# pvjosue/CWFA

Measured on AMD Instinct MI355X. Metric: volumes/sec inverse-pass @512×512×96 fp32; NLL match vs ref (1/2/4/8 GPU), higher is better.
Workload: dtype f32 (storage, accumulation, wavelets, couplings); convolution products on the bf16 matrix cores from an exact three-way bf16 split of both fp32 operands, six products per fp32 product: fp32-equivalent; plain-fp32-MFMA figure: fp32_mfma; 1 GPU; 512x512x96 volume, 4-scale CWFA (CAT blocks, 64 ch) + LRNN inverse, z=0, batch 1/GPU, random-init weights (BASELINE.json configs[2]); precision=split, parallelism=replicated x1 (independent volumes per GPU, no collective)

## Files before the change

### cwfa_amd/_lib.py

```python
import ctypes as C
import os

_HERE = os.path.dirname(os.path.abspath(__file__))
LIB_PATH = os.path.join(_HERE, "libcwfa_hip.so")

CLAMP = {"NONE": 0, "ATAN": 1, "TANH": 2, "SIGMOID": 3}
ACT = {None: 0, "none": 0, "elu": 1, "prelu": 2, "gelu": 3, "relu": 4}
CHAIN_MAX = 8

c_f32p = C.c_void_p
c_i64p = C.c_void_p
c_f64p = C.c_void_p


class AffineStage(C.Structure):
    _fields_ = [("s_raw", c_f32p), ("t", c_f32p), ("s_bs", C.c_int64), ("t_bs", C.c_int64), ("clamp_kind", C.c_int),
                ("clamp", C.c_float), ("pre_scale", C.c_float), ("t_neg_div_sqrt2", C.c_int), ("perm", c_i64p),
                ("perm_axis", C.c_int), ("gin", C.c_int)]


class Chain(C.Structure):
    _fields_ = [("n_stages", C.c_int), ("stage", AffineStage * CHAIN_MAX), ("src_c", C.c_void_p), ("src_h", C.c_void_p)]


class ChainGrads(C.Structure):
    _fields_ = [("ds", c_f32p * CHAIN_MAX), ("dt", c_f32p * CHAIN_MAX), ("ds_bs", C.c_int64 * CHAIN_MAX),
                ("dt_bs", C.c_int64 * CHAIN_MAX)]


class ConvOpts(C.Structure):
    _fields_ = [("bias", c_f32p), ("act", C.c_int), ("prelu_alpha", c_f32p), ("residual", c_f32p), ("res_bs", C.c_int64),
                ("act2", C.c_int), ("in_scale", c_f32p), ("in_shift", c_f32p), ("in_affine_bs", C.c_int), ("in_add", c_f32p),
                ("in_add_bs", C.c_int64), ("upshuffle2", C.c_int), ("in_blocked8", C.c_int), ("out_blocked8", C.c_int),
                ("in_cat", c_f32p), ("in_cat_bs", C.c_int64), ("in_cat_from", C.c_int), ("in_cat_c1", C.c_int), ("out_stats", c_f64p), ("prelu_per_channel", C.c_int),
                ("out_sample_stats", c_f64p)]


class Couple(C.Structure):
    _fields_ = [("x", c_f32p), ("y", c_f32p), ("x_bs", C.c_int64), ("y_bs", C.c_int64), ("n", C.c_int), ("clamp_kind", C.c_int),
                ("clamp", C.c_float), ("pre_scale", C.c_float), ("rev", C.c_int), ("logdet", c_f64p), ("in_blocked8", C.c_int)]


class EvalAffine(C.Structure):
    _fields_ = [("enabled", C.c_int), ("scale", C.c_float), ("std", C.c_float), ("mean", C.c_float)]


class EvalPost(C.Structure):
    _fields_ = [("normalize", C.c_int), ("threshold", C.c_int), ("norm_sub", C.c_float), ("norm_div", C.c_float),
                ("vol_min", C.c_float), ("lower", C.c_float), ("upper", C.c_float), ("clamp_value", C.c_float)]


LION_MAX_TENSORS = 96
LION_BLOCK_ELEMS = 4096


class LionTensor(C.Structure):
    _fields_ = [("p", c_f32p), ("g", c_f32p), ("m", c_f32p), ("numel", C.c_int64)]


class LionTable(C.Structure):
    _fields_ = [("n", C.c_int), ("t", LionTensor * LION_MAX_TENSORS)]


NLL_MAX_LEVELS = 8


class NllLevels(C.Structure):
    _fields_ = [("n", C.c_int), ("level", c_f32p * NLL_MAX_LEVELS), ("bs", C.c_int64 * NLL_MAX_LEVELS)]


EXTREMA_STRIDE = 12
SELECT_WORKSPACE_BYTES = 8448
PREP_MAX_BINS = 10239
PREP_MOMENTS_WORKSPACE = 4096
PREP_VOL = {"none": 0, "two": 1, "le": 2, "maxnorm": 3, "max_only": 4}
PREP_APPLY = {"clamp_zero": 0, "sub_div": 1, "div_mul": 2}
DECONV_PRE = {None: 0, "none": 0, "relu": 1}
DECONV_POST = {None: 0, "none": 0, "abs": 1}

i, i64, f, d, p = C.c_int, C.c_int64, C.c_float, C.c_double, C.c_void_p
SIGNATURES = {
    "cwfa_version": (i, []),
    "cwfa_last_error": (C.c_char_p, []),
    "cwfa_set_option": (i, [C.c_char_p, i]),
    "cwfa_haar1d_fwd_f32": (i, [p, p, p, i, i, i64, i64, i64, i64, p]),
    "cwfa_haar1d_inv_f32": (i, [p, p, p, i, i, i64, i64, i64, i64, p]),
    "cwfa_haar2d_fwd_f32": (i, [p, p, i, i, i, i, i, f, p]),
    "cwfa_haar2d_inv_f32": (i, [p, p, i, i, i, i, i, f, p]),
    "cwfa_haar3d_fwd_f32": (i, [p, p, i, i, i, i, i, f, i64, p]),
    "cwfa_haar3d_inv_f32": (i, [p, p, i, i, i, i, i, f, i64, p]),
    "cwfa_gather_f32": (i, [p, p, p, i, i, i, i, i, i64, i64, p]),
    "cwfa_affine_f32": (i, [p, p, C.POINTER(AffineStage), i, i, i, i, i, i64, i64, p, p, p]),
    "cwfa_channel_affine_f32": (i, [p, p, p, p, i, p, p, i, i, i64, i64, i64, p]),
    "cwfa_chain_inv_f32": (i, [p, p, p, C.POINTER(Chain), i, i, i, i, i64, i64, i64, p, p]),
    "cwfa_chain_inv_var_f32": (i, [p, p, C.POINTER(Chain), f, f, i, i, i, i, i64, i64, p]),
    "cwfa_chain_inv_roi_cov_f32": (i, [p, C.POINTER(Chain), f, i, i, i, i, i, p, i, p, i, p, i64, p]),
    "cwfa_rand_uniform_f32": (i, [p, i, i64, i64, C.c_uint64, C.c_uint32, C.c_uint32, p]),
    "cwfa_rand_trunc_normal_f32": (i, [p, i, i64, i64, f, C.c_uint64, C.c_uint32, C.c_uint32, p]),
    "cwfa_chain_inv_samples_f32": (i, [p, p, p, C.POINTER(Chain), i, i, i, i, i, i64, i64, i64, i64, i64, i64, f, C.c_uint64, C.c_uint32,
                                       C.c_uint32, p]),
    "cwfa_chain_nll_map_f32": (i, [p, p, p, p, C.POINTER(Chain), i, i, i, i, i64, i64, i64, i64, p, p]),
    "cwfa_nll_compose_f32": (i, [C.POINTER(NllLevels), p, i, i, i64, i64, p]),
    "cwfa_chain_fwd_f32": (i, [p, p, p, C.POINTER(Chain), p, i, i, i, i, i64, i64, i64, p, p, p]),
    "cwfa_conv2d_packed_floats": (i64, [i, i, i]),
    "cwfa_conv2d_pack_f32": (i, [p, p, i, i, i, i, p]),
    "cwfa_conv2d_f32": (i, [p, p, p, i, i, i, i, i, i, i64, i64, C.POINTER(ConvOpts), p]),
    "cwfa_subnet_pack1x1_f32": (i, [p, p, p]),
    "cwfa_subnet_layer_tape_f32": (i, [p, p, p, p, p, p, p, i, i, i, i64, i64, i64, p]),
    "cwfa_subnet_layer_f32": (i, [p, p, p, p, p, p, i, i, i, i64, i64, p]),
    "cwfa_conv3d_1k1_f32": (i, [p, p, p, p, p, p, p, i, i, i, i, i, p]),
    "cwfa_conv3d_1k1_split_f32": (i, [p, p, p, p, p, p, p, i, i, i, i, i, p]),
    "cwfa_channel_stats_f32": (i, [p, p, i, i, i64, i64, p]),
    "cwfa_bn_fold_f32": (i, [p, d, p, p, p, p, f, p, i, p, p, i, p]),
    "cwfa_maxpool_f32": (i, [p, p, p, p, p, i, i, i, i, i, i, p]),
    "cwfa_sample_stats_f32": (i, [p, p, i, i64, p]),
    "cwfa_layernorm_apply_f32": (i, [p, p, p, p, f, p, i, i64, p]),
    "cwfa_convnext_tail_f32": (i, [p, p, p, p, f, p, p, p, p, p, p, p, i, p, i, i, i64, i64, i64, i64, i64, p]),
    "cwfa_attention_combine_f32": (i, [p, p, p, p, p, p, p, p, i, i, i64, p]),
    "cwfa_scale_channels_f32": (i, [p, p, p, i, i, i64, p]),
    "cwfa_axpby_f32": (i, [p, p, f, f, p, i64, p]),
    "cwfa_bn_running_update_f32": (i, [p, C.c_double, f, p, p, p, i, p]),
    "cwfa_bn_finish_f32": (i, [p, d, p, p, p, f, i, p, p, f, p, p, f, f, i, p, p, i, i, p]),
    "cwfa_chain_bwd_f32": (i, [p, p, C.POINTER(Chain), C.POINTER(ChainGrads), p, p, i, i, i, i, i64, i64, i64, f, f, i, p, p]),
    "cwfa_affine_bwd_f32": (i, [p, p, C.POINTER(AffineStage), i, i, i, i, i, i64, i64, p, p, p, p, p]),
    "cwfa_chain_inv_bwd_f32": (i, [p, p, C.POINTER(Chain), C.POINTER(ChainGrads), i, i, i, i, i64, i64, f, i, i, p, p, p, p]),
    "cwfa_conv2d_wgrad_workspace_bytes": (i64, [i, i, i, i, i, i]),
    "cwfa_conv2d_wgrad_f32": (i, [p, p, p, p, p, i, i, i, i, i, i, i64, i64, f, p]),
    "cwfa_elu_bwd_f32": (i, [p, p, p, p, i, i64, i64, i64, i64, i64, p]),
    "cwfa_conv3d_hidden_fwd_f32": (i, [p, p, p, p, i, i, i, i, i, p]),
    "cwfa_conv3d_hidden_bwd_f32": (i, [p, p, p, p, p, p, i, i, i, i, i, p]),
    "cwfa_conv3d_input_bwd_f32": (i, [p, p, p, i, i, i, i, i, p]),
    "cwfa_conv3d_wgrad_workspace_bytes": (i64, [i, i, i, i]),
    "cwfa_conv3d_wgrad_f32": (i, [p, p, p, p, p, i, i, i, i, i, i, i, f, p]),
    "cwfa_prelu_bwd_f32": (i, [p, p, p, p, p, i, i64, i64, i64, i64, p]),
    "cwfa_plane_affine_f32": (i, [p, p, p, i, p, p, i, i, i64, i64, i64, i64, p]),
    "cwfa_bn_bwd_stats_f32": (i, [p, p, p, p, i, i, i64, i64, i64, p]),
    "cwfa_bn_act_bwd_f32": (i, [p, p, p, i, p, p, p, p, p, i, i, i64, i64, i64, i64, p]),
    "cwfa_maxpool2_bwd_f32": (i, [p, p, p, p, i, i, i, i, p]),
    "cwfa_gelu_f32": (i, [p, p, p, i64, i, p]),
    "cwfa_layernorm_bwd_f32": (i, [p, p, p, p, p, p, p, p, p, i, i64, p]),
    "cwfa_attention_bwd_f32": (i, [p, p, p, p, p, p, p, p, p, i, i, i64, p]),
    "cwfa_split_workspace_bytes": (i64, [i, i, i64]),
    "cwfa_split_input_f32": (i, [p, p, i, i, i64, i64, p, p, i64, p, i64, p]),
    "cwfa_conv_split_packed_bytes": (i64, [i, i, i]),
    "cwfa_conv_split_pack_f32": (i, [p, p, i, i, i, i, p]),
    "cwfa_conv_split_f32": (i, [p, p, p, i, i, i, i, i, i, i64, C.POINTER(ConvOpts), p]),
    "cwfa_conv3x3_split_packed_bytes": (i64, [i, i]),
    "cwfa_conv3x3_split_pack_f32": (i, [p, p, i, i, p]),
    "cwfa_conv3x3_split_f32": (i, [p, p, p, i, i, i, i, i, i64, i64, C.POINTER(ConvOpts), p]),
    "cwfa_conv7x7_split_packed_bytes": (i64, [i, i]),
    "cwfa_conv7x7_split_pack_f32": (i, [p, p, i, i, p]),
    "cwfa_conv7x7_split_f32": (i, [p, p, p, i, i, i, i, i, i64, i64, C.POINTER(ConvOpts), p]),
    "cwfa_couple_rows": (i, [i, p]),
    "cwfa_conv3x3_split_couple_f32": (i, [p, p, p, i, i, i, i, i64, C.POINTER(Couple), p]),
    "cwfa_subnet_layer_split_packed_bytes": (i64, []),
    "cwfa_subnet_layer_split_pack_f32": (i, [p, p, p, p]),
    "cwfa_subnet_layer_split_f32": (i, [p, p, p, p, p, i, i, i, i64, i64, i, p]),
    "cwfa_subnet_layer_split_tape_f32": (i, [p, p, p, p, p, p, i, i, i, i64, i64, i64, p]),
    "cwfa_conv3x3_out_split_packed_bytes": (i64, [i]),
    "cwfa_conv3x3_out_split_pack_f32": (i, [p, p, i, p]),
    "cwfa_conv3x3_out_split_f32": (i, [p, p, p, p, i, i, i, i, i64, i64, i, p]),
    "cwfa_subnet_layer_first_packed_bytes": (i64, []),
    "cwfa_subnet_layer_first_pack_f32": (i, [p, p, p, i, p, p]),
    "cwfa_subnet_layer_first_f32": (i, [p, p, p, p, p, p, i, i, i, i, i64, i64, i64, i, p]),
    "cwfa_extract_views_f32": (i, [p, p, p, i, i, i, i, i, i, f, f, i64, p]),
    "cwfa_eval_splits": (i64, [i, i64]),
    "cwfa_volume_extrema_f32": (i, [p, p, p, p, i, i64, i64, i64, C.POINTER(EvalAffine), p]),
    "cwfa_volume_metrics_f32": (i, [p, p, p, p, i, i64, i64, i64, C.POINTER(EvalAffine), f, f, f, p]),
    "cwfa_mip3_f32": (i, [p, p, p, p, p, p, i, i, i, i, i64, i64, i, C.POINTER(EvalAffine), C.POINTER(EvalPost), p]),
    "cwfa_projection_compose_f32": (i, [p, p, p, p, p, i, i, i, i, i, i, i, p]),
    "cwfa_roi_means_f32": (i, [p, p, p, i, i, i, i, i, i64, p]),
    "cwfa_select_positive_f32": (i, [p, i, i64, i64, i64, p, p, p, p]),
    "cwfa_prep_volumes_f16": (i, [p, p, p, i, i, i, i, i, i, i, i, i, f, f, i, p]),
    "cwfa_prep_frames_f32": (i, [p, p, i, i, i, i, i, i, i, p]),
    "cwfa_histogram_f32": (i, [p, i64, f, f, p, i, p, i, p]),
    "cwfa_prep_apply_f32": (i, [p, i64, i, f, f, i, p]),
    "cwfa_moments_f64": (i, [p, i64, d, p, p, i, p]),
    "cwfa_stack_mean_std_f32": (i, [p, p, p, i, i64, i64, p]),
    "cwfa_lion_step_f32": (i, [C.POINTER(LionTable), f, f, f, f, p, p, p]),
    "cwfa_wmse_workspace_bytes": (i64, [i64]),
    "cwfa_wmse_loss_f32": (i, [p, p, p, f, f, p, p, p, i64, p]),
    "cwfa_select_nonzero_f32": (i, [p, i, i64, i64, i64, p, p, p, p]),
    "cwfa_deconv_spectrum_mul_c64": (i, [p, p, p, i, i64, i, i, p]),
    "cwfa_deconv_project_f32": (i, [p, p, i, i, i, i, i, i, i, i, i, i, i, p]),
    "cwfa_deconv_ratio_f32": (i, [p, p, p, p, i64, p]),
    "cwfa_deconv_clamp_f32": (i, [p, i64, p, p, f, p]),
    "cwfa_deconv_update_f32": (i, [p, p, i, i, i, i, p]),
}
del i, i64, f, d, p

_lib = None


class CwfaHipError(RuntimeError):
    pass


def lib():
    global _lib
    if _lib is None:
        if not os.path.exists(LIB_PATH):
            raise CwfaHipError(
                f"{LIB_PATH} not found: build the HIP extension first (python -m cwfa_amd.build, or "
                f"__graft_entry__.build()).  cwfa_amd has no CPU / PyTorch fallback.")
        import torch
        h = C.CDLL(LIB_PATH)
        for name, (res, args) in SIGNATURES.items():
            fn = getattr(h, name)
            fn.restype = res
            fn.argtypes = args
        if h.cwfa_version() < 100:
            raise CwfaHipError("libcwfa_hip.so is older than this Python layer")
        _lib = h
    return _lib


def check(rc, what=""):
    if rc != 0:
        msg = lib().cwfa_last_error()
        raise CwfaHipError(f"{what or 'libcwfa_hip'} failed (code {rc}): {msg.decode() if msg else ''}")
```

### cwfa_amd/csrc/conv2d.hip

```cpp
#include "conv_internal.h"

#include <string.h>
#include <type_traits>

namespace {

template <int KS_, int CK_, int MT_, int NT_, int WM_, int WN_, int XV_ = 1>
struct Cfg {
    static constexpr int KS = KS_, CK = CK_, MT = MT_, NT = NT_, WM = WM_, WN = WN_;
    static constexpr int XV = XV_;
    static_assert(XV_ == 1 || (XV_ == 4 && KS_ == 1), "vector staging needs halo-free tiles");
    static constexpr int PAD = KS / 2;
    static constexpr int NTHREADS = 64 * WM * WN;
    static constexpr int CT = 32 * MT * WM;
    static constexpr int TR = NT * WN;
    static constexpr int TC = 32;
    static constexpr int XR = TR + KS - 1;
    static constexpr int XC = TC + KS - 1;
    static constexpr int XS = CK * XR * XC;
    static constexpr int XS_PAD = (XS + 3) & ~3;
    static constexpr int WS = KS * KS * CK * CT;
    static constexpr int XPT = (XS / XV + NTHREADS - 1) / NTHREADS;
    static constexpr int WPT = (WS / 4 + NTHREADS - 1) / NTHREADS;
    static constexpr int BUF = XS_PAD + WS;
// ... 481 lines not shown
    if (ks == 7) return cls == 0 ? Sel{6, C7_32::CT, C7_32::CK} : Sel{7, C7_64::CT, C7_64::CK};
    return Sel{-1, 0, 0};
}

int classify_epilogue(const cwfa_conv_opts& o) {
    const bool res = o.residual != nullptr;
    if (o.out_blocked8) return EPI_NONE_BLK8;
    if (o.upshuffle2) return (!res && o.act == CWFA_ACT_NONE && o.act2 == CWFA_ACT_NONE) ? EPI_UP : EPI_GENERIC;
    if (!res && o.act2 == CWFA_ACT_NONE) {
        if (o.act == CWFA_ACT_NONE) return EPI_NONE;
        if (o.act == CWFA_ACT_ELU) return EPI_ELU;
        if (o.act == CWFA_ACT_PRELU) return EPI_PRELU;
    }
    if (res && o.act == CWFA_ACT_NONE && o.act2 == CWFA_ACT_ELU) return EPI_RES_ELU;
    if (res && o.act == CWFA_ACT_NONE && o.act2 == CWFA_ACT_PRELU) return EPI_RES_PRELU;
    if (res && o.act == CWFA_ACT_GELU && o.act2 == CWFA_ACT_NONE) return EPI_GELU_RES;
    return EPI_GENERIC;
}

template <class C>
int prepare(ConvParams& p, dim3& grid) {
    p.tiles_x = (p.W + C::TC - 1) / C::TC;
    p.tiles_y = (p.H + C::TR - 1) / C::TR;
    p.nchunks = (p.Cin + C::CK - 1) / C::CK;
    const int ctiles = (p.Cout + C::CT - 1) / C::CT;
    CWFA_REQUIRE((int64_t)p.tiles_x * p.tiles_y < (1ll << 31) && ctiles <= 65535 && p.B <= 65535, CWFA_E_SHAPE,
                 "cwfa_conv2d_f32: grid too large");
    CWFA_REQUIRE((int64_t)(p.Cin + C::CK) * p.H * p.W * 4 < (1ll << 31), CWFA_E_SHAPE,
                 "cwfa_conv2d_f32: one sample's input must stay below 2 GiB (32-bit buffer offsets)");
    grid = dim3((unsigned)(p.tiles_x * p.tiles_y), ctiles, p.B);
    return CWFA_OK;
}

template <class C, int EPI, bool PRO>
int launch_epi(ConvParams p, hipStream_t stream) {
    dim3 grid;
    int rc = prepare<C>(p, grid);
    if (rc) return rc;
    constexpr int LDS = EPI == EPI_GENERIC && C::LDS_BYTES < C::NTHREADS * 64 ? C::NTHREADS * 64 : C::LDS_BYTES;
    rc = cwfa_max_lds<&conv2d_mfma_kernel<C, EPI, PRO>>(LDS, "cwfa_conv2d_f32");
    if (rc) return rc;
    hipLaunchKernelGGL((conv2d_mfma_kernel<C, EPI, PRO>), grid, dim3(C::NTHREADS), LDS, stream, p);
    CWFA_LAUNCH_CHECK("cwfa_conv2d_f32");
    return CWFA_OK;
}

template <class C, unsigned ALLOWED, bool PRO>
int launch_sel(const ConvParams& p, int epi, hipStream_t st) {
    if (!(ALLOWED & (1u << epi)) && epi != EPI_NONE_BLK8) epi = EPI_GENERIC;
    switch (epi) {
        case EPI_NONE: if constexpr (ALLOWED & (1u << EPI_NONE)) return launch_epi<C, EPI_NONE, PRO>(p, st); break;
        case EPI_ELU: if constexpr (ALLOWED & (1u << EPI_ELU)) return launch_epi<C, EPI_ELU, PRO>(p, st); break;
        case EPI_RES_ELU: if constexpr (ALLOWED & (1u << EPI_RES_ELU)) return launch_epi<C, EPI_RES_ELU, PRO>(p, st); break;
        case EPI_PRELU: if constexpr (ALLOWED & (1u << EPI_PRELU)) return launch_epi<C, EPI_PRELU, PRO>(p, st); break;
        case EPI_RES_PRELU: if constexpr (ALLOWED & (1u << EPI_RES_PRELU)) return launch_epi<C, EPI_RES_PRELU, PRO>(p, st); break;
        case EPI_GELU_RES: if constexpr (ALLOWED & (1u << EPI_GELU_RES)) return launch_epi<C, EPI_GELU_RES, PRO>(p, st); break;
        case EPI_UP: if constexpr (ALLOWED & (1u << EPI_UP)) return launch_epi<C, EPI_UP, PRO>(p, st); break;
        case EPI_NONE_BLK8:
            if constexpr (ALLOWED & (1u << EPI_NONE_BLK8)) return launch_epi<C, EPI_NONE_BLK8, PRO>(p, st);
            cwfa_set_error("cwfa_conv2d_f32: out_blocked8 is built for the 1x1 kernels with more than 32 output channels");
            return CWFA_E_SHAPE;
        default: break;
    }
    return launch_epi<C, EPI_GENERIC, PRO>(p, st);
}

template <class C, unsigned ALLOWED, unsigned ALLOWED_PRO>
int launch(const ConvParams& p, int epi, hipStream_t st) {
    if (p.o.in_scale || p.o.in_add) return launch_sel<C, ALLOWED_PRO, true>(p, epi, st);
    return launch_sel<C, ALLOWED, false>(p, epi, st);
}

}
int g_cwfa_split_xcd_map = 1;
int g_cwfa_split_rows16 = 1;
extern int g_cwfa_mip3_ablate;
namespace {

int fill_params(ConvParams& p, const char* name, const float* x, const float* w_packed, float* y, int B, int Cin, int H,
                int W, int Cout, int64_t x_bs, int64_t y_bs, const cwfa_conv_opts* opts) {
    CWFA_REQUIRE(B >= 0 && Cin > 0 && Cout > 0 && H >= 0 && W >= 0, CWFA_E_INVAL, "%s: bad size", name);
    if (B == 0 || H == 0 || W == 0) return 1;
    CWFA_REQUIRE(x && w_packed && y, CWFA_E_INVAL, "%s: null pointer", name);
    CWFA_REQUIRE(!opts || !opts->out_sample_stats, CWFA_E_INVAL, "%s: out_sample_stats is a feature of the few-channel cwfa_conv7x7_split_f32", name);
    CWFA_REQUIRE((int64_t)Cin * H * W < (1ll << 30) && (int64_t)Cout * H * W * (p.o.upshuffle2 ? 1 : 1) < (1ll << 30), CWFA_E_SHAPE, "%s: C*H*W exceeds the 32-bit byte offsets of a tile (2^30 elements per image)", name);
    CWFA_REQUIRE(cwfa_aligned16(w_packed), CWFA_E_ALIGN, "%s: packed weights must be 16-byte aligned", name);
    p.x = x; p.wp = w_packed; p.y = y;
    p.B = B; p.Cin = Cin; p.H = H; p.W = W; p.Cout = Cout;
    p.x_bs = x_bs; p.y_bs = y_bs;
    p.products = g_cwfa_operand == CwfaOperand::split3 ? 6 : 1;
    if (opts) p.o = *opts;
    CWFA_REQUIRE(!(p.o.in_scale && !p.o.in_shift), CWFA_E_INVAL, "%s: in_scale without in_shift", name);
    CWFA_REQUIRE(p.o.act >= 0 && p.o.act <= CWFA_ACT_RELU && p.o.act2 >= 0 && p.o.act2 <= CWFA_ACT_RELU, CWFA_E_INVAL,
                 "%s: bad activation", name);
    CWFA_REQUIRE(!((p.o.act == CWFA_ACT_PRELU || p.o.act2 == CWFA_ACT_PRELU) && !p.o.prelu_alpha), CWFA_E_INVAL,
                 "%s: PReLU without prelu_alpha", name);
    return CWFA_OK;
}

typedef Cfg<1, 16, 2, 4, 4, 2> CS;
constexpr int CS_XB = 3 * 2 * 8 * 32 * 16, CS_WB = 3 * 2 * 256 * 16, CS_BUFB = CS_XB + CS_WB;

__device__ __forceinline__ void split3(float v, unsigned short (&o)[3]) {
    const __bf16 a1 = (__bf16)v;
    const float r1 = v - (float)a1;
    const __bf16 a2 = (__bf16)r1;
    const float r2 = r1 - (float)a2;
    const __bf16 a3 = (__bf16)r2;
    o[0] = __builtin_bit_cast(unsigned short, a1);
    o[1] = __builtin_bit_cast(unsigned short, a2);
    o[2] = __builtin_bit_cast(unsigned short, a3);
}

__device__ __forceinline__ unsigned short f16_bits(float v) { return __builtin_bit_cast(unsigned short, (_Float16)v); }

template <bool F16 = false>
__global__ __launch_bounds__(256) void split_input_kernel(const float* __restrict__ x, uint4* __restrict__ ws, int Cin, int CG2,
                                                          int64_t HW, int64_t x_bs, const float* __restrict__ sc,
                                                          const float* __restrict__ sh, int64_t aff_bs,
                                                          const float* __restrict__ add, int64_t add_bs) {
    const int64_t px = (int64_t)blockIdx.x * 256 + threadIdx.x;
    if (px >= HW) return;
    const int cg = blockIdx.y, b = blockIdx.z;
    unsigned short pc[3][8];
#pragma unroll
    for (int j = 0; j < 8; ++j) {
        const int c = cg * 8 + j;
        float v = 0.f;
        if (c < Cin) {
            v = x[(int64_t)b * x_bs + (int64_t)c * HW + px];
            if (sc) v = v * sc[(int64_t)b * aff_bs + c] + sh[(int64_t)b * aff_bs + c];
            if (add) v += add[(int64_t)b * add_bs + (int64_t)c * HW + px];
        }
        if constexpr (F16) {
            pc[0][j] = f16_bits(v);
            continue;
        }
        unsigned short o[3];
        split3(v, o);
        pc[0][j] = o[0]; pc[1][j] = o[1]; pc[2][j] = o[2];
    }
#pragma unroll
    for (int q = 0; q < (F16 ? 1 : 3); ++q) {
        uint4 u;
        u.x = pc[q][0] | ((unsigned)pc[q][1] << 16);
        u.y = pc[q][2] | ((unsigned)pc[q][3] << 16);
        u.z = pc[q][4] | ((unsigned)pc[q][5] << 16);
        u.w = pc[q][6] | ((unsigned)pc[q][7] << 16);
        ws[(((int64_t)b * 3 + q) * CG2 + cg) * HW + px] = u;
    }
}

template <bool F16 = false>
__global__ __launch_bounds__(256) void split_pack_kernel(const float* __restrict__ w, uint4* __restrict__ out, int Cout, int Cin,
                                                         int nchunks, int taps, int transposed, int64_t total) {
    const int64_t i = (int64_t)blockIdx.x * blockDim.x + threadIdx.x;
    if (i >= total) return;
    const int col = (int)(i % 256), h = (int)((i / 256) % 2), tap = (int)((i / 512) % taps);
    const int chunk = (int)((i / (512 * (int64_t)taps)) % nchunks);
    const int ctile = (int)(i / ((int64_t)512 * taps * nchunks));
    const int co = ctile * 256 + col;
    unsigned short pc[3][8];
#pragma unroll
    for (int j = 0; j < 8; ++j) {
        const int ci = chunk * 16 + h * 8 + j;
        float v = 0.f;
        if (co < Cout && ci < Cin)
            v = transposed ? w[((int64_t)ci * (Cout / 4) + (co >> 2)) * 4 + (co & 3)] : w[((int64_t)co * Cin + ci) * taps + tap];
        if constexpr (F16) {
            pc[0][j] = f16_bits(v);
            pc[1][j] = pc[2][j] = 0;
            continue;
        }
        unsigned short o[3];
        split3(v, o);
        pc[0][j] = o[0]; pc[1][j] = o[1]; pc[2][j] = o[2];
    }
#pragma unroll
    for (int q = 0; q < 3; ++q) {
        uint4 u;
        u.x = pc[q][0] | ((unsigned)pc[q][1] << 16);
        u.y = pc[q][2] | ((unsigned)pc[q][3] << 16);
        u.z = pc[q][4] | ((unsigned)pc[q][5] << 16);
        u.w = pc[q][6] | ((unsigned)pc[q][7] << 16);
        out[((((int64_t)ctile * nchunks + chunk) * taps + tap) * 3 + q) * 512 + h * 256 + col] = u;
    }
}

struct SplitParams {
    ConvParams c;
    const void* ws;
    int CG2;
    int64_t ws_bs;
};

template <int EPI, bool F16 = false>
__global__ __launch_bounds__(512, 1) void conv1x1_split_kernel(SplitParams sp) {
    typedef CS C;
    const ConvParams& p = sp.c;
    extern __shared__ __attribute__((aligned(16))) float smem[];
    char* lds = reinterpret_cast<char*>(smem);
    const Tile t = make_tile<C>(p);
    const bool six = p.products != 1;
    const int tid = threadIdx.x, wave = tid >> 6;
    const int64_t HW = (int64_t)p.H * p.W;
    constexpr unsigned OOB = 0x80000000u;

    unsigned xoff[3];
#pragma unroll
    for (int i = 0; i < 3; ++i) {
        const int e = tid + i * 512;
        const int px = e & 31, row = (e >> 5) & 7, h = (e >> 8) & 1, piece = e >> 9;
        const int gr = t.row0 + row, gc = t.col0 + px;
        xoff[i] = (gr < p.H && gc < p.W) ? (unsigned)((((int64_t)piece * sp.CG2 + h) * HW + (int64_t)gr * p.W + gc) * 16) : OOB;
    }
    const auto rx = CWFA_RSRC(reinterpret_cast<const char*>(sp.ws) + (int64_t)t.b * sp.ws_bs, (int)sp.ws_bs);
    const auto rw = CWFA_RSRC(reinterpret_cast<const char*>(p.wp) + (int64_t)t.ct * p.nchunks * CS_WB, p.nchunks * CS_WB);
    const int xchunk = (int)(2 * HW * 16);
    constexpr int NPC = F16 ? 1 : 3;
    auto dma = [&](int chunk, int buf) {
        char* base = lds + buf * CS_BUFB + wave * 1024;
#pragma unroll
        for (int i = 0; i < NPC; ++i)
            __builtin_amdgcn_raw_ptr_buffer_load_lds(rx, (lds_ptr)(base + i * 8192), 16, xoff[i], chunk * xchunk, 0, 0);
#pragma unroll
        for (int i = 0; i < NPC; ++i)
            __builtin_amdgcn_raw_ptr_buffer_load_lds(rw, (lds_ptr)(base + CS_XB + i * 8192), 16, (unsigned)(tid + i * 512) * 16u,
                                                     chunk * CS_WB, 0, 0);
    };

    f32x16 acc[2][4];
#pragma unroll
    for (int m = 0; m < 2; ++m)
#pragma unroll
        for (int n = 0; n < 4; ++n)
#pragma unroll
            for (int r = 0; r < 16; ++r) acc[m][n][r] = 0.f;

    const char* alane = lds + CS_XB + ((t.kh * 256) + t.wm * 64 + t.l31) * 16;
    const char* blane = lds + ((t.kh * 8 + t.wn * 4) * 32 + t.l31) * 16;

    dma(0, 0);
    dma(1, 1);
    if constexpr (F16) asm volatile("s_waitcnt vmcnt(2)" ::: "memory");
    else asm volatile("s_waitcnt vmcnt(6)" ::: "memory");
    __builtin_amdgcn_s_barrier();
    int buf = 0;
    for (int chunk = 0; chunk < p.nchunks; ++chunk) {
        int nb = buf + 2;
        nb = nb >= 3 ? nb - 3 : nb;
        dma(chunk + 2, nb);
        const char* ab = alane + buf * CS_BUFB;
        const char* bb = blane + buf * CS_BUFB;
        bf16x8 A[2][3], Bq[2][3];
#pragma unroll
        for (int m = 0; m < 2; ++m)
#pragma unroll
            for (int q = 0; q < 3; ++q) A[m][q] = *reinterpret_cast<const bf16x8*>(ab + (q * 512 + m * 32) * 16);
#pragma unroll
        for (int q = 0; q < 3; ++q) Bq[0][q] = *reinterpret_cast<const bf16x8*>(bb + (q * 512) * 16);
#pragma unroll
        for (int n = 0; n < 4; ++n) {
            if (n < 3) {
#pragma unroll
                for (int q = 0; q < 3; ++q) Bq[(n + 1) & 1][q] = *reinterpret_cast<const bf16x8*>(bb + (q * 512 + (n + 1) * 32) * 16);
            }
#pragma unroll
            for (int m = 0; m < 2; ++m) {
                f32x16 c = acc[m][n];
                if constexpr (F16) {
                    acc[m][n] = __builtin_amdgcn_mfma_f32_32x32x16_f16(__builtin_bit_cast(f16x8, A[m][0]), __builtin_bit_cast(f16x8, Bq[n & 1][0]),
                                                                       c, 0, 0, 0);
                    continue;
                }
                if (six) {
                    c = __builtin_amdgcn_mfma_f32_32x32x16_bf16(A[m][2], Bq[n & 1][0], c, 0, 0, 0);
                    c = __builtin_amdgcn_mfma_f32_32x32x16_bf16(A[m][1], Bq[n & 1][1], c, 0, 0, 0);
                    c = __builtin_amdgcn_mfma_f32_32x32x16_bf16(A[m][0], Bq[n & 1][2], c, 0, 0, 0);
                    c = __builtin_amdgcn_mfma_f32_32x32x16_bf16(A[m][1], Bq[n & 1][0], c, 0, 0, 0);
                    c = __builtin_amdgcn_mfma_f32_32x32x16_bf16(A[m][0], Bq[n & 1][1], c, 0, 0, 0);
                }
                c = __builtin_amdgcn_mfma_f32_32x32x16_bf16(A[m][0], Bq[n & 1][0], c, 0, 0, 0);
                acc[m][n] = c;
            }
        }
        if constexpr (F16) asm volatile("s_waitcnt vmcnt(2)\n\ts_waitcnt lgkmcnt(0)" ::: "memory");
        else asm volatile("s_waitcnt vmcnt(6)\n\ts_waitcnt lgkmcnt(0)" ::: "memory");
        __builtin_amdgcn_s_barrier();
        buf = buf + 1 == 3 ? 0 : buf + 1;
    }
    asm volatile("s_waitcnt vmcnt(0)" ::: "memory");
    __syncthreads();
    epilogue<C, EPI>(p, t, acc);
}

template <int EPI>
int launch_split(SplitParams sp, hipStream_t stream) {
    ConvParams& p = sp.c;
    p.tiles_x = (p.W + CS::TC - 1) / CS::TC;
    p.tiles_y = (p.H + CS::TR - 1) / CS::TR;
    const int ctiles = (p.Cout + CS::CT - 1) / CS::CT;
    CWFA_REQUIRE((int64_t)p.tiles_x * p.tiles_y < (1ll << 31) && ctiles <= 65535 && p.B <= 65535, CWFA_E_SHAPE,
                 "cwfa_conv_split_f32: grid too large");
    constexpr int LDS = 3 * CS_BUFB;
    return cwfa_with_operand([&](auto, auto f16) -> int {
        constexpr auto kern = &conv1x1_split_kernel<EPI, f16>;
        const int rc = cwfa_max_lds<kern>(LDS, "cwfa_conv_split_f32");
        if (rc) return rc;
        hipLaunchKernelGGL(kern, dim3((unsigned)(p.tiles_x * p.tiles_y), ctiles, p.B), dim3(512), LDS, stream, sp);
        CWFA_LAUNCH_CHECK("cwfa_conv_split_f32");
        return CWFA_OK;
    });
}

}

extern "C" int64_t cwfa_split_workspace_bytes(int B, int Cin, int64_t HW) {
    if (B < 0 || Cin <= 0 || HW < 0) return -1;
    const int64_t CG2 = 2 * ((Cin + 15) / 16);
    return (int64_t)B * 3 * CG2 * HW * 16;
}

extern "C" int cwfa_split_input_f32(const float* x, void* ws, int B, int Cin, int64_t HW, int64_t x_bs, const float* in_scale,
                                    const float* in_shift, int64_t in_affine_bs, const float* in_add, int64_t in_add_bs,
                                    void* stream) {
    CWFA_REQUIRE(x && ws, CWFA_E_INVAL, "cwfa_split_input_f32: null pointer");
    CWFA_REQUIRE(B >= 0 && Cin > 0 && HW >= 0 && B <= 65535, CWFA_E_SHAPE, "cwfa_split_input_f32: bad shape");
    CWFA_REQUIRE(!in_scale == !in_shift, CWFA_E_INVAL, "cwfa_split_input_f32: in_scale and in_shift go together");
    CWFA_REQUIRE(cwfa_aligned16(ws), CWFA_E_ALIGN, "cwfa_split_input_f32: workspace must be 16-byte aligned");
    if (B == 0 || HW == 0) return CWFA_OK;
    const int CG2 = 2 * ((Cin + 15) / 16);
    CWFA_REQUIRE((int64_t)3 * CG2 * HW * 16 < (1ll << 31), CWFA_E_SHAPE, "cwfa_split_input_f32: one sample's planes must stay below 2 GiB");
    return cwfa_with_operand([&](auto, auto f16) -> int {
        hipLaunchKernelGGL(split_input_kernel<f16>, dim3((unsigned)((HW + 255) / 256), CG2, B), dim3(256), 0, (hipStream_t)stream, x,
                           reinterpret_cast<uint4*>(ws), Cin, CG2, HW, x_bs, in_scale, in_shift, in_affine_bs, in_add, in_add_bs);
        CWFA_LAUNCH_CHECK("cwfa_split_input_f32");
        return CWFA_OK;
    });
}

extern "C" int64_t cwfa_conv_split_packed_bytes(int Cout, int Cin, int ks) {
    if (Cout <= 0 || Cin <= 0 || ks != 1) return -1;
    return (int64_t)((Cout + 255) / 256) * ((Cin + 15) / 16) * CS_WB;
}

extern "C" int cwfa_conv_split_pack_f32(const float* w, void* packed, int Cout, int Cin, int ks, int transposed, void* stream) {
    CWFA_REQUIRE(w && packed, CWFA_E_INVAL, "cwfa_conv_split_pack_f32: null pointer");
    CWFA_REQUIRE(Cout > 0 && Cin > 0 && ks == 1 && (!transposed || Cout % 4 == 0), CWFA_E_SHAPE,
                 "cwfa_conv_split_pack_f32: bad shape (1x1 / transposed 2x2 only; 3x3: cwfa_conv3x3_split_pack_f32)");
    CWFA_REQUIRE(cwfa_aligned16(packed), CWFA_E_ALIGN, "cwfa_conv_split_pack_f32: packed image must be 16-byte aligned");
    const int nchunks = (Cin + 15) / 16, taps = ks * ks;
    const int64_t total = (int64_t)((Cout + 255) / 256) * nchunks * taps * 512;
    return cwfa_with_operand([&](auto, auto f16) -> int {
        hipLaunchKernelGGL(split_pack_kernel<f16>, dim3((unsigned)((total + 255) / 256)), dim3(256), 0, (hipStream_t)stream, w,
                           reinterpret_cast<uint4*>(packed), Cout, Cin, nchunks, taps, transposed, total);
        CWFA_LAUNCH_CHECK("cwfa_conv_split_pack_f32");
        return CWFA_OK;
    });
}

extern "C" int cwfa_conv_split_f32(const void* ws, const void* w_packed, float* y, int B, int Cin, int H, int W, int Cout, int ks,
                                   int64_t y_bs, const cwfa_conv_opts* opts, void* stream) {
    CWFA_REQUIRE(!(opts && (opts->in_blocked8 || opts->out_blocked8 || opts->in_cat)), CWFA_E_INVAL,
                 "cwfa_conv_split_f32: blocked layouts / two-source inputs are not built here");
    CWFA_REQUIRE(ws && w_packed && y, CWFA_E_INVAL, "cwfa_conv_split_f32: null pointer");
    CWFA_REQUIRE(ks == 1, CWFA_E_SHAPE, "cwfa_conv_split_f32: kernel size %d (1x1 only; 3x3: cwfa_conv3x3_split_f32)", ks);
    SplitParams sp{};
    int rc = fill_params(sp.c, "cwfa_conv_split_f32", reinterpret_cast<const float*>(ws), reinterpret_cast<const float*>(w_packed), y,
                         B, Cin, H, W, Cout, 0, y_bs, opts);
    if (rc) return rc < 0 ? rc : CWFA_OK;
    ConvParams& p = sp.c;
    CWFA_REQUIRE(!p.o.in_scale && !p.o.in_add, CWFA_E_INVAL, "cwfa_conv_split_f32: the load-side prologue belongs in cwfa_split_input_f32");
    CWFA_REQUIRE(!p.o.upshuffle2 || (ks == 1 && Cout % 4 == 0), CWFA_E_SHAPE, "cwfa_conv_split_f32: upshuffle2 needs ks=1, Cout=4*Co");
    CWFA_REQUIRE(!p.o.out_stats && !p.o.prelu_per_channel, CWFA_E_INVAL, "cwfa_conv_split_f32: out_stats / prelu_per_channel are features of cwfa_conv3x3_split_f32");
    p.nchunks = (Cin + 15) / 16;
    sp.ws = ws;
    sp.CG2 = 2 * p.nchunks;
    sp.ws_bs = (int64_t)3 * sp.CG2 * H * W * 16;
    CWFA_REQUIRE(sp.ws_bs + (int64_t)4 * H * W * 16 < (1ll << 31) && (int64_t)(p.nchunks * ks * ks + 2) * CS_WB < (1ll << 31), CWFA_E_SHAPE,
                 "cwfa_conv_split_f32: one sample's planes / one cout tile's weights must stay below 2 GiB");
    const int epi = classify_epilogue(p.o);
    hipStream_t st = (hipStream_t)stream;
    switch (epi) {
        case EPI_NONE: return launch_split<EPI_NONE>(sp, st);
        case EPI_UP: return launch_split<EPI_UP>(sp, st);
        default: return launch_split<EPI_GENERIC>(sp, st);
    }
}

int g_cwfa_wino_min_cout = 1;
int g_cwfa_wino_2d = 512;
CwfaOperand g_cwfa_operand = CwfaOperand::split3;

extern "C" int cwfa_set_option(const char* name, int value) {
    CWFA_REQUIRE(name, CWFA_E_INVAL, "cwfa_set_option: null name");
    if (strcmp(name, "winograd_min_cout") == 0) {
        g_cwfa_wino_min_cout = value;
        return CWFA_OK;
    }
    if (strcmp(name, "winograd_2d") == 0) {
        g_cwfa_wino_2d = value;
        return CWFA_OK;
    }
    if (strcmp(name, "wgrad_split") == 0) {
        g_cwfa_wgrad_split = value != 0;
        return CWFA_OK;
    }
    if (strcmp(name, "wgrad_rows") == 0) {
        g_cwfa_wgrad_rows = value;
        return CWFA_OK;
    }
    if (strcmp(name, "split3x3_xcd_map") == 0) {
        g_cwfa_split_xcd_map = value;
        return CWFA_OK;
    }
    if (strcmp(name, "mip3_ablate") == 0) {
        CWFA_REQUIRE(value >= 0 && value <= 7, CWFA_E_INVAL, "cwfa_set_option: mip3_ablate is a mask of bits 0..2");
        g_cwfa_mip3_ablate = value;
        return CWFA_OK;
    }
    if (strcmp(name, "split3x3_rows16") == 0) {
        g_cwfa_split_rows16 = value;
        return CWFA_OK;
    }
    if (strcmp(name, "split_products") == 0) {
        CWFA_REQUIRE(value == 1 || value == 6, CWFA_E_INVAL, "cwfa_set_option: split_products must be 1 or 6");
        CWFA_REQUIRE(value == 1 || g_cwfa_operand != CwfaOperand::fp16, CWFA_E_INVAL,
                     "cwfa_set_option: split_products = 6 needs split_operand = 0 (the three-piece split is a bf16 format)");
        if (value == 6) g_cwfa_operand = CwfaOperand::split3;
        else if (g_cwfa_operand == CwfaOperand::split3) g_cwfa_operand = CwfaOperand::bf16;
        return CWFA_OK;
    }
    if (strcmp(name, "split_operand") == 0) {
        CWFA_REQUIRE(value == 0 || value == 1, CWFA_E_INVAL, "cwfa_set_option: split_operand must be 0 (bf16) or 1 (fp16)");
        CWFA_REQUIRE(value == 0 || g_cwfa_operand != CwfaOperand::split3, CWFA_E_INVAL,
                     "cwfa_set_option: split_operand = 1 (fp16) needs split_products = 1 (fp16 operands take one product)");
        if (value == 1) g_cwfa_operand = CwfaOperand::fp16;
        else if (g_cwfa_operand == CwfaOperand::fp16) g_cwfa_operand = CwfaOperand::bf16;
        return CWFA_OK;
    }
    cwfa_set_error("cwfa_set_option: unknown option '%s'", name);
    return CWFA_E_INVAL;
}

extern "C" int64_t cwfa_conv2d_packed_floats(int Cout, int Cin, int ks) {
    const Sel s = select_cfg(ks, Cout);
    if (s.id < 0 || Cout <= 0 || Cin <= 0) return -1;
    if (cwfa_wino_selected(ks, Cout)) return cwfa_wino_packed_floats(Cout, Cin);
    const int64_t ctiles = (Cout + s.CT - 1) / s.CT, nchunks = (Cin + s.CK - 1) / s.CK;
    return ctiles * nchunks * ks * ks * s.CK * s.CT;
}

extern "C" int cwfa_conv2d_pack_f32(const float* w, float* packed, int Cout, int Cin, int ks, int transposed, void* stream) {
    CWFA_REQUIRE(w && packed, CWFA_E_INVAL, "cwfa_conv2d_pack_f32: null pointer");
    CWFA_REQUIRE(!transposed || (ks == 1 && Cout % 4 == 0), CWFA_E_SHAPE,
                 "cwfa_conv2d_pack_f32: transposed source needs ks=1 (2x2 stride-2 deconv as 1x1) and Cout = 4*Co");
    const int64_t total = cwfa_conv2d_packed_floats(Cout, Cin, ks);
    CWFA_REQUIRE(total > 0, CWFA_E_SHAPE, "cwfa_conv2d_pack_f32: unsupported filter %dx%d, Cout=%d, Cin=%d", ks, ks, Cout, Cin);
    if (cwfa_wino_selected(ks, Cout)) return cwfa_wino_pack(w, packed, Cout, Cin, (hipStream_t)stream);
    const Sel s = select_cfg(ks, Cout);
    const int nchunks = (Cin + s.CK - 1) / s.CK;
    hipLaunchKernelGGL(pack_kernel, dim3((unsigned)((total + 255) / 256)), dim3(256), 0, (hipStream_t)stream, w, packed, Cout,
                       Cin, ks, s.CT, s.CK, nchunks, total, transposed);
    CWFA_LAUNCH_CHECK("cwfa_conv2d_pack_f32");
    return CWFA_OK;
}

extern "C" int cwfa_conv2d_f32(const float* x, const float* w_packed, float* y, int B, int Cin, int H, int W, int Cout, int ks,
                               int64_t x_bs, int64_t y_bs, const cwfa_conv_opts* opts, void* stream) {
    CWFA_REQUIRE(!(opts && opts->in_blocked8), CWFA_E_INVAL, "cwfa_conv2d_f32: in_blocked8 is a cwfa_conv3x3_split_f32 feature");
    CWFA_REQUIRE(!(opts && opts->in_cat) || (ks == 1 && Cout <= 64 && !opts->in_scale && !opts->in_add && opts->in_cat_from % 16 == 0 &&
                                             opts->in_cat_from > 0 && opts->in_cat_from < Cin && opts->in_cat_c1 > 0 &&
                                             opts->in_cat_c1 <= opts->in_cat_from),
                 CWFA_E_INVAL, "cwfa_conv2d_f32: in_cat needs a 1x1 bank with <= 64 outputs packed with in_cat_from (a multiple of 16) "
                               "columns for the first source, and no load-side affine / add");
    CWFA_REQUIRE(!(opts && opts->out_blocked8) || (ks == 1 && Cout % 8 == 0 && !opts->residual && opts->act == CWFA_ACT_NONE &&
                                                   opts->act2 == CWFA_ACT_NONE && !opts->upshuffle2 && !opts->in_scale && !opts->in_add &&
                                                   cwfa_aligned16(y) && (y_bs & 3) == 0 && (!opts->bias || cwfa_aligned16(opts->bias))),
                 CWFA_E_INVAL, "cwfa_conv2d_f32: out_blocked8 needs a plain 1x1 bank (bias only), Cout %% 8 == 0 and 16-byte aligned y / bias");
    const Sel s = select_cfg(ks, Cout);
    CWFA_REQUIRE(s.id >= 0, CWFA_E_SHAPE, "cwfa_conv2d_f32: kernel size %d not in {1,3,7}", ks);
    ConvParams p{};
    int rc = fill_params(p, "cwfa_conv2d_f32", x, w_packed, y, B, Cin, H, W, Cout, x_bs, y_bs, opts);
    if (rc) return rc < 0 ? rc : CWFA_OK;
    CWFA_REQUIRE(!p.o.upshuffle2 || (ks == 1 && Cout % 4 == 0), CWFA_E_SHAPE, "cwfa_conv2d_f32: upshuffle2 needs ks=1, Cout=4*Co");
    CWFA_REQUIRE(!p.o.out_stats && !p.o.prelu_per_channel, CWFA_E_INVAL, "cwfa_conv2d_f32: out_stats / prelu_per_channel are features of cwfa_conv3x3_split_f32");
    const int epi = classify_epilogue(p.o);
    hipStream_t st = (hipStream_t)stream;
    if (cwfa_wino_selected(ks, Cout)) return cwfa_wino_conv(x, w_packed, y, B, Cin, H, W, Cout, x_bs, y_bs, p.o, st);
// ... 69 lines not shown
```

### cwfa_amd/csrc/conv_split3x3.hip

```cpp
#include "conv_internal.h"

extern int g_cwfa_split_xcd_map;
extern int g_cwfa_split_rows16;

namespace {

constexpr int TR = 8, TC = 32;

template <int KS, int RPW = 4>
struct XG {
    static constexpr int TRW = 2 * RPW, NT = 2 * RPW;
    static constexpr int PAD = KS / 2, XR = TRW + 2 * PAD, XC = TC + 2 * PAD, NTAP = KS * KS;
    static constexpr int EPK = XR * XC;
    static constexpr int KHB = KS == 7 ? 8512 : RPW == 8 ? 9792 : 5440;
    static constexpr int XPB = 2 * KHB;
    static constexpr int XB = 3 * XPB;
    static constexpr bool SPECIAL = KS == 3 && RPW == 4;
    static constexpr int NEK = SPECIAL ? 2 : 3;
    static_assert(EPK * 16 <= KHB && KHB % 256 == 64 && 2 * EPK <= 512 * NEK, "staging entry map");
    static_assert(!SPECIAL || (EPK > 256 && EPK <= 384), "3x3 staging entry map");
    static_assert(KS == 3 || RPW == 4, "7x7: 8-row tiles");
};

template <int MPW, int KS = 3, int RPW = 4, int WM = 4>
// ... 229 lines not shown
            for (int mt = 0; mt < MPW; ++mt) {
                mfma6(acc[mt][nt], A[mt], Bq[nt % NB]);
                CWFA_FENCE();
                if (MA < MPW && nt == 0 && mt == 0) {
                    read_a(abase, MA, MPW);
#pragma unroll
                    for (int n2 = 1; n2 < NB && n2 < NT; ++n2) read_b(n2, bbase, n2);
                    CWFA_FENCE();
                }
            }
            if (nt == 0) {
                if (P == LA || P == LB) load_entry(cwfa_ic<0>{}, xs[0], sk[0], P == LA ? ce + 2 : co + 2);
                if (P == LA + 1 || P == LB + 1) load_entry(cwfa_ic<1>{}, xs[1], sk[1], P == LA + 1 ? ce + 2 : co + 2);
                if constexpr (NEK > 2) {
                    if (P == LA + 2 || P == LB + 2) load_entry(cwfa_ic<NEK - 1>{}, xs[NEK - 1], sk[NEK - 1], P == LA + 2 ? ce + 2 : co + 2);
                }
                CWFA_FENCE();
            }
            if (nt == 1) {
                dma_w(step + 1, sl ^ 1);
                CWFA_FENCE();
            }
        }
        {
            const int nP = P == NTAP - 1 ? 0 : P + 1;
            const int nA = 2 * nP, nB = 2 * nP + 1;
            const int nbufA = nA >= NTAP, ntA = nA - NTAP * nbufA, nbufB = nB >= NTAP, ntB = nB - NTAP * nbufB;
            const int noffA = nbufA * XB + ((ntA / KS) * XC + ntA % KS) * 16, noffB = nbufB * XB + ((ntB / KS) * XC + ntB % KS) * 16;
            read_b(0, blane + (sel ? noffB : noffA), 0);
            CWFA_FENCE();
        }
        asm volatile("s_waitcnt vmcnt(0)" ::: "memory");
        if constexpr (SIX) asm volatile("s_waitcnt lgkmcnt(3)" ::: "memory");
        else asm volatile("s_waitcnt lgkmcnt(1)" ::: "memory");
        __builtin_amdgcn_s_barrier();
        sl ^= 1;
        if (++P == NTAP) {
            P = 0;
            ce += 2;
        }
    }
    asm volatile("s_waitcnt vmcnt(0)" ::: "memory");

    const auto ry = CWFA_RSRC(p.y + (int64_t)b * p.y_bs, p.Cout * plane);
    const auto rr = CWFA_RSRC(p.o.residual ? p.o.residual + (int64_t)b * p.o.res_bs : p.y, p.o.residual ? p.Cout * plane : 0);
    const auto rb = CWFA_RSRC(p.o.bias ? p.o.bias : p.y, p.o.bias ? p.Cout * 4 : 0);
    const bool alpha_pc = p.o.prelu_per_channel != 0;
    const float alpha = (p.o.prelu_alpha && !alpha_pc) ? *p.o.prelu_alpha : 0.f;
    const auto rpa = CWFA_RSRC(alpha_pc ? p.o.prelu_alpha : p.y, alpha_pc ? p.Cout * 4 : 0);
    const int cwave = ct * CT + wm * MPW * 16;
    const unsigned glane = (unsigned)(4 * g) * (unsigned)plane;
    if constexpr (ACT1 == EPI_COUPLE) {
        static_assert(MPW <= 2 && !ADD, "coupling epilogue: narrow tilings only");
        constexpr int NP = MPW == 1 ? 2 : 4;
        const cwfa_couple& cp = p.cp;
        const auto cx = CWFA_RSRC(cp.x + (int64_t)b * cp.x_bs, cp.n * plane);
        const auto cy = CWFA_RSRC(cp.y + (int64_t)b * cp.y_bs, cp.n * plane);
        const unsigned jlane = (unsigned)((MPW == 1 ? 2 : 4) * g) * (unsigned)plane;
        const int jwave = wm * (MPW == 1 ? 8 : 16);
        float bs[NP], bt[NP];
#pragma unroll
        for (int k = 0; k < NP; ++k) {
            const int rs = k, rt = MPW == 1 ? k + 2 : 16 + k;
            bs[k] = __builtin_bit_cast(float, __builtin_amdgcn_raw_buffer_load_b32(rb, (unsigned)(16 * g), (cwave + rs) * 4, 0));
            bt[k] = __builtin_bit_cast(float, __builtin_amdgcn_raw_buffer_load_b32(rb, (unsigned)(16 * g), (cwave + rt) * 4, 0));
        }
        float ssum = 0.f;
#pragma unroll
        for (int nt = 0; nt < NT; ++nt) {
            const int row = row0 + wn * RW + (nt >> 1), col = col0 + 16 * (nt & 1) + c16;
            const bool ok = row < p.H && col < p.W;
            const unsigned po = ok ? (unsigned)((row * p.W + col) * 4) + jlane : OOB;
            float xv[NP];
#pragma unroll
            for (int k = 0; k < NP; ++k) xv[k] = __builtin_bit_cast(float, __builtin_amdgcn_raw_buffer_load_b32(cx, po, (jwave + k) * plane, 0));
#pragma unroll
            for (int k = 0; k < NP; ++k) {
                const float sr = acc[0][nt][k] + bs[k];
                float tr;
                if constexpr (MPW == 1) tr = acc[0][nt][k + 2] + bt[k];
                else tr = acc[MPW - 1][nt][k] + bt[k];
                const float sv = cwfa_soft_clamp(sr * cp.pre_scale, cp.clamp_kind, cp.clamp);
                const float tv = tr * cp.pre_scale;
                const float yv = cp.rev ? (xv[k] - tv) * __expf(-sv) : __expf(sv) * xv[k] + tv;
                __builtin_amdgcn_raw_buffer_store_b32(__builtin_bit_cast(unsigned, yv), cy, po, (jwave + k) * plane, 0);
                ssum += ok ? sv : 0.f;
            }
            CWFA_FENCE();
        }
        if (cp.logdet) {
            const double ws = cwfa_wave_sum((double)ssum);
            double* red = reinterpret_cast<double*>(lds);
            __builtin_amdgcn_s_barrier();
            if (lane == 0) red[wave] = ws;
            __syncthreads();
            if (tid == 0) {
                double tot = 0.0;
#pragma unroll
                for (int w = 0; w < 8; ++w) tot += red[w];
                atomicAdd(&cp.logdet[b], cp.rev ? -tot : tot);
            }
        }
        return;
    }
    const bool outb = p.o.out_blocked8 != 0;
    const bool want_stats = ACT1 != EPI_RUNTIME && p.o.out_stats != nullptr;
    float* red = reinterpret_cast<float*>(lds);
#pragma unroll
    for (int mt = 0; mt < MPW; ++mt) {
        float bias[4];
        float st1[4] = {0.f, 0.f, 0.f, 0.f}, st2[4] = {0.f, 0.f, 0.f, 0.f};
#pragma unroll
        for (int r = 0; r < 4; ++r)
            bias[r] = __builtin_bit_cast(float, __builtin_amdgcn_raw_buffer_load_b32(rb, (unsigned)(16 * g), (cwave + mt * 16 + r) * 4, 0));
        float al[4] = {alpha, alpha, alpha, alpha};
        if (alpha_pc) {
#pragma unroll
            for (int r = 0; r < 4; ++r)
                al[r] = __builtin_bit_cast(float, __builtin_amdgcn_raw_buffer_load_b32(rpa, (unsigned)(16 * g), (cwave + mt * 16 + r) * 4, 0));
        }
        constexpr int RLA = NT < 4 ? NT : 4;
        float rv[ACT1 == EPI_RUNTIME ? NT : 1][4];
        auto load_res = [&](int nt) {
            const int row = row0 + wn * RW + (nt >> 1), col = col0 + 16 * (nt & 1) + c16;
            const unsigned po = (row < p.H && col < p.W) ? (unsigned)((row * p.W + col) * 4) + glane : OOB;
#pragma unroll
            for (int r = 0; r < 4; ++r)
                rv[ACT1 == EPI_RUNTIME ? nt : 0][r] = __builtin_bit_cast(float, __builtin_amdgcn_raw_buffer_load_b32(rr, po, (cwave + mt * 16 + r) * plane, 0));
        };
        if constexpr (ACT1 == EPI_RUNTIME) {
#pragma unroll
            for (int nt = 0; nt < NT; ++nt)
#pragma unroll
                for (int r = 0; r < 4; ++r) rv[nt][r] = 0.f;
            if (p.o.residual) {
#pragma unroll
                for (int nt = 0; nt < RLA; ++nt) load_res(nt);
            }
            CWFA_FENCE();
        }
#pragma unroll
        for (int nt = 0; nt < NT; ++nt) {
            const int row = row0 + wn * RW + (nt >> 1), col = col0 + 16 * (nt & 1) + c16;
            if constexpr (ACT1 == EPI_RUNTIME) {
                if (nt + RLA < NT && p.o.residual) load_res(nt + RLA);
                CWFA_FENCE();
            }
            if constexpr (ACT1 != EPI_RUNTIME) {
                if (outb) {
                    f32x4 o4;
#pragma unroll
                    for (int r = 0; r < 4; ++r) o4[r] = cwfa_act_ct<ACT1>(acc[mt][nt][r] + bias[r], al[r]);
                    const unsigned pb = (row < p.H && col < p.W) ? (unsigned)(((g >> 1) * HW + row * p.W + col) * 32 + (g & 1) * 16) : OOB;
                    cwfa_buffer_store_b128(__builtin_bit_cast(u32x4, o4), ry, pb, (cwave + mt * 16) * plane);
                    continue;
                }
            }
            const unsigned po = (row < p.H && col < p.W) ? (unsigned)((row * p.W + col) * 4) + glane : OOB;
#pragma unroll
            for (int r = 0; r < 4; ++r) {
                const int soff = (cwave + mt * 16 + r) * plane;
                float v = acc[mt][nt][r] + bias[r];
                if constexpr (ACT1 == EPI_RUNTIME) {
                    v = cwfa_act(v, p.o.act, al[r]);
                    v += rv[nt][r];
                    v = cwfa_act(v, p.o.act2, al[r]);
                } else {
                    v = cwfa_act_ct<ACT1>(v, al[r]);
                    if (want_stats) {
                        const float vm = po != OOB ? v : 0.f;
                        st1[r] += vm;
                        st2[r] += vm * vm;
                    }
                }
                __builtin_amdgcn_raw_buffer_store_b32(__builtin_bit_cast(unsigned, v), ry, po, soff, 0);
            }
            CWFA_FENCE();
        }
        if constexpr (ACT1 != EPI_RUNTIME) {
            if (want_stats) {
#pragma unroll
                for (int r = 0; r < 4; ++r) {
                    const float a1 = cwfa_row16_sum(st1[r]), a2 = cwfa_row16_sum(st2[r]);
                    if (c16 == 0) {
                        const int ch = (wm * MPW + mt) * 16 + 4 * g + r;
                        red[(wn * CT + ch) * 2] = a1;
                        red[(wn * CT + ch) * 2 + 1] = a2;
                    }
                }
            }
        }
    }
    if constexpr (ACT1 != EPI_RUNTIME) {
        if (want_stats) {
            asm volatile("s_waitcnt lgkmcnt(0)\n\ts_barrier" ::: "memory");
            const int ch = ct * CT + tid;
            if (tid < CT && ch < p.Cout) {
                double s1 = 0.0, s2 = 0.0;
#pragma unroll
                for (int k = 0; k < WN; ++k) {
                    s1 += (double)red[(k * CT + tid) * 2];
                    s2 += (double)red[(k * CT + tid) * 2 + 1];
                }
                atomicAdd(&p.o.out_stats[2 * ch], s1);
                atomicAdd(&p.o.out_stats[2 * ch + 1], s2);
            }
        }
    }
}

namespace few {
constexpr int XR = TR + 6, XC = TC + 6, EPK = XR * XC;
constexpr int XPB = EPK * 16;
constexpr int NSTEP = 13, CT = 64, MPW = 2, WM = 2, WN = 4, RW = 2, NT = 4;
constexpr int WSL = 3 * 4 * CT * 16;
constexpr int OFF_W = 3 * XPB, LDS = OFF_W + 2 * WSL;
static_assert(2 * 512 >= EPK && 2 * LDS <= 160 * 1024, "few-channel 7x7: staging map / two blocks per CU");
}

template <bool SIX, bool F16>
__global__ __launch_bounds__(512, 2) void conv7x7_few_split_kernel(SParams p) {
    using namespace few;
    extern __shared__ __attribute__((aligned(16))) char lds[];
    const int tid = threadIdx.x, lane = tid & 63, c16 = lane & 15, g = lane >> 4;
    const int wave = __builtin_amdgcn_readfirstlane(tid >> 6);
    const int wm = wave % WM, wn = wave / WM;
    const int plane = p.H * p.W * 4;
    constexpr unsigned OOB = 0x80000000u;
    constexpr int NQ = SIX ? 3 : 1;
    const int b = blockIdx.z;
    int sp;
    if (p.xcd_map && (p.ntiles & 7) == 0) sp = (blockIdx.x & 7) * (p.ntiles >> 3) + (blockIdx.x >> 3);
    else sp = blockIdx.x;
    const int row0 = (sp / p.tiles_x) * TR, col0 = (sp % p.tiles_x) * TC;

    constexpr int NPC = (SIX ? WSL : WSL / 3) / 1024;
    const auto rw = CWFA_RSRC(p.wp, NSTEP * WSL);
    auto dma_w = [&](int slice, int slot) {
        cwfa_static_for<(NPC + 7) / 8>([&](auto ic_) {
            constexpr int i = decltype(ic_)::value;
            const int piece = i * 8 + wave;
            if (piece < NPC) {
                char* dst = lds + OFF_W + slot * WSL + piece * 1024;
                __builtin_amdgcn_raw_ptr_buffer_load_lds(rw, (lds_ptr)dst, 16, (unsigned)(lane * 16), slice * WSL + piece * 1024, 0, 0);
            }
        });
    };

    {
        const auto rx = CWFA_RSRC(p.x + (int64_t)b * p.x_bs, p.Cin * plane);
        float xv[2][8];
#pragma unroll
        for (int k = 0; k < 2; ++k) {
            const int e = tid + 512 * k, r = e / XC, c = e % XC;
            const int gr = row0 + r - 3, gc = col0 + c - 3;
            const bool ok = e < EPK && gr >= 0 && gr < p.H && gc >= 0 && gc < p.W;
            const unsigned fo = ok ? (unsigned)((gr * p.W + gc) * 4) : OOB;
#pragma unroll
            for (int j = 0; j < 8; ++j) xv[k][j] = __builtin_bit_cast(float, __builtin_amdgcn_raw_buffer_load_b32(rx, fo, j * plane, 0));
        }
        dma_w(0, 0);
#pragma unroll
        for (int k = 0; k < 2; ++k) {
            const int e = tid + 512 * k;
            bf16x8 pc[3];
#pragma unroll
            for (int j = 0; j < 8; ++j) {
                __bf16 a1, a2 = (__bf16)0.f, a3 = (__bf16)0.f;
                cwfa_split3<SIX, F16>(xv[k][j], a1, a2, a3);
                pc[0][j] = a1; pc[1][j] = a2; pc[2][j] = a3;
            }
            if (e < EPK) {
#pragma unroll
                for (int q = 0; q < NQ; ++q) *reinterpret_cast<bf16x8*>(lds + q * XPB + e * 16) = pc[q];
            }
        }
    }
    asm volatile("s_waitcnt vmcnt(0)\n\ts_waitcnt lgkmcnt(0)" ::: "memory");
    __builtin_amdgcn_s_barrier();

    const int alane = OFF_W + (g * CT + wm * MPW * 16 + c16) * 16;
    const int blane = (wn * RW * XC + c16) * 16;
    auto bbase_of = [&](int s) {
        const int t = 4 * s + g < 48 ? 4 * s + g : 48;
        return blane + ((t / 7) * XC + t % 7) * 16;
    };

    f32x4 acc[MPW][NT];
#pragma unroll
    for (int mt = 0; mt < MPW; ++mt)
#pragma unroll
        for (int nt = 0; nt < NT; ++nt) acc[mt][nt] = f32x4{0.f, 0.f, 0.f, 0.f};
    bf16x8 A[MPW][3], Bq[2][3];
    auto read_b = [&](int set, int bbase, int nt) {
#pragma unroll
        for (int q = 0; q < NQ; ++q)
            Bq[set][q] = *reinterpret_cast<const bf16x8*>(lds + bbase + q * XPB + ((nt >> 1) * XC + 16 * (nt & 1)) * 16);
    };
    auto mfma6 = [&](f32x4& c, const bf16x8 (&a)[3], const bf16x8 (&bb)[3]) {
        if constexpr (SIX) {
            CWFA_MFMA(a[2], bb[0], c);
            CWFA_MFMA(a[1], bb[1], c);
            CWFA_MFMA(a[0], bb[2], c);
            CWFA_MFMA(a[1], bb[0], c);
            CWFA_MFMA(a[0], bb[1], c);
        }
// ... 163 lines not shown
inline int nsteps_of(int Cin, int ntap = 9) { return ntap * (((Cin + 15) / 16 + 1) / 2); }

template <int MPW, bool ADD, int ACT1, int KS = 3, int RPW = 4, int WM = 4>
int launch(const SParams& p, hipStream_t stream) {
    typedef Geo<MPW, KS, RPW, WM> G;
    constexpr int TRW = XG<KS, RPW>::TRW;
    const int tiles_y = (p.H + TRW - 1) / TRW, ctiles = (p.Cout + G::CT - 1) / G::CT;
    SParams q = p;
    q.ntiles = p.tiles_x * tiles_y;
    q.ctiles = ctiles;
    q.xcd_map = g_cwfa_split_xcd_map;
    if ((int64_t)q.ntiles * ctiles >= (1ll << 31)) {
        cwfa_set_error("cwfa_conv3x3_split_f32: grid too large");
        return CWFA_E_SHAPE;
    }
    if ((ACT1 == EPI_RUNTIME || ACT1 == EPI_COUPLE) && (p.o.out_stats || p.o.out_blocked8)) {
        cwfa_set_error("cwfa_conv3x3_split_f32: out_stats / out_blocked8 reached a run-time epilogue");
        return CWFA_E_INVAL;
    }
    return cwfa_with_operand([&](auto six, auto f16) -> int {
        constexpr auto kern = &conv3x3_split_kernel<MPW, six, ADD, ACT1, KS, RPW, WM, f16>;
        const int rc = cwfa_max_lds<kern>(G::LDS, "cwfa_conv3x3_split_f32");
        if (rc) return rc;
        hipLaunchKernelGGL(kern, dim3((unsigned)(q.ntiles * ctiles), 1, p.B), dim3(512), G::LDS, stream, q);
        CWFA_LAUNCH_CHECK("cwfa_conv3x3_split_f32");
        return CWFA_OK;
    });
}

template <int MPW>
int launch_epi(const SParams& p, hipStream_t st) {
    const bool plain = !p.o.residual && p.o.act2 == CWFA_ACT_NONE;
    if (p.o.in_add) {
        if (plain && p.o.act == CWFA_ACT_PRELU) return launch<MPW, true, CWFA_ACT_PRELU>(p, st);
        return launch<MPW, true, EPI_RUNTIME>(p, st);
    }
    if (plain && p.o.act == CWFA_ACT_PRELU) return launch<MPW, false, CWFA_ACT_PRELU>(p, st);
    if (plain && p.o.act == CWFA_ACT_NONE) return launch<MPW, false, CWFA_ACT_NONE>(p, st);
    return launch<MPW, false, EPI_RUNTIME>(p, st);
}

void pack_bank(const float* w, void* packed, int Cout, int Cin, int ct, int ntap, hipStream_t st) {
    const int nchunks = (Cin + 15) / 16, nsteps = nsteps_of(Cin, ntap);
    const int64_t total = (int64_t)((Cout + ct - 1) / ct) * nsteps * 4 * ct;
    cwfa_with_operand([&](auto, auto f16) -> int {
        auto go = [&](auto CT) {
            hipLaunchKernelGGL((split3x3_pack_kernel<decltype(CT)::value, f16>), dim3((unsigned)((total + 255) / 256)), dim3(256), 0, st, w,
                               reinterpret_cast<uint4*>(packed), Cout, Cin, nchunks, nsteps, total, ntap);
        };
        if (ct == 16) go(cwfa_ic<16>{});
        else if (ct == 32) go(cwfa_ic<32>{});
        else if (ct == 48) go(cwfa_ic<48>{});
        else if (ct == 96) go(cwfa_ic<96>{});
        else if (ct == 128) go(cwfa_ic<128>{});
        else if (ct == 256) go(cwfa_ic<256>{});
        else go(cwfa_ic<64>{});
        return CWFA_OK;
    });
}

}

static int couple_row_source(int n, int r) {
    int j, which;
    if (n <= 32) {
        const int wm = r >> 4, g = (r >> 2) & 3, q = r & 3;
        j = 8 * wm + 2 * g + (q & 1);
        which = q >> 1;
    } else {
        const int wm = r >> 5;
        which = (r >> 4) & 1;
        j = 16 * wm + (r & 15);
    }
    return j < n ? which * n + j : -1;
}

extern "C" int cwfa_couple_rows(int n, int* rows) {
    if (n <= 0 || n > 64) return -1;
    const int total = n <= 32 ? 64 : 128;
    if (rows)
        for (int r = 0; r < total; ++r) rows[r] = couple_row_source(n, r);
    return total;
}

extern "C" int cwfa_conv3x3_split_couple_f32(const float* x, const void* w_packed, const float* bias_rows, int B, int Cin, int H, int W,
                                             int64_t x_bs, const cwfa_couple* cp, void* stream) {
    CWFA_REQUIRE(B >= 0 && Cin > 0 && H >= 0 && W >= 0, CWFA_E_INVAL, "cwfa_conv3x3_split_couple_f32: bad size");
    CWFA_REQUIRE(cp, CWFA_E_INVAL, "cwfa_conv3x3_split_couple_f32: null coupling descriptor");
    CWFA_REQUIRE(cp->n > 0 && cp->n <= 64, CWFA_E_SHAPE, "cwfa_conv3x3_split_couple_f32: 1 <= n <= 64 (got %d)", cp->n);
    if (B == 0 || H == 0 || W == 0) return CWFA_OK;
    CWFA_REQUIRE(x && w_packed && cp->x && cp->y, CWFA_E_INVAL, "cwfa_conv3x3_split_couple_f32: null pointer");
    CWFA_REQUIRE(cwfa_aligned16(w_packed), CWFA_E_ALIGN, "cwfa_conv3x3_split_couple_f32: packed weights must be 16-byte aligned");
    CWFA_REQUIRE(cp->clamp_kind >= CWFA_CLAMP_NONE && cp->clamp_kind <= CWFA_CLAMP_SIGMOID, CWFA_E_INVAL,
                 "cwfa_conv3x3_split_couple_f32: bad clamp kind %d", cp->clamp_kind);
    SParams p{};
    p.x = x; p.wp = w_packed; p.y = cp->y;
    p.B = B; p.Cin = Cin; p.H = H; p.W = W; p.x_bs = x_bs; p.y_bs = cp->y_bs;
    p.Cout = cwfa_couple_rows(cp->n, nullptr);
    p.o.bias = bias_rows;
    p.o.in_blocked8 = cp->in_blocked8;
    CWFA_REQUIRE(!cp->in_blocked8 || (Cin % 8 == 0 && cwfa_aligned16(x) && (x_bs & 3) == 0), CWFA_E_ALIGN,
                 "cwfa_conv3x3_split_couple_f32: blocked input needs Cin %% 8 == 0 and 16-byte alignment");
    p.cp = *cp;
    p.nchunks = (Cin + 15) / 16;
    p.nsteps = nsteps_of(Cin);
    p.nrun = p.nsteps - ((p.nchunks & 1) ? 4 : 0);
    p.tiles_x = (W + TC - 1) / TC;
    CWFA_REQUIRE((int64_t)(Cin + 64) * H * W * 4 < (1ll << 31) && (int64_t)(cp->n + 64) * H * W * 4 < (1ll << 31), CWFA_E_SHAPE,
                 "cwfa_conv3x3_split_couple_f32: one sample's input / active half must stay below 2 GiB");
    CWFA_REQUIRE((int64_t)p.tiles_x * ((H + TR - 1) / TR) < (1ll << 31) && B <= 65535, CWFA_E_SHAPE,
                 "cwfa_conv3x3_split_couple_f32: grid too large");
    hipStream_t st = (hipStream_t)stream;
    if (p.Cout == 64) {
        if (g_cwfa_split_rows16 && H > 8)
            return launch<1, false, EPI_COUPLE, 3, 8>(p, st);
        return launch<1, false, EPI_COUPLE>(p, st);
    }
    return launch<2, false, EPI_COUPLE>(p, st);
}

extern "C" int64_t cwfa_conv3x3_split_packed_bytes(int Cout, int Cin) {
    if (Cout <= 0 || Cin <= 0) return -1;
    const int ct = ct_of(Cout);
    return (int64_t)((Cout + ct - 1) / ct) * nsteps_of(Cin) * 3 * 4 * ct * 16;
}

extern "C" int cwfa_conv3x3_split_pack_f32(const float* w, void* packed, int Cout, int Cin, void* stream) {
    CWFA_REQUIRE(w && packed, CWFA_E_INVAL, "cwfa_conv3x3_split_pack_f32: null pointer");
    CWFA_REQUIRE(Cout > 0 && Cin > 0, CWFA_E_SHAPE, "cwfa_conv3x3_split_pack_f32: bad shape");
    CWFA_REQUIRE(cwfa_aligned16(packed), CWFA_E_ALIGN, "cwfa_conv3x3_split_pack_f32: packed image must be 16-byte aligned");
    pack_bank(w, packed, Cout, Cin, ct_of(Cout), 9, (hipStream_t)stream);
    CWFA_LAUNCH_CHECK("cwfa_conv3x3_split_pack_f32");
    return CWFA_OK;
}

extern "C" int cwfa_conv3x3_split_f32(const float* x, const void* w_packed, float* y, int B, int Cin, int H, int W, int Cout,
                                      int64_t x_bs, int64_t y_bs, const cwfa_conv_opts* opts, void* stream) {
    CWFA_REQUIRE(B >= 0 && Cin > 0 && Cout > 0 && H >= 0 && W >= 0, CWFA_E_INVAL, "cwfa_conv3x3_split_f32: bad size");
    if (B == 0 || H == 0 || W == 0) return CWFA_OK;
    CWFA_REQUIRE(x && w_packed && y, CWFA_E_INVAL, "cwfa_conv3x3_split_f32: null pointer");
    CWFA_REQUIRE(cwfa_aligned16(w_packed), CWFA_E_ALIGN, "cwfa_conv3x3_split_f32: packed weights must be 16-byte aligned");
    SParams p{};
    p.x = x; p.wp = w_packed; p.y = y;
    p.B = B; p.Cin = Cin; p.H = H; p.W = W; p.Cout = Cout; p.x_bs = x_bs; p.y_bs = y_bs;
    if (opts) p.o = *opts;
    CWFA_REQUIRE(!p.o.upshuffle2 && !p.o.in_cat, CWFA_E_SHAPE, "cwfa_conv3x3_split_f32: upshuffle2 / in_cat are 1x1 features");
    CWFA_REQUIRE(!p.o.out_sample_stats, CWFA_E_INVAL, "cwfa_conv3x3_split_f32: out_sample_stats is a feature of the few-channel cwfa_conv7x7_split_f32");
    CWFA_REQUIRE(!p.o.in_blocked8 || (Cin % 8 == 0 && cwfa_aligned16(x) && (x_bs & 3) == 0 && !p.o.in_add), CWFA_E_ALIGN,
                 "cwfa_conv3x3_split_f32: blocked input needs Cin %% 8 == 0, 16-byte alignment and no added tensor");
    CWFA_REQUIRE(!p.o.out_blocked8 || (Cout % 8 == 0 && cwfa_aligned16(y) && (y_bs & 3) == 0 && !p.o.residual && p.o.act2 == CWFA_ACT_NONE &&
                                       (p.o.act == CWFA_ACT_NONE || p.o.act == CWFA_ACT_PRELU)),
                 CWFA_E_ALIGN, "cwfa_conv3x3_split_f32: blocked output needs Cout %% 8 == 0, 16-byte alignment and a bias / PReLU epilogue");
    CWFA_REQUIRE(!(p.o.in_scale && !p.o.in_shift), CWFA_E_INVAL, "cwfa_conv3x3_split_f32: in_scale without in_shift");
    CWFA_REQUIRE(!p.o.out_stats || (!p.o.out_blocked8 && !p.o.residual && p.o.act2 == CWFA_ACT_NONE &&
                                    (p.o.act == CWFA_ACT_NONE || p.o.act == CWFA_ACT_PRELU)),
                 CWFA_E_INVAL, "cwfa_conv3x3_split_f32: out_stats needs an NCHW output and a bias / PReLU epilogue");
    CWFA_REQUIRE(!((p.o.out_stats || p.o.out_blocked8) && p.o.in_add && p.o.act == CWFA_ACT_NONE), CWFA_E_INVAL,
                 "cwfa_conv3x3_split_f32: out_stats / out_blocked8 with in_add need a PReLU epilogue");
    CWFA_REQUIRE(p.o.act >= 0 && p.o.act <= CWFA_ACT_RELU && p.o.act2 >= 0 && p.o.act2 <= CWFA_ACT_RELU, CWFA_E_INVAL,
                 "cwfa_conv3x3_split_f32: bad activation");
    CWFA_REQUIRE(!((p.o.act == CWFA_ACT_PRELU || p.o.act2 == CWFA_ACT_PRELU) && !p.o.prelu_alpha), CWFA_E_INVAL,
                 "cwfa_conv3x3_split_f32: PReLU without prelu_alpha");
    p.nchunks = (Cin + 15) / 16;
    p.nsteps = nsteps_of(Cin);
    p.nrun = p.nsteps - ((p.nchunks & 1) ? 4 : 0);
    p.tiles_x = (W + TC - 1) / TC;
    const int mpw = mpw_of(Cout);
    CWFA_REQUIRE((int64_t)(Cin + 64) * H * W * 4 < (1ll << 31) && (int64_t)(Cout + 64 * mpw) * H * W * 4 < (1ll << 31) &&
                     (int64_t)(p.nsteps + 2) * 3 * 4 * 64 * mpw * 16 < (1ll << 31), CWFA_E_SHAPE,
                 "cwfa_conv3x3_split_f32: one sample's input / output / one cout tile's weights must stay below 2 GiB");
    CWFA_REQUIRE((int64_t)p.tiles_x * ((H + TR - 1) / TR) < (1ll << 31) && B <= 65535, CWFA_E_SHAPE, "cwfa_conv3x3_split_f32: grid too large");
    hipStream_t st = (hipStream_t)stream;
    const int wm = wm_of(Cout);
    if (wm != 4) {
        CWFA_REQUIRE(!p.o.in_scale && !p.o.in_add && !p.o.out_blocked8, CWFA_E_INVAL,
                     "cwfa_conv3x3_split_f32: banks with <= 48 or 65 .. 96 outputs take no load-side prologue and write NCHW");
        const bool plain = !p.o.residual && p.o.act2 == CWFA_ACT_NONE;
        const int epi = plain && p.o.act == CWFA_ACT_NONE ? 0 : plain && p.o.act == CWFA_ACT_PRELU ? 1 : 2;
#define CWFA_NARROW(M, W_)                                                                                                                   \
    do {                                                                                                                                     \
        if (epi == 0) return launch<M, false, CWFA_ACT_NONE, 3, 8, W_>(p, st);                                                               \
        if (epi == 1) return launch<M, false, CWFA_ACT_PRELU, 3, 8, W_>(p, st);                                                              \
        return launch<M, false, EPI_RUNTIME, 3, 8, W_>(p, st);                                                                               \
    } while (0)
        if (mpw == 3 && wm == 2) CWFA_NARROW(3, 2);
        if (mpw == 3) CWFA_NARROW(3, 1);
        if (mpw == 2) CWFA_NARROW(2, 1);
        CWFA_NARROW(1, 1);
#undef CWFA_NARROW
    }
    if (mpw == 4) return launch_epi<4>(p, st);
    if (mpw == 2) return launch_epi<2>(p, st);
    if (g_cwfa_split_rows16 && H > 8 && !p.o.in_scale && !p.o.in_add && !p.o.residual && p.o.act == CWFA_ACT_NONE && p.o.act2 == CWFA_ACT_NONE)
        return launch<2, false, CWFA_ACT_NONE, 3, 8, 2>(p, st);
    if (g_cwfa_split_rows16 && H > 8 && !p.o.in_scale && !p.o.in_add && !p.o.out_stats && !p.o.out_blocked8)
        return launch<2, false, EPI_RUNTIME, 3, 8, 2>(p, st);
    return launch_epi<1>(p, st);
}

extern "C" int64_t cwfa_conv7x7_split_packed_bytes(int Cout, int Cin) {
    if (Cout <= 0 || Cout > 64 || Cin <= 0) return -1;
    if (Cin <= 8) return (int64_t)few::NSTEP * few::WSL;
    return (int64_t)nsteps_of(Cin, 49) * 3 * 4 * 64 * 16;
}

extern "C" int cwfa_conv7x7_split_pack_f32(const float* w, void* packed, int Cout, int Cin, void* stream) {
    CWFA_REQUIRE(w && packed, CWFA_E_INVAL, "cwfa_conv7x7_split_pack_f32: null pointer");
    CWFA_REQUIRE(Cout > 0 && Cout <= 64 && Cin > 0, CWFA_E_SHAPE, "cwfa_conv7x7_split_pack_f32: 1 <= Cout <= 64");
    CWFA_REQUIRE(cwfa_aligned16(packed), CWFA_E_ALIGN, "cwfa_conv7x7_split_pack_f32: packed image must be 16-byte aligned");
    if (Cin <= 8) {
        cwfa_with_operand([&](auto, auto f16) -> int {
            hipLaunchKernelGGL((split7x7_few_pack_kernel<f16>), dim3((few::NSTEP * 4 * 64 + 255) / 256), dim3(256), 0, (hipStream_t)stream, w,
                               reinterpret_cast<uint4*>(packed), Cout, Cin);
            return CWFA_OK;
        });
    } else {
        pack_bank(w, packed, Cout, Cin, 64, 49, (hipStream_t)stream);
    }
    CWFA_LAUNCH_CHECK("cwfa_conv7x7_split_pack_f32");
    return CWFA_OK;
}

extern "C" int cwfa_conv7x7_split_f32(const float* x, const void* w_packed, float* y, int B, int Cin, int H, int W, int Cout,
                                      int64_t x_bs, int64_t y_bs, const cwfa_conv_opts* opts, void* stream) {
    CWFA_REQUIRE(B >= 0 && Cin > 0 && Cout > 0 && Cout <= 64 && H >= 0 && W >= 0, CWFA_E_INVAL, "cwfa_conv7x7_split_f32: bad size (Cout <= 64)");
    if (B == 0 || H == 0 || W == 0) return CWFA_OK;
    CWFA_REQUIRE(x && w_packed && y, CWFA_E_INVAL, "cwfa_conv7x7_split_f32: null pointer");
    CWFA_REQUIRE(cwfa_aligned16(w_packed), CWFA_E_ALIGN, "cwfa_conv7x7_split_f32: packed weights must be 16-byte aligned");
    SParams p{};
    p.x = x; p.wp = w_packed; p.y = y;
    p.B = B; p.Cin = Cin; p.H = H; p.W = W; p.Cout = Cout; p.x_bs = x_bs; p.y_bs = y_bs;
    if (opts) p.o = *opts;
    CWFA_REQUIRE(!p.o.upshuffle2 && !p.o.in_cat && !p.o.in_scale && !p.o.in_add && !p.o.in_blocked8 && !p.o.out_blocked8 && !p.o.residual && !p.o.out_stats &&
                     p.o.act == CWFA_ACT_NONE && p.o.act2 == CWFA_ACT_NONE,
                 CWFA_E_INVAL, "cwfa_conv7x7_split_f32: bias-only epilogue, no load-side prologue, NCHW maps");
    CWFA_REQUIRE(!p.o.out_sample_stats || Cin <= 8, CWFA_E_INVAL, "cwfa_conv7x7_split_f32: out_sample_stats is written by the few-channel form (Cin <= 8) only");
    p.nchunks = (Cin + 15) / 16;
    p.nsteps = nsteps_of(Cin, 49);
    p.nrun = p.nchunks == 1 ? 25 : p.nsteps;
    p.tiles_x = (W + TC - 1) / TC;
    CWFA_REQUIRE((int64_t)(Cin + 64) * H * W * 4 < (1ll << 31) && (int64_t)(Cout + 64) * H * W * 4 < (1ll << 31), CWFA_E_SHAPE,
                 "cwfa_conv7x7_split_f32: one sample's input / output must stay below 2 GiB");
    CWFA_REQUIRE((int64_t)p.tiles_x * ((H + TR - 1) / TR) < (1ll << 31) && B <= 65535, CWFA_E_SHAPE, "cwfa_conv7x7_split_f32: grid too large");
    hipStream_t st = (hipStream_t)stream;
    if (Cin <= 8) {
        p.ntiles = p.tiles_x * ((H + TR - 1) / TR);
        p.ctiles = 1;
        p.xcd_map = g_cwfa_split_xcd_map;
        return cwfa_with_operand([&](auto six, auto f16) -> int {
            constexpr auto kern = &conv7x7_few_split_kernel<six, f16>;
            const int rc = cwfa_max_lds<kern>(few::LDS, "cwfa_conv7x7_split_f32");
            if (rc) return rc;
            hipLaunchKernelGGL(kern, dim3((unsigned)p.ntiles, 1, B), dim3(512), few::LDS, st, p);
            CWFA_LAUNCH_CHECK("cwfa_conv7x7_split_f32");
            return CWFA_OK;
        });
    }
    return launch<2, false, CWFA_ACT_NONE, 7, 4, 2>(p, st);
}
```

### cwfa_amd/csrc/lrnn_ops.hip

```cpp
#include "common.h"

__global__ __launch_bounds__(256) void channel_stats_kernel(const float* __restrict__ x, double* __restrict__ stats, int64_t HW,
                                                            int64_t x_bs, int vec_ok) {
    __shared__ double red[16];
    const int c = blockIdx.y;
    const float* p = x + (int64_t)blockIdx.z * x_bs + (int64_t)c * HW;
    const int64_t per = (((HW + gridDim.x - 1) / gridDim.x) + 3) & ~(int64_t)3;
    const int64_t lo = (int64_t)blockIdx.x * per < HW ? (int64_t)blockIdx.x * per : HW, hi = lo + per < HW ? lo + per : HW;
    double s = 0.0, q = 0.0;
    if (vec_ok && (lo & 3) == 0) {
        const int64_t n4 = (hi - lo) >> 2;
        const f32x4* p4 = reinterpret_cast<const f32x4*>(p + lo);
        int64_t i = threadIdx.x;
        for (; i + 3 * (int64_t)blockDim.x < n4; i += 4 * (int64_t)blockDim.x) {
            f32x4 v[4];
#pragma unroll
            for (int u = 0; u < 4; ++u) v[u] = p4[i + u * (int64_t)blockDim.x];
#pragma unroll
            for (int u = 0; u < 4; ++u) {
                s += ((double)v[u][0] + (double)v[u][1]) + ((double)v[u][2] + (double)v[u][3]);
                q += ((double)v[u][0] * v[u][0] + (double)v[u][1] * v[u][1]) + ((double)v[u][2] * v[u][2] + (double)v[u][3] * v[u][3]);
            }
        }
        for (; i < n4; i += blockDim.x) {
// ... 75 lines not shown
                                 const float* __restrict__ mask_u, float drop_p, float keep_scale, int B, float* __restrict__ scale,
                                 float* __restrict__ shift, int C, int zero_stats) {
    const int c = blockIdx.x * blockDim.x + threadIdx.x;
    if (c == 0 && nbt && update_running) *nbt += 1;
    if (c >= C) return;
    double sc = 1.0, sh = 0.0;
    if (stats || rm) {
        double mean, var;
        if (stats) {
            const double s1 = stats[2 * c], s2 = stats[2 * c + 1];
            mean = s1 / count;
            var = s2 / count - mean * mean;
            if (var < 0.0) var = 0.0;
            if (update_running) {
                const double var_u = (s2 - s1 * mean) / (count > 1.0 ? count - 1.0 : 1.0);
                rm[c] = rm[c] * (1.f - momentum) + momentum * (float)mean;
                rv[c] = rv[c] * (1.f - momentum) + momentum * (float)var_u;
            }
            if (zero_stats) stats[2 * c] = stats[2 * c + 1] = 0.0;
        } else {
            mean = rm[c];
            var = rv[c];
        }
        sc = (w ? (double)w[c] : 1.0) / sqrt(var + (double)eps);
        sh = (bsh ? (double)bsh[c] : 0.0) - mean * sc;
    }
    if (mask || mask_u) {
        for (int b = 0; b < B; ++b) {
            const float m = mask ? mask[b * C + c] : (mask_u[b * C + c] >= drop_p ? 1.f : 0.f) / keep_scale;
            scale[b * C + c] = (float)sc * m;
            shift[b * C + c] = (float)sh * m;
        }
    } else {
        scale[c] = (float)sc;
        shift[c] = (float)sh;
    }
}

extern "C" int cwfa_bn_finish_f32(double* stats, double count, float* running_mean, float* running_var, long long* num_batches_tracked,
                                  float momentum, int update_running, const float* weight, const float* bias, float eps,
                                  const float* mask_bc, const float* mask_u, float drop_p, float keep_scale, int B, float* scale,
                                  float* shift, int C, int zero_stats, void* stream) {
    CWFA_REQUIRE(scale && shift, CWFA_E_INVAL, "cwfa_bn_finish_f32: null output");
    CWFA_REQUIRE(stats || (running_mean && running_var) || mask_bc || mask_u, CWFA_E_INVAL,
                 "cwfa_bn_finish_f32: neither batch nor running statistics nor a mask");
    CWFA_REQUIRE(!running_mean == !running_var, CWFA_E_INVAL, "cwfa_bn_finish_f32: running_mean and running_var go together");
    CWFA_REQUIRE(!(mask_bc && mask_u), CWFA_E_INVAL, "cwfa_bn_finish_f32: a mask OR a uniform draw");
    CWFA_REQUIRE(!(mask_bc || mask_u) || B > 0, CWFA_E_INVAL, "cwfa_bn_finish_f32: mask needs B > 0");
    CWFA_REQUIRE(!mask_u || (drop_p >= 0.f && drop_p < 1.f), CWFA_E_INVAL, "cwfa_bn_finish_f32: 0 <= drop_p < 1");
    CWFA_REQUIRE(!stats || count > 0, CWFA_E_INVAL, "cwfa_bn_finish_f32: count must be positive");
    CWFA_REQUIRE(!update_running || (stats && running_mean), CWFA_E_INVAL, "cwfa_bn_finish_f32: the running update needs statistics and buffers");
    CWFA_REQUIRE(C >= 0, CWFA_E_INVAL, "cwfa_bn_finish_f32: negative size");
    if (C == 0) return CWFA_OK;
    CWFA_REQUIRE(!mask_u || keep_scale > 0.f, CWFA_E_INVAL, "cwfa_bn_finish_f32: keep_scale = fp32(1 - p) must be positive");
    hipLaunchKernelGGL(bn_finish_kernel, dim3((C + 255) / 256), dim3(256), 0, (hipStream_t)stream, stats, count, running_mean, running_var,
                       num_batches_tracked, momentum, update_running, weight, bias, eps, mask_bc, mask_u, drop_p, keep_scale, B, scale,
                       shift, C, zero_stats);
    CWFA_LAUNCH_CHECK("cwfa_bn_finish_f32");
    return CWFA_OK;
}

__global__ void bn_running_update_kernel(const double* __restrict__ stats, double count, float momentum, float* __restrict__ rm,
                                         float* __restrict__ rv, long long* __restrict__ nbt, int C) {
    const int c = blockIdx.x * blockDim.x + threadIdx.x;
    if (c == 0 && nbt) *nbt += 1;
    if (c >= C) return;
    const double mean = stats[2 * c] / count;
    const double var_u = (stats[2 * c + 1] - stats[2 * c] * mean) / (count > 1.0 ? count - 1.0 : 1.0);
    rm[c] = rm[c] * (1.f - momentum) + momentum * (float)mean;
    rv[c] = rv[c] * (1.f - momentum) + momentum * (float)var_u;
}

extern "C" int cwfa_bn_running_update_f32(const double* stats, double count, float momentum, float* running_mean,
                                          float* running_var, long long* num_batches_tracked, int C, void* stream) {
    CWFA_REQUIRE(stats && running_mean && running_var, CWFA_E_INVAL, "cwfa_bn_running_update_f32: null pointer");
    CWFA_REQUIRE(C >= 0 && count > 0.0, CWFA_E_INVAL, "cwfa_bn_running_update_f32: bad size");
    if (C == 0) return CWFA_OK;
    hipLaunchKernelGGL(bn_running_update_kernel, dim3((C + 127) / 128), dim3(128), 0, (hipStream_t)stream, stats, count, momentum,
                       running_mean, running_var, num_batches_tracked, C);
    CWFA_LAUNCH_CHECK("cwfa_bn_running_update_f32");
    return CWFA_OK;
}

extern "C" int cwfa_bn_fold_f32(const double* stats, double count, const float* running_mean, const float* running_var,
                                const float* weight, const float* bias, float eps, const float* mask_bc, int B, float* scale,
                                float* shift, int C, void* stream) {
    CWFA_REQUIRE(scale && shift, CWFA_E_INVAL, "cwfa_bn_fold_f32: null output");
    CWFA_REQUIRE(stats || (running_mean && running_var) || mask_bc, CWFA_E_INVAL,
                 "cwfa_bn_fold_f32: neither batch nor running statistics nor a mask");
    CWFA_REQUIRE(!running_mean == !running_var, CWFA_E_INVAL, "cwfa_bn_fold_f32: running_mean and running_var go together");
    CWFA_REQUIRE(!mask_bc || B > 0, CWFA_E_INVAL, "cwfa_bn_fold_f32: mask needs B > 0");
    CWFA_REQUIRE(!stats || count > 0, CWFA_E_INVAL, "cwfa_bn_fold_f32: count must be positive");
    CWFA_REQUIRE(C >= 0, CWFA_E_INVAL, "cwfa_bn_fold_f32: negative size");
    if (C == 0) return CWFA_OK;
    hipLaunchKernelGGL(bn_fold_kernel, dim3((C + 255) / 256), dim3(256), 0, (hipStream_t)stream, stats, count, running_mean,
                       running_var, weight, bias, eps, mask_bc, B, scale, shift, C);
    CWFA_LAUNCH_CHECK("cwfa_bn_fold_f32");
    return CWFA_OK;
}

__global__ __launch_bounds__(256) void maxpool_kernel(const float* __restrict__ x, float* __restrict__ y,
                                                      float* __restrict__ full, const float* __restrict__ scale,
                                                      const float* __restrict__ shift, int C, int H, int W, int Ho, int Wo) {
    const int64_t n = (int64_t)Ho * Wo;
    const int64_t i = (int64_t)blockIdx.x * blockDim.x + threadIdx.x;
    if (i >= n) return;
    const int bc = blockIdx.y, c = bc % C;
    const int oy = (int)(i / Wo), ox = (int)(i % Wo);
    const int y0 = (int)(((int64_t)oy * H) / Ho), y1 = (int)((((int64_t)oy + 1) * H + Ho - 1) / Ho);
    const int x0 = (int)(((int64_t)ox * W) / Wo), x1 = (int)((((int64_t)ox + 1) * W + Wo - 1) / Wo);
    const float sc = scale ? scale[c] : 1.f, sh = shift ? shift[c] : 0.f;
    const float* px = x + (int64_t)bc * H * W;
    float* pf = full ? full + (int64_t)bc * H * W : nullptr;
    float m = -INFINITY;
    for (int yy = y0; yy < y1; ++yy)
        for (int xx = x0; xx < x1; ++xx) {
            float v = px[(int64_t)yy * W + xx];
            if (scale) v = v * sc + sh;
            if (pf) pf[(int64_t)yy * W + xx] = v;
            m = (v > m || v != v) ? v : m;
        }
    y[(int64_t)bc * n + i] = m;
}

__global__ __launch_bounds__(256) void maxpool2x2_kernel(const float* __restrict__ x, float* __restrict__ y, float* __restrict__ full,
                                                         const float* __restrict__ scale, const float* __restrict__ shift, int C,
                                                         int H, int W) {
    const int Wo = W >> 1, Ho = H >> 1, wq = W >> 2;
    const int64_t i = (int64_t)blockIdx.x * blockDim.x + threadIdx.x;
    if (i >= (int64_t)Ho * wq) return;
    const int bc = blockIdx.y, c = bc % C;
    const int oy = (int)(i / wq), q = (int)(i % wq);
    const float sc = scale ? scale[c] : 1.f, sh = shift ? shift[c] : 0.f;
    const int64_t o = (int64_t)bc * H * W + (int64_t)(2 * oy) * W + 4 * q;
    f32x4 r0 = *reinterpret_cast<const f32x4*>(x + o), r1 = *reinterpret_cast<const f32x4*>(x + o + W);
    if (scale) {
        r0 = r0 * sc + sh;
        r1 = r1 * sc + sh;
    }
    if (full) {
        *reinterpret_cast<f32x4*>(full + o) = r0;
        *reinterpret_cast<f32x4*>(full + o + W) = r1;
    }
    float m[2];
#pragma unroll
    for (int k = 0; k < 2; ++k) {
        float a = -INFINITY;
        const float v4[4] = {r0[2 * k], r0[2 * k + 1], r1[2 * k], r1[2 * k + 1]};
#pragma unroll
        for (int j = 0; j < 4; ++j) a = (v4[j] > a || v4[j] != v4[j]) ? v4[j] : a;
        m[k] = a;
    }
    *reinterpret_cast<float2*>(y + (int64_t)bc * Ho * Wo + (int64_t)oy * Wo + 2 * q) = make_float2(m[0], m[1]);
}

extern "C" int cwfa_maxpool_f32(const float* x, float* y, float* full, const float* scale, const float* shift, int B, int C,
                                int H, int W, int Ho, int Wo, void* stream) {
    CWFA_REQUIRE(x && y, CWFA_E_INVAL, "cwfa_maxpool_f32: null pointer");
    CWFA_REQUIRE(!(scale && !shift), CWFA_E_INVAL, "cwfa_maxpool_f32: scale without shift");
    CWFA_REQUIRE(B >= 0 && C >= 0 && H > 0 && W > 0 && Ho > 0 && Wo > 0 && Ho <= H && Wo <= W, CWFA_E_SHAPE,
                 "cwfa_maxpool_f32: bad shape");
    CWFA_REQUIRE((int64_t)B * C <= 65535, CWFA_E_SHAPE, "cwfa_maxpool_f32: B*C too large");
    if (B == 0 || C == 0) return CWFA_OK;
    const int64_t n = (int64_t)Ho * Wo;
    if (H == 2 * Ho && W == 2 * Wo && (W & 3) == 0 && cwfa_aligned16(x) && (!full || cwfa_aligned16(full)) &&
        (reinterpret_cast<uintptr_t>(y) & 7) == 0) {
        hipLaunchKernelGGL(maxpool2x2_kernel, dim3((unsigned)((n / 2 + 255) / 256), B * C), dim3(256), 0, (hipStream_t)stream, x, y, full,
                           scale, shift, C, H, W);
        CWFA_LAUNCH_CHECK("cwfa_maxpool_f32");
        return CWFA_OK;
    }
    hipLaunchKernelGGL(maxpool_kernel, dim3((unsigned)((n + 255) / 256), B * C), dim3(256), 0, (hipStream_t)stream, x, y, full,
                       scale, shift, C, H, W, Ho, Wo);
    CWFA_LAUNCH_CHECK("cwfa_maxpool_f32");
    return CWFA_OK;
}

__global__ __launch_bounds__(256) void sample_stats_kernel(const float* __restrict__ x, double* __restrict__ stats,
                                                           int64_t CHW) {
    __shared__ double red[16];
    const int b = blockIdx.y;
    const float* px = x + (int64_t)b * CHW;
    double s = 0.0, q = 0.0;
    for (int64_t i = (int64_t)blockIdx.x * blockDim.x + threadIdx.x; i < CHW; i += (int64_t)gridDim.x * blockDim.x) {
        const float v = px[i];
        s += v;
        q += (double)v * v;
    }
    s = cwfa_block_sum(s, red);
    q = cwfa_block_sum(q, red);
    if (threadIdx.x == 0) {
        atomicAdd(&stats[2 * b], s);
        atomicAdd(&stats[2 * b + 1], q);
    }
}

extern "C" int cwfa_sample_stats_f32(const float* x, double* stats, int B, int64_t CHW, void* stream) {
    CWFA_REQUIRE(x && stats, CWFA_E_INVAL, "cwfa_sample_stats_f32: null pointer");
    CWFA_REQUIRE(B >= 0 && CHW >= 0 && B <= 65535, CWFA_E_SHAPE, "cwfa_sample_stats_f32: bad shape");
    if (B == 0 || CHW == 0) return CWFA_OK;
    int blocks = (int)((CHW + 256 * 16 - 1) / (256 * 16));
    if (blocks < 1) blocks = 1;
    if (blocks > 1024) blocks = 1024;
    hipLaunchKernelGGL(sample_stats_kernel, dim3(blocks, B), dim3(256), 0, (hipStream_t)stream, x, stats, CHW);
    CWFA_LAUNCH_CHECK("cwfa_sample_stats_f32");
    return CWFA_OK;
}

__device__ __forceinline__ void cwfa_ln_coefs(const double* __restrict__ stats, int b, int64_t CHW, float eps, float& mean_f, float& rstd) {
    const double mean = stats[2 * b] / (double)CHW;
    double var = stats[2 * b + 1] / (double)CHW - mean * mean;
    if (var < 0.0) var = 0.0;
    rstd = (float)(1.0 / sqrt(var + (double)eps));
    mean_f = (float)mean;
}
__device__ __forceinline__ float cwfa_ln_apply(float x, float mean, float rstd, float w, float b) {
    const float v = (x - mean) * rstd;
    return v * w + b;
}

__global__ __launch_bounds__(256) void layernorm_apply_kernel(const float* __restrict__ x, const double* __restrict__ stats,
                                                              const float* __restrict__ w, const float* __restrict__ bsh,
                                                              float eps, float* __restrict__ y, int64_t CHW) {
    const int64_t i = (int64_t)blockIdx.x * blockDim.x + threadIdx.x;
    if (i >= CHW) return;
    const int b = blockIdx.y;
    float mean, rstd;
    cwfa_ln_coefs(stats, b, CHW, eps, mean, rstd);
    y[(int64_t)b * CHW + i] = cwfa_ln_apply(x[(int64_t)b * CHW + i], mean, rstd, w ? w[i] : 1.f, bsh ? bsh[i] : 0.f);
}

extern "C" int cwfa_layernorm_apply_f32(const float* x, const double* stats, const float* w, const float* b, float eps,
                                        float* y, int B, int64_t CHW, void* stream) {
    CWFA_REQUIRE(x && stats && y, CWFA_E_INVAL, "cwfa_layernorm_apply_f32: null pointer");
    CWFA_REQUIRE(B >= 0 && CHW >= 0 && B <= 65535, CWFA_E_SHAPE, "cwfa_layernorm_apply_f32: bad shape");
    if (B == 0 || CHW == 0) return CWFA_OK;
    hipLaunchKernelGGL(layernorm_apply_kernel, dim3((unsigned)((CHW + 255) / 256), B), dim3(256), 0, (hipStream_t)stream, x,
                       stats, w, b, eps, y, CHW);
    CWFA_LAUNCH_CHECK("cwfa_layernorm_apply_f32");
    return CWFA_OK;
}

struct TailParams {
    const float *v, *lw, *lb, *w1, *b1, *u, *gate, *x, *w0, *b0;
    const double* stats;
    float* y;
    float eps;
    int C, c_in, KP;
    int64_t HW, v_bs, u_bs, x_bs, y_bs, ntiles;
};

template <int MT, bool XRES>
__global__ __launch_bounds__(256, 4) void convnext_tail_kernel(TailParams p) {
    constexpr int KC = 8;
    constexpr unsigned OOB = 0x80000000u;
    __shared__ float Ws[MT * 32 * 65];
    __shared__ float Es[MT * 32 * 10];
    const int tid = threadIdx.x, lane = tid & 63, l31 = lane & 31, kh = lane >> 5;
    const int wave = __builtin_amdgcn_readfirstlane(tid >> 6);
    const int b = blockIdx.y, C = p.C, LS = p.KP + 1;
    const int plane = (int)(p.HW * 4);
    const int cbytes = C * plane;
    const auto rv = CWFA_RSRC(p.v + (int64_t)b * p.v_bs, cbytes);
    const auto rlw = CWFA_RSRC(p.lw, cbytes);
    const auto rlb = CWFA_RSRC(p.lb, cbytes);
    const auto ru = CWFA_RSRC(XRES ? p.v : p.u + (int64_t)b * p.u_bs, XRES ? 0 : cbytes);
    const auto rx = CWFA_RSRC(XRES ? p.x + (int64_t)b * p.x_bs : p.v, XRES ? p.c_in * plane : 0);
    const auto ry = CWFA_RSRC(p.y + (int64_t)b * p.y_bs, cbytes);
    auto ldf = [](decltype(rv) r, unsigned vo, int so) { return __builtin_bit_cast(float, __builtin_amdgcn_raw_buffer_load_b32(r, vo, so, 0)); };
    const int HW = (int)p.HW, ntiles = (int)p.ntiles, tstep = (int)gridDim.x * 4;
    float xa[KC], wa[KC], ba[KC], xb[KC], wb[KC], bb[KC];
    auto vo_of = [&](int tile) { const int px = tile * 32 + l31; return px < HW ? (unsigned)(px + kh * HW) * 4u : OOB; };
    auto load = [&](float (&xv)[KC], float (&wv)[KC], float (&bv)[KC], unsigned vo, int c) {
#pragma unroll
        for (int j = 0; j < KC; ++j) {
            const int so = (c * KC + j) * 2 * plane;
            xv[j] = ldf(rv, vo, so);
            wv[j] = ldf(rlw, vo, so);
            bv[j] = ldf(rlb, vo, so);
        }
    };
    int tile = (int)blockIdx.x * 4 + wave;
    unsigned vo = vo_of(tile);
    if (tile < ntiles) load(xa, wa, ba, vo, 0);
    CWFA_FENCE();

    for (int co = tid >> 6, ci = tid & 63; co < MT * 32; co += 4)
        if (ci < p.KP) Ws[co * LS + ci] = (co < C && ci < C) ? p.w1[co * C + ci] : 0.f;
    for (int e = tid; e < MT * 32 * 10; e += 256) {
        const int co = e / 10, j = e % 10;
        float val = 0.f;
        if (co < C) {
            if (j < 8) val = (XRES && j < p.c_in) ? p.w0[co * p.c_in + j] : 0.f;
            else if (j == 8) val = (XRES && p.b0) ? p.b0[co] : 0.f;
            else val = p.b1 ? p.b1[co] : 0.f;
        }
        Es[e] = val;
    }
    __syncthreads();

    float mean, rstd;
    cwfa_ln_coefs(p.stats, b, (int64_t)C * p.HW, p.eps, mean, rstd);
    const float gate = p.gate ? p.gate[b] : 1.f;
    const bool gated = p.gate != nullptr;
    const float* wl = Ws + l31 * LS + kh;
    const float* el = Es + 4 * kh * 10;
// ... 149 lines not shown
```

### cwfa_amd/ops.py

```python
import ctypes as C

import torch

from . import _lib
from ._lib import AffineStage, Chain, ConvOpts, check

__all__ = ["haar1d", "haar2d", "gather", "affine", "channel_affine", "chain_inv", "chain_inv_var", "chain_inv_roi_cov", "chain_inv_samples", "rand_uniform", "rand_trunc_normal", "chain_nll_map", "nll_compose", "chain_fwd", "pack_conv_weight",
           "conv2d", "conv2d_wgrad", "elu_bwd", "set_precision", "gelu_add", "gelu_bwd", "layernorm_bwd", "attention_bwd", "plane_affine", "bn_bwd_stats", "bn_act_bwd", "maxpool2_bwd", "chain_bwd", "chain_inv_bwd", "prelu_bwd", "conv3d_1k1_backward", "pack_1x1_panel", "pack_split_layer_weight", "subnet_layer", "conv3d_1k1", "channel_stats", "bn_fold", "bn_running_update", "maxpool", "sample_stats", "layernorm_apply",
           "convnext_tail", "conv_writes_sample_stats", "attention_combine", "scale_channels", "axpby", "stage", "lion_step", "global_extrema", "wmse_loss"]


def _stream():
    return C.c_void_p(torch.cuda.current_stream().cuda_stream)


def _p(t):
    return None if t is None else C.c_void_p(t.data_ptr())


def _dev(t, name="tensor"):
    if not torch.is_tensor(t):
        raise TypeError(f"{name}: expected a torch.Tensor, got {type(t)}")
    if not t.is_cuda:
        raise RuntimeError(f"{name}: cwfa_amd runs on MI355X only -- got a {t.device} tensor (no CPU fallback exists)")
# ... 409 lines not shown

def chain_fwd(x, stages, final_perm=None, logdet=None, sumsq=None, tables=None):
    L = _lib.lib()
    x, xbs = planes(x, "x")
    B, D, H, W = x.shape
    Cc = D // 2
    ch, keep = _chain(stages, tables)
    low = torch.empty((B, Cc, H, W), dtype=torch.float32, device=x.device)
    z = torch.empty((B, Cc, H, W), dtype=torch.float32, device=x.device)
    rec = chain_event_sink
    if rec is not None:
        e0, e1 = torch.cuda.Event(enable_timing=True), torch.cuda.Event(enable_timing=True)
        e0.record()
    check(L.cwfa_chain_fwd_f32(_p(x), _p(low), _p(z), C.byref(ch), _p(_idx(final_perm)), B, Cc, H, W, xbs, Cc * H * W,
                               Cc * H * W, _p(logdet), _p(sumsq), _stream()), "chain_fwd")
    if rec is not None:
        e1.record()
        rec.append(("fwd", B, Cc, H, W, len(stages), True, e0, e1))
    return z, low


chain_event_sink = None


def _chain_grads(grads, shape):
    B, Cc, H, W = shape
    gr = _lib.ChainGrads()
    for k, (ds, dt) in enumerate(grads):
        for name, t in (("ds", ds), ("dt", dt)):
            if t is None:
                continue
            t2, bs = planes(t, name)
            if t2.data_ptr() != t.data_ptr() or tuple(t.shape) != (B, Cc, H, W):
                raise ValueError(f"chain backward: {name}[{k}] must be a [B,C,H,W] view with contiguous planes")
            getattr(gr, name)[k] = t.data_ptr()
            getattr(gr, name + "_bs")[k] = bs
    return gr


def chain_inv_bwd(xhat, gt, stages, grads, gscale, loss_kind=2, accumulate=False, want_latent_grad=False, want_low_grad=False):
    L = _lib.lib()
    xhat, xbs = planes(xhat, "xhat")
    gt, gbs = planes(gt, "gt")
    if tuple(xhat.shape) != tuple(gt.shape):
        raise ValueError("chain_inv_bwd: xhat and gt differ in shape")
    B, D, H, W = xhat.shape
    Cc = D // 2
    ch, keep = _chain(stages)
    gr = _chain_grads(grads, (B, Cc, H, W))
    loss = torch.zeros(1, dtype=torch.float64, device=xhat.device)
    if want_low_grad and loss_kind != 0:
        raise ValueError("chain_inv_bwd: dL/dlow is formed from an upstream gradient (loss_kind 0)")
    gz = torch.empty((B, Cc, H, W), dtype=torch.float32, device=xhat.device) if want_latent_grad else None
    glow = torch.empty((B, Cc, H, W), dtype=torch.float32, device=xhat.device) if want_low_grad else None
    check(L.cwfa_chain_inv_bwd_f32(_p(xhat), _p(gt), C.byref(ch), C.byref(gr), B, Cc, H, W, xbs, gbs, float(gscale), int(loss_kind),
                                   int(bool(accumulate)), _p(loss), _p(gz), _p(glow), _stream()), "chain_inv_bwd")
    if want_latent_grad or want_low_grad:
        return loss, gz, glow
    return loss


def chain_bwd(z, stages, grads, final_perm=None, gscale=0.0, ldscale=0.0, gz=None, want_input_grad=False, accumulate=False, gld=None):
    L = _lib.lib()
    z, zbs = planes(z, "z")
    B, Cc, H, W = z.shape
    ch, keep = _chain(stages)
    gr = _chain_grads(grads, (B, Cc, H, W))
    gzbs = 0
    if gz is not None:
        gz, gzbs = planes(gz, "gz")
    gv0 = torch.empty((B, Cc, H, W), dtype=torch.float32, device=z.device) if want_input_grad else None
    if gld is not None:
        gld = _dev(gld, "gld").contiguous()
        if gld.numel() != B:
            raise ValueError("chain_bwd: gld must hold one value per sample")
    check(L.cwfa_chain_bwd_f32(_p(z), _p(gz), C.byref(ch), C.byref(gr), _p(_idx(final_perm)), _p(gv0), B, Cc, H, W, zbs, gzbs,
                               Cc * H * W, float(gscale), float(ldscale), int(bool(accumulate)), _p(gld), _stream()), "chain_bwd")
    return gv0


class PackedConv:
    __slots__ = ("packed", "cout", "cin", "ks", "transposed", "version", "src_ptr", "split", "epoch", "version1", "src_ptr1", "cat_c1",
                 "cat_from", "short", "walk")

    def __init__(self, packed, cout, cin, ks, transposed, version, src_ptr, split=False):
        self.packed, self.cout, self.cin, self.ks = packed, cout, cin, ks
        self.transposed, self.version, self.src_ptr = transposed, version, src_ptr
        self.split = split
        self.epoch = _pack_epoch
        self.walk = None


def pack_conv_weight(w, transposed=False, direct=False):
    pc = _pack_conv_weight(w, transposed, direct)
    if not direct and out_walk_bank(pc.cout, pc.cin, pc.ks, transposed):
        L = _lib.lib()
        wc = _dev(w, "weight").detach().contiguous()
        pc.walk = torch.empty(L.cwfa_conv3x3_out_split_packed_bytes(pc.cout), dtype=torch.uint8, device=wc.device)
        check(L.cwfa_conv3x3_out_split_pack_f32(_p(wc), _p(pc.walk), pc.cout, _stream()), "conv3x3_out_split_pack")
    return pc


def _pack_conv_weight(w, transposed, direct):
    L = _lib.lib()
    w = _dev(w, "weight").detach().contiguous()
    if transposed:
        cin, co, kh, kw = w.shape
        if (kh, kw) != (2, 2):
            raise ValueError("only 2x2 stride-2 transposed convolutions are supported")
        cout, ks = 4 * co, 1
    else:
        cout, cin, ks, kw = w.shape
        if ks != kw:
            raise ValueError("square kernels only")
    if direct:
        pass
    elif _split_bf16 and ks == 1 and cout >= 128:
        packed = torch.empty(L.cwfa_conv_split_packed_bytes(cout, cin, ks), dtype=torch.uint8, device=w.device)
        check(L.cwfa_conv_split_pack_f32(_p(w), _p(packed), cout, cin, ks, int(transposed), _stream()), "conv_split_pack")
        return PackedConv(packed, cout, cin, ks, transposed, w._version, w.data_ptr(), split=True)
    narrow_max = 32 if single_product() else SPLIT_3X3_NARROW_MAX
    if not direct and _split_bf16 >= 2 and ks == 3 and cout >= SPLIT_3X3_MIN_COUT and (cout > 32 or (cout <= narrow_max and cin >= 29)):
        packed = torch.empty(L.cwfa_conv3x3_split_packed_bytes(cout, cin), dtype=torch.uint8, device=w.device)
        check(L.cwfa_conv3x3_split_pack_f32(_p(w), _p(packed), cout, cin, _stream()), "conv3x3_split_pack")
        return PackedConv(packed, cout, cin, ks, transposed, w._version, w.data_ptr(), split=True)
    if not direct and SPLIT_7X7 and _split_bf16 >= 2 and ks == 7 and cout <= 64 and cin >= 32:
        packed = torch.empty(L.cwfa_conv7x7_split_packed_bytes(cout, cin), dtype=torch.uint8, device=w.device)
        check(L.cwfa_conv7x7_split_pack_f32(_p(w), _p(packed), cout, cin, _stream()), "conv7x7_split_pack")
        return PackedConv(packed, cout, cin, ks, transposed, w._version, w.data_ptr(), split=True)
    n = L.cwfa_conv2d_packed_floats(cout, cin, ks)
    if n <= 0:
        raise ValueError(f"unsupported filter bank {tuple(w.shape)}")
    packed = torch.empty(n, dtype=torch.float32, device=w.device)
    check(L.cwfa_conv2d_pack_f32(_p(w), _p(packed), cout, cin, ks, int(transposed), _stream()), "conv2d_pack")
    return PackedConv(packed, cout, cin, ks, transposed, w._version, w.data_ptr())


def pack_conv_weight_cat(w, c1):
    w = _dev(w, "weight").detach()
    cout, cin, ks, kw = w.shape
    if ks != 1 or kw != 1 or cout > 64 or not (0 < c1 < cin):
        raise ValueError(f"pack_conv_weight_cat: a 1x1 bank with <= 64 outputs and 0 < c1 < Cin is needed, got {tuple(w.shape)}, c1 = {c1}")
    start = (c1 + 15) // 16 * 16
    wz = torch.zeros((cout, start + cin - c1, 1, 1), dtype=torch.float32, device=w.device)
    wz[:, :c1] = w[:, :c1]
    wz[:, start:] = w[:, c1:]
    pc = pack_conv_weight(wz)
    pc.version, pc.src_ptr = w._version, w.data_ptr()
    pc.cat_c1, pc.cat_from = c1, start
    return pc


def conv_writes_stats(pc, act=None, residual=None, act2=None, out_blocked=False, in_add=False):
    return bool(pc.split and pc.ks == 3 and act in (None, "prelu") and residual is None and act2 is None and not out_blocked
                and not (in_add and act is None))


def conv_writes_sample_stats(pc):
    return bool(pc.split and pc.ks == 7 and pc.cin <= 8)


def conv2d(x, pc, bias=None, act=None, prelu_alpha=None, residual=None, act2=None, in_scale=None, in_shift=None,
           in_add=None, out=None, in_blocked=False, out_blocked=False, cat=None, out_stats=None, out_sample_stats=None):
    L = _lib.lib()
    x, xbs = planes(x, "x")
    B, Cin, H, W = x.shape
    o = ConvOpts()
    keep = [x]
    walk = out_walk_selected(pc, H, W, act=act, prelu_alpha=prelu_alpha, residual=residual, act2=act2, in_scale=in_scale, in_add=in_add,
                             out_blocked=out_blocked, cat=cat, out_stats=out_stats, out_sample_stats=out_sample_stats)
    if cat is not None:
        cat, cbs = planes(cat, "cat")
        c1 = getattr(pc, "cat_c1", None)
        if c1 is None or Cin != c1 or tuple(cat.shape) != (B, pc.cin - pc.cat_from, H, W) or in_scale is not None or in_add is not None:
            raise ValueError("conv2d: `cat` needs a bank from pack_conv_weight_cat for exactly these two inputs, and no load-side prologue")
        o.in_cat, o.in_cat_bs, o.in_cat_from, o.in_cat_c1 = cat.data_ptr(), cbs, pc.cat_from, c1
        keep.append(cat)
        Cin = pc.cin
    if Cin != pc.cin:
        raise ValueError(f"conv2d: input has {Cin} channels, filter bank expects {pc.cin}")
    up = bool(pc.transposed)
    oshape = (B, pc.cout // 4, 2 * H, 2 * W) if up else (B, pc.cout, H, W)
    if out is None:
        out = torch.empty(oshape, dtype=torch.float32, device=x.device)
        ybs = oshape[1] * oshape[2] * oshape[3]
    else:
        if tuple(out.shape) != oshape:
            raise ValueError(f"conv2d: out has shape {tuple(out.shape)}, expected {oshape}")
        out_c, ybs = planes(out, "out")
        if out_c.data_ptr() != out.data_ptr():
            raise ValueError("conv2d: `out` must have contiguous planes")
    if bias is not None:
        o.bias = _dev(bias, "bias").data_ptr()
    o.act, o.act2 = _lib.ACT[act], _lib.ACT[act2]
    if prelu_alpha is not None:
        prelu_alpha = _dev(prelu_alpha, "prelu_alpha")
        o.prelu_alpha = prelu_alpha.data_ptr()
        if prelu_alpha.numel() != 1:
            if prelu_alpha.numel() != pc.cout or not prelu_alpha.is_contiguous() or not (pc.split and pc.ks == 3):
                raise ValueError("conv2d: per-channel PReLU slopes need [Cout] contiguous values and the split-bf16 3x3 kernel")
            o.prelu_per_channel = 1
    elif "prelu" in (act, act2):
        raise ValueError("conv2d: PReLU needs prelu_alpha")
    if residual is not None:
        residual, rbs = planes(residual, "residual")
        if tuple(residual.shape) != oshape:
            raise ValueError(f"conv2d: residual {tuple(residual.shape)} != output {oshape}")
        o.residual, o.res_bs = residual.data_ptr(), rbs
        keep.append(residual)
    if in_scale is not None:
        o.in_scale, o.in_shift = _dev(in_scale).data_ptr(), _dev(in_shift).data_ptr()
        if in_scale.numel() not in (Cin, B * Cin) or in_shift.numel() != in_scale.numel():
            raise ValueError("conv2d: in_scale / in_shift must be [Cin] or [B,Cin]")
        o.in_affine_bs = Cin if (in_scale.numel() == B * Cin and B > 1) else 0
    if in_add is not None:
        in_add, abs_ = planes(in_add, "in_add")
        if tuple(in_add.shape) != tuple(x.shape):
            raise ValueError("conv2d: in_add shape mismatch")
        o.in_add, o.in_add_bs = in_add.data_ptr(), abs_
        keep.append(in_add)
    o.upshuffle2 = int(up)
    if in_blocked:
        if not (walk or (pc.split and pc.ks == 3)):
            raise ValueError("conv2d: channel-blocked input is read by the split-bf16 3x3 kernels only")
        o.in_blocked8 = 1
    if out_blocked:
        ok3 = (pc.split and pc.ks == 3 and pc.cout % 8 == 0 and residual is None and act2 is None and act in (None, "prelu")
               and not split3x3_narrow(pc.cout) and not (in_add is not None and act is None))
        ok1 = not pc.split and pc.ks == 1 and pc.cout >= 33 and pc.cout % 8 == 0 and not up
        if not (ok3 or ok1):
            raise ValueError("conv2d: channel-blocked output is written by the split-bf16 3x3 kernel (bias / PReLU) and by the "
                             "direct 1x1 kernel with 40..64 output channels only")
        o.out_blocked8 = 1
    if out_stats is not None:
        if not conv_writes_stats(pc, act, residual, act2, out_blocked, in_add is not None):
            raise ValueError("conv2d: out_stats needs the split-bf16 3x3 kernel with an NCHW output and a bias / PReLU epilogue")
        if out_stats.dtype != torch.float64 or out_stats.numel() != 2 * pc.cout or not out_stats.is_cuda:
            raise ValueError("conv2d: out_stats must be a float64 [2*Cout] tensor on the HIP device")
        o.out_stats = out_stats.data_ptr()
    if out_sample_stats is not None:
        if not conv_writes_sample_stats(pc):
            raise ValueError("conv2d: out_sample_stats needs the few-channel split 7x7 kernel (a composed ConvNeXt bank with <= 8 inputs)")
        if out_sample_stats.dtype != torch.float64 or out_sample_stats.numel() != 2 * B or not out_sample_stats.is_cuda:
            raise ValueError("conv2d: out_sample_stats must be a float64 [2*B] tensor on the HIP device")
        o.out_sample_stats = out_sample_stats.data_ptr()
    rec = conv_event_sink
    if rec is not None:
        key = (pc.ks, Cin, pc.cout, H, W, B, "%s|%s|%s|%s|%s" % ("pro" if (in_scale is not None or in_add is not None) else "",
                                                                 act or "", "res" if residual is not None else "", act2 or "",
                                                                 ("up" if up else "") + ("+split" if pc.split else "")),
               in_add is not None)
        if rec.want(key):
            e0, e1 = torch.cuda.Event(enable_timing=True), torch.cuda.Event(enable_timing=True)
            e0.record()
    if walk:
        check(L.cwfa_conv3x3_out_split_f32(_p(x), _p(pc.walk), _p(bias), _p(out), B, H, W, pc.cout, xbs, ybs, int(bool(in_blocked)),
                                           _stream()), "conv3x3_out_split")
    elif pc.split and pc.ks == 7:
        if act or act2 or residual is not None or in_scale is not None or in_add is not None:
            raise ValueError("conv2d: the split-bf16 7x7 kernel has a bias-only epilogue and no load-side prologue")
        check(L.cwfa_conv7x7_split_f32(_p(x), _p(pc.packed), _p(out), B, Cin, H, W, pc.cout, xbs, ybs, C.byref(o), _stream()),
              "conv7x7_split")
    elif pc.split and pc.ks == 3:
        if split3x3_narrow(pc.cout) and (in_scale is not None or in_add is not None):
            if (H * W) % 4 == 0:
                x = plane_affine(x, in_scale, in_shift, add=in_add)
            else:
                if in_scale is not None:
                    if in_scale.numel() == Cin:
                        x = channel_affine(x, in_scale.reshape(-1), in_shift.reshape(-1))
                    else:
                        x = torch.cat([channel_affine(x[i:i + 1], in_scale.reshape(B, Cin)[i].contiguous(), in_shift.reshape(B, Cin)[i].contiguous())
                                       for i in range(B)], 0)
                if in_add is not None:
                    x = axpby(x.contiguous(), 1.0, in_add, 1.0)
            x, xbs = planes(x, "x")
            o.in_scale = o.in_shift = o.in_add = None
        check(L.cwfa_conv3x3_split_f32(_p(x), _p(pc.packed), _p(out), B, Cin, H, W, pc.cout, xbs, ybs, C.byref(o),
                                       _stream()), "conv3x3_split")
    elif pc.split:
        ws = torch.empty(L.cwfa_split_workspace_bytes(B, Cin, H * W), dtype=torch.uint8, device=x.device)
        per_sample = in_scale is not None and in_scale.numel() == B * Cin and B > 1
        check(L.cwfa_split_input_f32(_p(x), _p(ws), B, Cin, H * W, xbs, _p(in_scale), _p(in_shift), Cin if per_sample else 0,
                                     _p(in_add), in_add.stride(0) if in_add is not None else 0, _stream()), "split_input")
        o.in_scale = o.in_shift = o.in_add = None
        check(L.cwfa_conv_split_f32(_p(ws), _p(pc.packed), _p(out), B, Cin, H, W, pc.cout, pc.ks, ybs, C.byref(o), _stream()),
              "conv_split")
    else:
        check(L.cwfa_conv2d_f32(_p(x), _p(pc.packed), _p(out), B, Cin, H, W, pc.cout, pc.ks, xbs, ybs, C.byref(o),
                                _stream()), "conv2d")
    if rec is not None and rec.want(key):
        e1.record()
        rec.add(key, e0, e1)
    return out


def pack_couple_weight(w, bias):
    L = _lib.lib()
    w = _dev(w, "weight").detach()
    n2, cin, ks, kw = w.shape
    if ks != 3 or kw != 3 or n2 % 2 or n2 // 2 > 64:
        raise ValueError(f"pack_couple_weight: a [2n,Cin,3,3] bank with n <= 64 is needed, got {tuple(w.shape)}")
    n = n2 // 2
    total = L.cwfa_couple_rows(n, None)
    rows_c = (C.c_int * total)()
    L.cwfa_couple_rows(n, rows_c)
    rows = torch.tensor(list(rows_c), dtype=torch.int64, device=w.device)
    live = (rows >= 0)
    wr = torch.zeros((total, cin, 3, 3), dtype=torch.float32, device=w.device)
    wr[live] = w[rows[live]]
    br = torch.zeros(total, dtype=torch.float32, device=w.device)
    if bias is not None:
        br[live] = _dev(bias, "bias").detach()[rows[live]]
    packed = torch.empty(L.cwfa_conv3x3_split_packed_bytes(total, cin), dtype=torch.uint8, device=w.device)
    check(L.cwfa_conv3x3_split_pack_f32(_p(wr), _p(packed), total, cin, _stream()), "conv3x3_split_pack (coupling bank)")
    pc = PackedConv(packed, n2, cin, 3, False, w._version, w.data_ptr(), split=True)
    pc.version1, pc.src_ptr1 = (bias._version, bias.data_ptr()) if bias is not None else (None, None)
    return pc, br


def conv3x3_couple(u, pc_bias, x, out, clamp_kind, clamp, pre_scale, rev, logdet=None, in_blocked=False):
    L = _lib.lib()
    pc, br = pc_bias
    u, ubs = planes(u, "u")
    B, Cin, H, W = u.shape
    n = pc.cout // 2
    if Cin != pc.cin:
        raise ValueError(f"conv3x3_couple: input has {Cin} channels, filter bank expects {pc.cin}")
    x2, xbs = planes(x, "x")
    o2, obs = planes(out, "out")
    if tuple(x.shape) != (B, n, H, W) or tuple(out.shape) != (B, n, H, W) or o2.data_ptr() != out.data_ptr():
        raise ValueError("conv3x3_couple: x / out must be [B,n,H,W] views with contiguous planes")
    cp = _lib.Couple()
    cp.x, cp.y, cp.x_bs, cp.y_bs, cp.n = x2.data_ptr(), out.data_ptr(), xbs, obs, n
    cp.clamp_kind, cp.clamp, cp.pre_scale, cp.rev = _lib.CLAMP[clamp_kind], float(clamp), float(pre_scale), int(bool(rev))
    if logdet is not None:
        cp.logdet = logdet.data_ptr()
    cp.in_blocked8 = int(bool(in_blocked))
    rec = conv_event_sink
    if rec is not None:
        key = (3, Cin, pc.cout, H, W, B, "||||couple+split", False)
        if rec.want(key):
            e0, e1 = torch.cuda.Event(enable_timing=True), torch.cuda.Event(enable_timing=True)
            e0.record()
    check(L.cwfa_conv3x3_split_couple_f32(_p(u), _p(pc.packed), _p(br), B, Cin, H, W, ubs, C.byref(cp), _stream()),
          "conv3x3_split_couple")
    if rec is not None and rec.want(key):
        e1.record()
        rec.add(key, e0, e1)
    return out


BLOCKED_MAPS = True
SPLIT_7X7 = True
VIRTUAL_CAT = True
COUPLE_EPILOGUE = True


def couple_fused():
    return COUPLE_EPILOGUE and _split_bf16 >= 2


def split3x3_narrow(cout):
    return cout <= 48 or 64 < cout <= 96


SPLIT_3X3_MIN_COUT = 1
SPLIT_3X3_NARROW_MAX = 16
OUT_WALK = True
OUT_WALK_MT = (1, 2, 3)


def out_walk_bank(cout, cin, ks, transposed=False):
    return bool(OUT_WALK and _split_bf16 >= 2 and ks == 3 and not transposed and cin == 64 and 1 <= cout <= 48
                and (cout + 15) // 16 in OUT_WALK_MT)


def out_walk_selected(pc, H, W, act=None, prelu_alpha=None, residual=None, act2=None, in_scale=None, in_add=None, out_blocked=False,
                      cat=None, out_stats=None, out_sample_stats=None):
    return bool(OUT_WALK and getattr(pc, "walk", None) is not None and act is None and prelu_alpha is None
                and residual is None and act2 is None and in_scale is None and in_add is None and not out_blocked and cat is None
                and out_stats is None and out_sample_stats is None and 64 * H * W * 4 < 2 ** 31)


conv_event_sink = None


def pack_1x1_panel(w):
    L = _lib.lib()
    w = _dev(w, "weight").detach().contiguous()
    if tuple(w.shape) != (64, 64, 1, 1):
        raise ValueError("pack_1x1_panel: the fused layer kernel is specialised for 64 channels")
    panel = torch.empty(4096, dtype=torch.float32, device=w.device)
    check(L.cwfa_subnet_pack1x1_f32(_p(w), _p(panel), _stream()), "subnet_pack1x1")
    return PackedConv(panel, 64, 64, 1, False, w._version, w.data_ptr())


def pack_split_layer_weight(w3, w1):
    L = _lib.lib()
    w3 = _dev(w3, "weight").detach().contiguous()
    w1 = _dev(w1, "weight").detach().contiguous()
    if tuple(w3.shape) != (64, 64, 3, 3) or tuple(w1.shape) != (64, 64, 1, 1):
        raise ValueError("pack_split_layer_weight: 64x64x3x3 and 64x64x1x1 only")
    packed = torch.empty(L.cwfa_subnet_layer_split_packed_bytes(), dtype=torch.uint8, device=w3.device)
    check(L.cwfa_subnet_layer_split_pack_f32(_p(w3), _p(w1), _p(packed), _stream()), "subnet_layer_split_pack")
    pc = PackedConv(packed, 64, 64, 3, False, w3._version, w3.data_ptr(), split=True)
    pc.version1, pc.src_ptr1 = w1._version, w1.data_ptr()
    return pc


FIRST_LAYER_COMPOSED = True
FIRST_LAYER_FUSED_X = True


def pack_first_layer_weight(w0, b0, w3, w1, short=None):
    L = _lib.lib()
    w0, w3, w1 = _dev(w0, "w0").detach(), _dev(w3, "w3").detach(), _dev(w1, "w1").detach().contiguous()
    cin = w0.shape[1]
    if tuple(w0.shape) != (64, cin, 1, 1) or cin > 31 or tuple(w3.shape) != (64, 64, 3, 3) or tuple(w1.shape) != (64, 64, 1, 1):
        raise ValueError("pack_first_layer_weight: 64-channel layers with a 1x1 bank of <= 31 inputs in front only")
    w0p = torch.cat([w0.reshape(64, cin).double(), (b0.detach().double() if b0 is not None else torch.zeros(64, dtype=torch.float64, device=w0.device)).reshape(64, 1)], 1)
    wc = torch.einsum("omt,mi->oit", w3.double().reshape(64, 64, 9), w0p)
    w3c = torch.zeros((64, 32, 3, 3), dtype=torch.float32, device=w0.device)
    w3c[:, :cin + 1] = wc.reshape(64, cin + 1, 3, 3).to(torch.float32)
    w0c = torch.zeros((64, 32), dtype=torch.float32, device=w0.device)
    w0c[:, :cin + 1] = w0p.to(torch.float32)
    packed = torch.empty(L.cwfa_subnet_layer_first_packed_bytes(), dtype=torch.uint8, device=w0.device)
    short = (FIRST_LAYER_FUSED_X and cin + 1 <= 16) if short is None else bool(short)
    if short and cin + 1 > 16:
        raise ValueError("pack_first_layer_weight: the short form needs cin + 1 <= 16")
    check(L.cwfa_subnet_layer_first_pack_f32(_p(w3c), _p(w1), _p(w0c), int(short), _p(packed), _stream()), "subnet_layer_first_pack")
    pc = PackedConv(packed, 64, cin + 1, 3, False, w3._version, w3.data_ptr(), split=True)
    pc.short = short
    pc.version1, pc.src_ptr1 = w1._version, w1.data_ptr()
    return pc


CONVNEXT_COMPOSED = True


def convnext_composed(c_in, c_out, biases=True):
    return bool(CONVNEXT_COMPOSED and SPLIT_7X7 and _split_bf16 >= 2 and c_in + 1 <= 16 and c_out <= 64 and biases)


def pack_convnext_composed(w0, b0, w7):
    L = _lib.lib()
    w0, b0, w7 = _dev(w0, "w0").detach(), _dev(b0, "b0").detach(), _dev(w7, "w7").detach()
    c, cin = w0.shape[0], w0.shape[1]
    cout = w7.shape[0]
    if tuple(w0.shape) != (c, cin, 1, 1) or cin + 1 > 16 or tuple(w7.shape) != (cout, c, 7, 7) or cout > 64 or tuple(b0.shape) != (c,):
        raise ValueError("pack_convnext_composed: a 1x1 bank with <= 15 inputs and a bias in front of a 7x7 bank with <= 64 outputs only")
    w0p = torch.cat([w0.reshape(c, cin).double(), b0.double().reshape(c, 1)], 1)
    wc = torch.einsum("omt,mi->oit", w7.double().reshape(cout, c, 49), w0p)
    cpad = 8 if cin + 1 <= 8 else 16
    w7c = torch.zeros((cout, cpad, 7, 7), dtype=torch.float32, device=w0.device)
    w7c[:, :cin + 1] = wc.reshape(cout, cin + 1, 7, 7).to(torch.float32)
    packed = torch.empty(L.cwfa_conv7x7_split_packed_bytes(cout, cpad), dtype=torch.uint8, device=w0.device)
    check(L.cwfa_conv7x7_split_pack_f32(_p(w7c), _p(packed), cout, cpad, _stream()), "conv7x7_split_pack (composed bank)")
    return PackedConv(packed, cout, cin + 1, 7, False, w7._version, w7.data_ptr(), split=True)


def subnet_layer_first(u1, x, pc, b3, b1, layout=0):
    L = _lib.lib()
    u1, ubs = planes(u1, "u1")
    B, Cu, H, W = u1.shape
    xbs = 0
    if x is not None:
        x, xbs = planes(x, "x")
    if (x is not None and tuple(x.shape) != (B, 64, H, W)) or Cu != pc.cin:
        raise ValueError(f"subnet_layer_first: u1 {tuple(u1.shape)} / x {None if x is None else tuple(x.shape)} do not match the composed "
                         f"bank ({pc.cin} inputs)")
    short = bool(getattr(pc, "short", False))
    if short and x is not None:
        raise ValueError("subnet_layer_first: a short-form image (pack_first_layer_weight(short=True)) forms its first map itself: x must be None")
    out = torch.empty((B, 64, H, W), dtype=torch.float32, device=u1.device)
    rec = conv_event_sink
    if rec is not None:
        key = ("L", 16 if short else 32, 64, H, W, B, "layer1+split" if x is not None else "layer1x+split", False)
        if rec.want(key):
            e0, e1 = torch.cuda.Event(enable_timing=True), torch.cuda.Event(enable_timing=True)
            e0.record()
    check(L.cwfa_subnet_layer_first_f32(_p(u1), _p(x), _p(pc.packed), _p(_dev(b3)), _p(_dev(b1)), _p(out), B, Cu, H, W, ubs, xbs,
                                        64 * H * W, int(layout) | (4 if short else 0), _stream()), "subnet_layer_first")
    if rec is not None and rec.want(key):
        e1.record()
        rec.add(key, e0, e1)
    return out


_ones_scope = None
_first_maps = None


class first_map_scope:

    def __init__(self, maps):
        self.maps = maps

    def __enter__(self):
        global _first_maps
        self.prev, _first_maps = _first_maps, self.maps
        return self

    def __exit__(self, *exc):
        global _first_maps
        _first_maps = self.prev
        return False


def first_map_of(net):
    return None if _first_maps is None else _first_maps.get(id(net))


class ones_channel_scope:

    def __enter__(self):
        global _ones_scope
# ... 203 lines not shown

def gelu_bwd(g, p):
    L = _lib.lib()
    p, g = _dev(p, "p").contiguous(), _dev(g, "g").contiguous()
    if tuple(g.shape) != tuple(p.shape):
        raise ValueError("gelu_bwd: g and p differ in shape")
    out = torch.empty_like(p)
    check(L.cwfa_gelu_f32(_p(p), _p(g), _p(out), p.numel(), 1, _stream()), "gelu_bwd")
    return out


def layernorm_bwd(g, v, weight, mean, invstd, dw, db):
    L = _lib.lib()
    g, v = _dev(g, "g").contiguous(), _dev(v, "v").contiguous()
    B, n = v.shape[0], v[0].numel()
    if tuple(g.shape) != tuple(v.shape) or weight.numel() != n or mean.numel() != B or invstd.numel() != B or dw.numel() != n or db.numel() != n:
        raise ValueError("layernorm_bwd: operand shapes do not match")
    st = torch.zeros(2 * B, dtype=torch.float64, device=v.device)
    gv = torch.empty_like(v)
    check(L.cwfa_layernorm_bwd_f32(_p(g), _p(v), _p(_dev(weight).contiguous()), _p(_dev(mean).contiguous()), _p(_dev(invstd).contiguous()),
                                   _p(st), _p(gv), _p(dw), _p(db), B, n, _stream()), "layernorm_bwd")
    return gv


def attention_bwd(mean, w1, b1, w2, b2, m, g):
    L = _lib.lib()
    mean, m, g = _dev(mean).contiguous(), _dev(m).contiguous(), _dev(g).contiguous()
    if tuple(m.shape) != tuple(mean.shape) or tuple(g.shape) != tuple(mean.shape):
        raise ValueError("attention_bwd: mean, m and g differ in shape")
    B, Cc = mean.shape[:2]
    HW = mean[0, 0].numel()
    gm = torch.empty_like(m)
    pg = torch.zeros(Cc * Cc * 3 + Cc + Cc * Cc + Cc, dtype=torch.float64, device=mean.device)
    check(L.cwfa_attention_bwd_f32(_p(mean), _p(_dev(w1).contiguous()), _p(_dev(b1)), _p(_dev(w2).contiguous()), _p(_dev(b2)), _p(m),
                                   _p(g), _p(gm), _p(pg), B, Cc, HW, _stream()), "attention_bwd")
    return gm, pg


def prelu_bwd(g, o, alpha, dalpha=None, out=None):
    L = _lib.lib()
    g, gbs = planes(g, "g")
    o, obs = planes(o, "o")
    if tuple(o.shape) != tuple(g.shape):
        raise ValueError("prelu_bwd: g and o differ in shape")
    B, n = g.shape[0], g[0].numel()
    if out is None:
        out = torch.empty(tuple(g.shape), dtype=torch.float32, device=g.device)
    o2, ybs = planes(out, "out")
    if o2.data_ptr() != out.data_ptr():
        raise ValueError("prelu_bwd: `out` must have contiguous planes")
    check(L.cwfa_prelu_bwd_f32(_p(g), _p(o), _p(_dev(alpha)), _p(out), _p(dalpha), B, n, gbs, obs, ybs, _stream()), "prelu_bwd")
    return out


def conv3d_1k1_backward(x, dy, w1, b1, alpha, w2, want_input_grad=True):
    L = _lib.lib()
    x = _dev(x, "x").contiguous()
    dy = _dev(dy, "dy").contiguous()
    B, D, H, W = x.shape
    K = w1.shape[0]
    w1c, w2c = _dev(w1).detach().contiguous(), _dev(w2).detach().contiguous()
    st = _stream()
    q = torch.empty((B, K, D, H, W), dtype=torch.float32, device=x.device)
    m = torch.empty_like(q)
    dalpha = torch.zeros(1, dtype=torch.float64, device=x.device)
    ws = torch.empty(L.cwfa_conv3d_wgrad_workspace_bytes(B, D, H, W), dtype=torch.uint8, device=x.device)
    g2 = torch.empty(32, 32, dtype=torch.float32, device=x.device)
    g1 = torch.empty(32, 32, dtype=torch.float32, device=x.device)
    check(L.cwfa_conv3d_hidden_fwd_f32(_p(x), _p(w1c), _p(_dev(b1)), _p(q), B, D, H, W, K, st), "conv3d_hidden_fwd")
    check(L.cwfa_conv3d_wgrad_f32(_p(q), _p(dy), _p(_dev(alpha)), _p(g2), _p(ws), B, D, H, W, K, -1, 0, 0.0, st), "conv3d_wgrad")
    check(L.cwfa_conv3d_hidden_bwd_f32(_p(dy), _p(w2c), _p(q), _p(_dev(alpha)), _p(m), _p(dalpha), B, D, H, W, K, st), "conv3d_hidden_bwd")
    check(L.cwfa_conv3d_wgrad_f32(_p(m), _p(x), None, _p(g1), _p(ws), B, D, H, W, K, 1, 1, 0.0, st), "conv3d_wgrad")
    dx = None
    if want_input_grad:
        dx = torch.empty_like(x)
        check(L.cwfa_conv3d_input_bwd_f32(_p(m), _p(w1c), _p(dx), B, D, H, W, K, st), "conv3d_input_bwd")
    dW1 = g1[:K, :27].reshape(K, 1, 3, 3, 3).contiguous()
    db1 = g1[:K, 27].contiguous()
    dW2 = g2[:K, :27].reshape(1, K, 3, 3, 3).contiguous()
    db2 = sample_stats(dy.reshape(1, -1, 1, 1))[0:1].to(torch.float32)
    return dx, dW1, db1, dW2, db2, dalpha


SPLIT_CONV3D = True


def conv3d_1k1(x, w1, b1, alpha, w2, b2):
    L = _lib.lib()
    x = _dev(x, "x").contiguous()
    B, D, H, W = x.shape
    K = w1.shape[0]
    out = torch.empty_like(x)
    if SPLIT_CONV3D and _split_bf16 >= 2 and K <= 32 and (D + 4) * H * W * 4 < 2 ** 31:
        check(L.cwfa_conv3d_1k1_split_f32(_p(x), _p(_dev(w1).contiguous()), _p(_dev(b1)), _p(_dev(alpha)), _p(_dev(w2).contiguous()),
                                          _p(_dev(b2)), _p(out), B, D, H, W, K, _stream()), "conv3d_1k1_split")
        return out
    check(L.cwfa_conv3d_1k1_f32(_p(x), _p(_dev(w1).contiguous()), _p(_dev(b1)), _p(_dev(alpha)), _p(_dev(w2).contiguous()),
                                _p(_dev(b2)), _p(out), B, D, H, W, K, _stream()), "conv3d_1k1")
    return out


def channel_stats(x, out=None):
    L = _lib.lib()
    x, xbs = planes(x, "x")
    B, Cc, H, W = x.shape
    st = out if out is not None else torch.zeros(2 * Cc, dtype=torch.float64, device=x.device)
    check(L.cwfa_channel_stats_f32(_p(x), _p(st), B, Cc, H * W, xbs, _stream()), "channel_stats")
    return st


def bn_running_update(stats, count, momentum, running_mean, running_var, num_batches_tracked=None):
    L = _lib.lib()
    check(L.cwfa_bn_running_update_f32(_p(stats), float(count), float(momentum), _p(_dev(running_mean)), _p(_dev(running_var)),
                                       _p(num_batches_tracked), running_mean.numel(), _stream()), "bn_running_update")


def bn_fold(C_, weight=None, bias=None, eps=1e-5, stats=None, count=0.0, running_mean=None, running_var=None,
            mask_bc=None):
    L = _lib.lib()
    ref = next(t for t in (weight, stats, running_mean, mask_bc) if t is not None)
    B = 0
    n = C_
    if mask_bc is not None:
        mask_bc = _dev(mask_bc, "mask").contiguous()
        B = mask_bc.numel() // C_
        n = B * C_
    scale = torch.empty(n, dtype=torch.float32, device=ref.device)
    shift = torch.empty(n, dtype=torch.float32, device=ref.device)
    check(L.cwfa_bn_fold_f32(_p(stats), float(count), _p(running_mean), _p(running_var), _p(weight), _p(bias),
                             float(eps), _p(mask_bc), B, _p(scale), _p(shift), C_, _stream()), "bn_fold")
    return scale, shift


def bn_finish(C_, weight=None, bias=None, eps=1e-5, stats=None, count=0.0, running_mean=None, running_var=None, momentum=None,
              num_batches_tracked=None, mask_bc=None, mask_u=None, drop_p=0.0, zero_stats=False):
    L = _lib.lib()
    ref = next(t for t in (weight, stats, running_mean, mask_bc, mask_u) if t is not None)
    B, n = 0, C_
    mk = mask_bc if mask_bc is not None else mask_u
    if mk is not None:
        mk = _dev(mk, "mask").contiguous()
        B = mk.numel() // C_
        n = B * C_
    scale = torch.empty(n, dtype=torch.float32, device=ref.device)
    shift = torch.empty(n, dtype=torch.float32, device=ref.device)
    upd = momentum is not None and stats is not None and running_mean is not None
    check(L.cwfa_bn_finish_f32(_p(stats), float(count), _p(running_mean), _p(running_var), _p(num_batches_tracked),
                               float(momentum or 0.0), int(upd), _p(weight), _p(bias), float(eps), _p(mk if mask_bc is not None else None),
                               _p(mk if mask_u is not None else None), float(drop_p), float(1.0 - drop_p), B, _p(scale), _p(shift), C_,
                               int(bool(zero_stats)), _stream()), "bn_finish")
    return scale, shift


def maxpool(x, Ho, Wo, scale=None, shift=None, want_full=False):
    L = _lib.lib()
    x = _dev(x, "x").contiguous()
    B, Cc, H, W = x.shape
    for t in (scale, shift):
        if t is not None and t.numel() != Cc:
            raise ValueError("maxpool: the load-side affine must be a [C] table")
    y = torch.empty((B, Cc, Ho, Wo), dtype=x.dtype, device=x.device)
    full = torch.empty_like(x) if want_full else None
    check(L.cwfa_maxpool_f32(_p(x), _p(y), _p(full), _p(scale), _p(shift), B, Cc, H, W, Ho, Wo, _stream()), "maxpool")
    return (y, full) if want_full else y


def sample_stats(x):
    L = _lib.lib()
    x = _dev(x, "x").contiguous()
    B = x.shape[0]
    st = torch.zeros(2 * B, dtype=torch.float64, device=x.device)
    check(L.cwfa_sample_stats_f32(_p(x), _p(st), B, x[0].numel(), _stream()), "sample_stats")
    return st


def layernorm_apply(x, stats, weight, bias, eps):
    L = _lib.lib()
    x = _dev(x, "x").contiguous()
    if stats.numel() != 2 * x.shape[0] or weight.numel() != x[0].numel() or bias.numel() != x[0].numel():
        raise ValueError("layernorm_apply: statistics / affine do not match x")
    out = torch.empty_like(x)
    check(L.cwfa_layernorm_apply_f32(_p(x), _p(stats), _p(weight), _p(bias), float(eps), _p(out), x.shape[0],
                                     x[0].numel(), _stream()), "layernorm_apply")
    return out


CONVNEXT_TAIL_FUSED = True
CONVNEXT_RESIDUAL_FUSED = True


def convnext_tail(v, stats, ln_weight, ln_bias, eps, w1, b1, u=None, gate=None, x=None, w0=None, b0=None, out=None):
    L = _lib.lib()
    v, vbs = planes(v, "v")
    B, Cc, H, W = v.shape
    HW = H * W
    if stats.dtype != torch.float64 or stats.numel() != 2 * B or not stats.is_cuda:
        raise ValueError("convnext_tail: stats must be a float64 [2*B] tensor on the HIP device")
    ln_weight, ln_bias = _dev(ln_weight, "ln_weight").contiguous(), _dev(ln_bias, "ln_bias").contiguous()
    w1 = _dev(w1, "w1").detach().contiguous()
    if Cc > 64 or ln_weight.numel() != Cc * HW or ln_bias.numel() != Cc * HW or w1.numel() != Cc * Cc:
        raise ValueError("convnext_tail: C <= 64, LayerNorm tables of C*H*W values and a [C,C,1,1] bank are needed")
    if b1 is not None and _dev(b1, "b1").numel() != Cc:
        raise ValueError("convnext_tail: b1 must hold C values")
    if (u is None) == (x is None):
        raise ValueError("convnext_tail: pass the residual u, or the block input x it is formed from")
    ubs = xbs = cin = 0
    if u is not None:
        u, ubs = planes(u, "u")
        if tuple(u.shape) != (B, Cc, H, W):
            raise ValueError(f"convnext_tail: residual {tuple(u.shape)} != {(B, Cc, H, W)}")
    else:
        x, xbs = planes(x, "x")
        cin = x.shape[1]
        w0 = _dev(w0, "w0").detach().contiguous()
        if tuple(x.shape) != (B, cin, H, W) or cin > 8 or w0.numel() != Cc * cin or (b0 is not None and _dev(b0, "b0").numel() != Cc):
            raise ValueError("convnext_tail: x [B,c_in <= 8,H,W] with w0 [C,c_in,1,1] and b0 [C] is needed")
    if gate is not None:
        gate = _dev(gate, "gate").reshape(-1).contiguous()
        if gate.numel() != B:
            raise ValueError("convnext_tail: gate must hold one factor per sample")
    if out is None:
        out = torch.empty((B, Cc, H, W), dtype=torch.float32, device=v.device)
        ybs = Cc * HW
    else:
        out_c, ybs = planes(out, "out")
        if tuple(out.shape) != (B, Cc, H, W) or out_c.data_ptr() != out.data_ptr():
            raise ValueError("convnext_tail: `out` must be [B,C,H,W] with contiguous planes")
    check(L.cwfa_convnext_tail_f32(_p(v), _p(stats), _p(ln_weight), _p(ln_bias), float(eps), _p(w1), _p(b1), _p(u), _p(gate), _p(x),
                                   _p(w0), _p(b0), cin, _p(out), B, Cc, HW, vbs, ubs, xbs, ybs, _stream()), "convnext_tail")
    return out


def attention_combine(mean, w1, b1, w2, b2, m=None, x=None):
    L = _lib.lib()
    mean = _dev(mean, "mean").contiguous()
    B, Cc = mean.shape[:2]
    HW = mean[0, 0].numel()
    out = torch.empty_like(mean)
    m = None if m is None else _dev(m).contiguous()
    x = None if x is None else _dev(x).contiguous()
    for t in (m, x):
        if t is not None and tuple(t.shape) != tuple(mean.shape):
            raise ValueError("attention_combine: mean, m and x must share one shape")
    if w1.numel() != Cc * Cc * 3 or b1.numel() != Cc or w2.numel() != Cc * Cc or b2.numel() != Cc:
        raise ValueError("attention_combine: the Conv1d banks do not match the channel count")
    check(L.cwfa_attention_combine_f32(_p(mean), _p(_dev(w1).contiguous()), _p(_dev(b1)), _p(_dev(w2).contiguous()),
                                       _p(_dev(b2)), _p(m), _p(x), _p(out), B, Cc, HW, _stream()), "attention_combine")
    return out


def scale_channels(x, scale_bc):
    L = _lib.lib()
    x = _dev(x, "x").contiguous()
    B, Cc = x.shape[:2]
    if scale_bc.numel() != B * Cc:
        raise ValueError(f"scale_channels: the table must hold B*C = {B * Cc} factors")
    out = torch.empty_like(x)
    check(L.cwfa_scale_channels_f32(_p(x), _p(_dev(scale_bc).contiguous()), _p(out), B, Cc, x[0, 0].numel(), _stream()),
          "scale_channels")
    return out


def axpby(x, a, z=None, b=0.0):
    L = _lib.lib()
    x = _dev(x, "x").contiguous()
    z = None if z is None else _dev(z).contiguous()
    if z is not None and z.numel() != x.numel():
        raise ValueError("axpby: x and z differ in size")
    out = torch.empty_like(x)
    check(L.cwfa_axpby_f32(_p(x), _p(z), float(a), float(b), _p(out), x.numel(), _stream()), "axpby")
    return out


def extract_views(image, coords_yx, subimage_shape, mean=0.0, std=1.0):
    L = _lib.lib()
    image = _dev(image, "image")
    if image.dim() != 4 or image.shape[1] != 1:
        raise ValueError(f"extract_views: image must be [B,1,H,W], got {tuple(image.shape)}")
    if image.dtype != torch.float32:
        raise TypeError("extract_views: fp32 images only")
    image = image if image[0].is_contiguous() else image.contiguous()
    B, _, Hs, Ws = image.shape
    co = torch.as_tensor(coords_yx, dtype=torch.int32).reshape(-1, 2)
    sh, sw = int(subimage_shape[0]), int(subimage_shape[1])
    ys, xs = co[:, 0], co[:, 1]
    if len(co) and (bool(((torch.minimum(ys + sh // 2, torch.tensor(Hs)) - torch.clamp(ys - sh // 2, min=0)) <= 0).any()) or
                    bool(((torch.minimum(xs + sw // 2, torch.tensor(Ws)) - torch.clamp(xs - sw // 2, min=0)) <= 0).any())):
        raise ValueError("extract_views: a lenslet window lies outside the image")
    cod = co.contiguous().to(image.device)
    out = torch.empty((B, len(co), sh, sw), dtype=torch.float32, device=image.device)
    check(L.cwfa_extract_views_f32(_p(image), _p(cod), _p(out), B, Hs, Ws, len(co), sh, sw, float(mean), float(std),
                                   image.stride(0), _stream()), "extract_views")
    return out


_split_bf16 = 0
_precision = "fp32"
_pack_epoch = 0


def single_product():
    return _precision in ("bf16", "fp16")


def pack_epoch():
    return _pack_epoch


def invalidate_packs():
    global _pack_epoch
# ... 456 lines not shown
```

### cwfa_amd/unet.py

```python
import torch
from torch import nn

from . import ops
from .amp import amp_entry

__all__ = ["UNet", "UNetConvBlock", "UNetUpBlock"]


_MATERIALIZE_UP = False
_MATERIALIZE = True


class _Packed:

    def __init__(self):
        self._c = {}

    def get(self, conv, transposed=False):
        w = conv.weight
        pc = self._c.get(id(conv))
        if pc is None or pc.version != w._version or pc.src_ptr != w.data_ptr() or pc.epoch != ops.pack_epoch():
            pc = self._c[id(conv)] = ops.pack_conv_weight(w, transposed=transposed)
        return pc


class _Drop:
    __slots__ = ("u", "p")

    def __init__(self, u, p):
        self.u, self.p = u, p

    def mask(self):
        return ((self.u >= self.p).to(torch.float32) / (1.0 - self.p)).contiguous()


STATS_IN_EPILOGUE = True


def _bn_batch_stats(bn):
    return bn.training or not bn.track_running_stats


def _bn_stats_buffer(bn, device):
    key = (str(device), torch.cuda.current_stream(device).cuda_stream)
    bufs = bn.__dict__.setdefault("_cwfa_stats", {})
    st = bufs.get(key)
    if st is None or getattr(bn, "_cwfa_stats_dirty", False):
        st = bufs[key] = torch.zeros(2 * bn.num_features, dtype=torch.float64, device=device)
    bn._cwfa_stats_dirty = True
    return st


def _bn_affine(bn, y, drop=None, stats=None):
    C = bn.num_features
    mu, mb, p = (drop.u, None, drop.p) if isinstance(drop, _Drop) else (None, drop, 0.0)
    if _bn_batch_stats(bn):
        st = stats
        if st is None:
            st = _bn_stats_buffer(bn, y.device)
            ops.channel_stats(y, out=st)
        n = y.numel() // C
        track = bn.track_running_stats and bn.momentum is not None
        out = ops.bn_finish(C, bn.weight, bn.bias, bn.eps, stats=st, count=float(n), running_mean=bn.running_mean if track else None,
                            running_var=bn.running_var if track else None, momentum=bn.momentum if track else None,
                            num_batches_tracked=bn.num_batches_tracked if track else None, mask_bc=mb, mask_u=mu, drop_p=p,
                            zero_stats=True)
        bn._cwfa_stats_dirty = False
        return out
    return ops.bn_finish(C, bn.weight, bn.bias, bn.eps, running_mean=bn.running_mean, running_var=bn.running_var, mask_bc=mb,
                         mask_u=mu, drop_p=p)


def _drop_mask(p, B, C, device):
    if not p:
        return None
    return _Drop(torch.rand(B, C, device=device), p).mask()


def _drop(p, B, C, device, pool=None):
    if not p:
        return None
    return _Drop(pool.take(B, C) if pool is not None else torch.rand(B, C, device=device), p)


class _DrawPool:

    def __init__(self, n, device):
        self.u = torch.rand(n, device=device) if n > 0 else None
        self.pos = 0

    def take(self, B, C):
        out = self.u[self.pos:self.pos + B * C].view(B, C)
        self.pos += B * C
        return out


def _drop_affine(C, drop):
    if isinstance(drop, _Drop):
        return ops.bn_finish(C, mask_u=drop.u, drop_p=drop.p)
    return ops.bn_finish(C, mask_bc=drop)


class UNetConvBlock(nn.Module):

    def __init__(self, in_size, out_size, padding, batch_norm, kernel_size=3, use_bias=False, stride=1,
                 activation=nn.LeakyReLU):
        super().__init__()
        if stride != 1 or kernel_size != 3 or not padding:
            raise NotImplementedError("cwfa_amd UNetConvBlock: 3x3, stride 1, padded convolutions only")
        block = [nn.Conv2d(in_size, out_size, kernel_size=kernel_size, stride=stride, padding=int(padding), bias=use_bias),
                 activation()]
        if batch_norm:
            block.append(nn.BatchNorm2d(out_size))
        block += [nn.Conv2d(out_size, out_size, kernel_size=kernel_size, stride=1, padding=int(padding), bias=use_bias),
                  activation()]
        if batch_norm:
            block.append(nn.BatchNorm2d(out_size))
        self.block = nn.Sequential(*block)
        self.batch_norm = batch_norm
        self._packed = _Packed()

    def _layers(self):
        mods = list(self.block)
        step = 3 if self.batch_norm else 2
        return [(mods[i], mods[i + 1], mods[i + 2] if self.batch_norm else None) for i in (0, step)]

    @staticmethod
    def _act(a):
        if isinstance(a, nn.PReLU):
            if a.weight.numel() != 1:
                raise NotImplementedError("per-channel PReLU")
            return "prelu", a.weight
        if isinstance(a, nn.ELU):
            return "elu", None
        if isinstance(a, nn.ReLU):
            return "relu", None
        raise NotImplementedError(f"activation {type(a).__name__} has no HIP epilogue")

    def run(self, x, in_affine=None, in_add=None, out_mask=None):
        aff = in_affine
        layers = self._layers()
        packs = [self._packed.get(conv) for conv, _, _ in layers]
        for li, (conv, act, bn) in enumerate(layers):
            kind, alpha = self._act(act)
            sc, sh = aff if aff is not None else (None, None)
            add = in_add if li == 0 else None
            if (_MATERIALIZE and ops._split_bf16 < 2 and (sc is not None or add is not None)
                    and (x.shape[2] * x.shape[3]) % 4 == 0):
                x = ops.plane_affine(x, sc, sh, add=add)
                sc = sh = add = None
            st = None
            if (STATS_IN_EPILOGUE and bn is not None and _bn_batch_stats(bn)
                    and ops.conv_writes_stats(packs[li], kind, in_add=add is not None)):
                st = _bn_stats_buffer(bn, x.device)
            x = ops.conv2d(x, packs[li], bias=conv.bias, act=kind, prelu_alpha=alpha, in_scale=sc,
                           in_shift=sh, in_add=add, out_stats=st)
            last = li == len(layers) - 1
            m = out_mask if last else None
            if bn is not None:
                aff = _bn_affine(bn, x, m, stats=st)
            elif m is not None:
                aff = _drop_affine(x.shape[1], m)
            else:
                aff = None
        return x, aff

    @amp_entry
    def forward(self, x):
        y, aff = self.run(x)
        if aff is None:
            return y
        return ops.channel_affine(y, aff[0], aff[1])


class UNetUpBlock(nn.Module):

    def __init__(self, in_size, out_size, up_mode, padding, batch_norm, use_bias=False, skip_conn=True,
                 activation=nn.Softplus):
        super().__init__()
        self.skip_conn = skip_conn
        if up_mode != 'upconv':
            raise NotImplementedError("cwfa_amd UNetUpBlock: up_mode='upconv' only (what the LRNN uses, networks.py:532)")
        self.up = nn.ConvTranspose2d(in_size, out_size, kernel_size=2, stride=2, bias=use_bias)
        in_size = out_size if not skip_conn else in_size // 2
        self.conv_block = UNetConvBlock(in_size, out_size, padding, batch_norm, use_bias=use_bias, activation=activation)
        self._packed = _Packed()

    @staticmethod
    def center_crop(layer, target_size):
        _, _, h, w = layer.size()
        dy, dx = (h - target_size[0]) // 2, (w - target_size[1]) // 2
        return layer[:, :, dy:(dy + target_size[0]), dx:(dx + target_size[1])]

    def run(self, x, bridge, in_affine=None, out_mask=None):
        sc, sh = in_affine if in_affine is not None else (None, None)
        if _MATERIALIZE_UP and ops._split_bf16 < 1 and sc is not None and (x.shape[2] * x.shape[3]) % 4 == 0:
            x = ops.plane_affine(x, sc, sh)
            sc = sh = None
        up = ops.conv2d(x, self._packed.get(self.up, transposed=True), bias=self.up.bias, in_scale=sc, in_shift=sh)
        add = self.center_crop(bridge, up.shape[2:]) if self.skip_conn else None
        return self.conv_block.run(up, in_add=add, out_mask=out_mask)

    @amp_entry
    def forward(self, x, bridge):
        y, aff = self.run(x, bridge)
        return y if aff is None else ops.channel_affine(y, aff[0], aff[1])


class UNet(nn.Module):

    def __init__(self, in_channels=1, n_classes=2, depth=5, wf=6, padding=True, batch_norm=True, up_mode='upsample',
                 drop_out=0, use_bias=False, skip_conn=False, activation=nn.PReLU):
        super().__init__()
        assert up_mode in ('upconv', 'upsample')
        self.padding, self.depth, self.skip_conn, self.drop_out = padding, depth, skip_conn, drop_out
        prev = in_channels
        self.down_path = nn.ModuleList()
        for i in range(depth):
            self.down_path.append(UNetConvBlock(prev, 2 ** (wf + i), padding, batch_norm, use_bias=use_bias,
                                                activation=activation))
            prev = 2 ** (wf + i)
        self.up_path = nn.ModuleList()
        for i in reversed(range(depth - 1)):
            self.up_path.append(UNetUpBlock(prev, 2 ** (wf + i), up_mode, padding, batch_norm, use_bias=use_bias,
                                            skip_conn=skip_conn, activation=activation))
            prev = 2 ** (wf + i)
        self.last = nn.Sequential(nn.Conv2d(prev, n_classes, kernel_size=1, bias=use_bias), activation())
        self._packed = _Packed()

    @amp_entry
    def forward(self, x, store_activations=False, in_affine=None):
        if store_activations:
            raise NotImplementedError("store_activations is a debugging aid of the reference, not on the hot path")
        B, dev = x.shape[0], x.device
        skips, aff = [], in_affine
        n_draw = 0
        if self.drop_out:
            n_draw = B * (sum(d.block[0].out_channels for d in list(self.down_path)[:-1]) +
                          sum(u.conv_block.block[0].out_channels for u in self.up_path))
        pool = _DrawPool(n_draw, dev)
        for i, down in enumerate(self.down_path):
            x, aff = down.run(x, in_affine=aff)
            if i != len(self.down_path) - 1:
                sc, sh = aff if aff is not None else (None, None)
                x, full = ops.maxpool(x, x.shape[-1] // 2, x.shape[-1] // 2, sc, sh, want_full=True)
                skips.append(full)
                m = _drop(self.drop_out, B, x.shape[1], dev, pool)
                aff = _drop_affine(x.shape[1], m) if m is not None else None
        for i, up in enumerate(self.up_path):
            m = _drop(self.drop_out, B, up.conv_block.block[0].out_channels, dev, pool)
            x, aff = up.run(x, skips[-i - 1], in_affine=aff, out_mask=m)
        kind, alpha = UNetConvBlock._act(self.last[1])
        sc, sh = aff if aff is not None else (None, None)
        return ops.conv2d(x, self._packed.get(self.last[0]), bias=self.last[0].bias, act=kind, prelu_alpha=alpha,
                          in_scale=sc, in_shift=sh)
```

### include/cwfa_hip.h

```cpp
#ifndef CWFA_HIP_H
#define CWFA_HIP_H

#include <stdint.h>

#ifdef __cplusplus
extern "C" {
#endif

#define CWFA_VERSION 100

enum {
    CWFA_OK = 0,
    CWFA_E_INVAL = -1,
    CWFA_E_SHAPE = -2,
    CWFA_E_ALIGN = -3,
    CWFA_E_HIP = -4
};

enum { CWFA_CLAMP_NONE = 0, CWFA_CLAMP_ATAN = 1, CWFA_CLAMP_TANH = 2, CWFA_CLAMP_SIGMOID = 3 };

enum { CWFA_ACT_NONE = 0, CWFA_ACT_ELU = 1, CWFA_ACT_PRELU = 2, CWFA_ACT_GELU = 3, CWFA_ACT_RELU = 4 };

int cwfa_version(void);
const char* cwfa_last_error(void);
int cwfa_set_option(const char* name, int value);


int cwfa_haar1d_fwd_f32(const float* x, float* lo, float* hi, int B, int D, int64_t HW,
                        int64_t x_bs, int64_t lo_bs, int64_t hi_bs, void* stream);

int cwfa_haar1d_inv_f32(const float* lo, const float* hi, float* x, int B, int D, int64_t HW,
                        int64_t lo_bs, int64_t hi_bs, int64_t x_bs, void* stream);

int cwfa_haar2d_fwd_f32(const float* x, float* y, int B, int C, int H, int W, int order_by_wavelet, float fac,
                        void* stream);
int cwfa_haar2d_inv_f32(const float* y, float* x, int B, int C, int H, int W, int order_by_wavelet, float fac,
                        void* stream);

int cwfa_haar3d_fwd_f32(const float* x, float* y, int B, int D, int H, int W, int order_by_wavelet, float fac, int64_t x_bs,
                        void* stream);
int cwfa_haar3d_inv_f32(const float* y, float* x, int B, int D, int H, int W, int order_by_wavelet, float fac, int64_t x_bs,
                        void* stream);


int cwfa_gather_f32(const float* x, const int64_t* perm, float* y, int B, int C, int H, int W, int axis,
                    int64_t x_bs, int64_t y_bs, void* stream);


typedef struct {
    const float* s_raw;
    const float* t;
    int64_t s_bs, t_bs;
    int clamp_kind;
    float clamp;
    float pre_scale;
    int t_neg_div_sqrt2;
    const int64_t* perm;
    int perm_axis;
    int gin;
} cwfa_affine_stage;

int cwfa_affine_f32(const float* x, float* y, const cwfa_affine_stage* st, int rev, int B, int C, int H, int W,
                    int64_t x_bs, int64_t y_bs, double* logdet, double* sumsq, void* stream);

int cwfa_channel_affine_f32(const float* x, float* y, const float* scale, const float* shift, int mode,
                            const int64_t* perm_in, const int64_t* perm_out, int B, int C, int64_t HW,
                            int64_t x_bs, int64_t y_bs, void* stream);

#define CWFA_CHAIN_MAX 8

typedef struct {
    int n_stages;
    cwfa_affine_stage stage[CWFA_CHAIN_MAX];
    const int32_t* src_c;
    const int32_t* src_h;
} cwfa_chain;

int cwfa_chain_inv_f32(const float* z, const float* low, float* x, const cwfa_chain* ch, int B, int C, int H, int W,
                       int64_t z_bs, int64_t low_bs, int64_t x_bs, double* logdet, void* stream);

int cwfa_chain_inv_var_f32(const float* var_low, float* out, const cwfa_chain* ch, float z_var, float std_scale,
                           int B, int C, int H, int W, int64_t var_low_bs, int64_t out_bs, void* stream);

int cwfa_chain_inv_roi_cov_f32(double* out, const cwfa_chain* ch, float z_var, int B, int C, int H, int W, int level,
                               const int32_t* boxes, int R, const int32_t* pairs, int P, const int32_t* dev_table, int64_t out_bs,
                               void* stream);

int cwfa_rand_uniform_f32(float* out, int N, int64_t n, int64_t out_ss, uint64_t seed, uint32_t stream_id, uint32_t sample_offset,
                          void* stream);
int cwfa_rand_trunc_normal_f32(float* out, int N, int64_t n, int64_t out_ss, float temperature, uint64_t seed, uint32_t stream_id,
                               uint32_t sample_offset, void* stream);

int cwfa_chain_inv_samples_f32(const float* low, float* x, float* z_out, const cwfa_chain* ch, int N, int B, int C, int H, int W,
                               int64_t low_ss, int64_t low_bs, int64_t x_ss, int64_t x_bs, int64_t z_ss, int64_t z_bs,
                               float temperature, uint64_t seed, uint32_t stream_id, uint32_t sample_offset, void* stream);

int cwfa_chain_nll_map_f32(const float* x, float* low, float* z, float* nll, const cwfa_chain* ch, int B, int C, int H, int W,
                           int64_t x_bs, int64_t low_bs, int64_t z_bs, int64_t nll_bs, double* nll_sum, void* stream);

#define CWFA_NLL_MAX_LEVELS 8
typedef struct {
    int n;
    const float* level[CWFA_NLL_MAX_LEVELS];
    int64_t bs[CWFA_NLL_MAX_LEVELS];
} cwfa_nll_levels;
int cwfa_nll_compose_f32(const cwfa_nll_levels* levels, float* out, int B, int D, int64_t HW, int64_t out_bs, void* stream);

int cwfa_chain_fwd_f32(const float* x, float* low, float* z, const cwfa_chain* ch, const int64_t* final_perm,
                       int B, int C, int H, int W, int64_t x_bs, int64_t low_bs, int64_t z_bs,
                       double* logdet, double* sumsq, void* stream);


int64_t cwfa_conv2d_packed_floats(int Cout, int Cin, int ks);
int cwfa_conv2d_pack_f32(const float* w, float* packed, int Cout, int Cin, int ks, int transposed, void* stream);

typedef struct {
    const float* bias;
    int act;
    const float* prelu_alpha;
    const float* residual;
    int64_t res_bs;
    int act2;
    const float* in_scale;
    const float* in_shift;
    int in_affine_bs;
    const float* in_add;
    int64_t in_add_bs;
    int upshuffle2;
    int in_blocked8;
    int out_blocked8;
    const float* in_cat;
    int64_t in_cat_bs;
    int in_cat_from, in_cat_c1;
    double* out_stats;
    int prelu_per_channel;
    double* out_sample_stats;
} cwfa_conv_opts;

int cwfa_conv2d_f32(const float* x, const float* w_packed, float* y, int B, int Cin, int H, int W, int Cout, int ks,
                    int64_t x_bs, int64_t y_bs, const cwfa_conv_opts* opts, void* stream);

int cwfa_subnet_pack1x1_f32(const float* w, float* panel, void* stream);
int cwfa_subnet_layer_f32(const float* x, const float* w3_packed, const float* b3, const float* w1_panel, const float* b1,
                          float* y, int B, int H, int W, int64_t x_bs, int64_t y_bs, void* stream);
int cwfa_subnet_layer_tape_f32(const float* x, const float* w3_packed, const float* b3, const float* w1_panel, const float* b1,
                               float* y, float* hidden, int B, int H, int W, int64_t x_bs, int64_t y_bs, int64_t hidden_bs,
                               void* stream);

int cwfa_conv3d_1k1_f32(const float* x, const float* w1, const float* b1, const float* alpha, const float* w2,
                        const float* b2, float* y, int B, int D, int H, int W, int K, void* stream);
int cwfa_conv3d_1k1_split_f32(const float* x, const float* w1, const float* b1, const float* alpha, const float* w2,
                              const float* b2, float* y, int B, int D, int H, int W, int K, void* stream);


int cwfa_channel_stats_f32(const float* x, double* stats, int B, int C, int64_t HW, int64_t x_bs, void* stream);
int cwfa_bn_fold_f32(const double* stats, double count, const float* running_mean, const float* running_var,
                     const float* weight, const float* bias, float eps, const float* mask_bc, int B, float* scale,
                     float* shift, int C, void* stream);
int cwfa_bn_finish_f32(double* stats, double count, float* running_mean, float* running_var, long long* num_batches_tracked,
                       float momentum, int update_running, const float* weight, const float* bias, float eps, const float* mask_bc,
                       const float* mask_u, float drop_p, float keep_scale, int B, float* scale, float* shift, int C, int zero_stats,
                       void* stream);
int cwfa_bn_running_update_f32(const double* stats, double count, float momentum, float* running_mean, float* running_var,
                               long long* num_batches_tracked, int C, void* stream);
int cwfa_maxpool_f32(const float* x, float* y, float* full, const float* scale, const float* shift, int B, int C,
                     int H, int W, int Ho, int Wo, void* stream);
int cwfa_sample_stats_f32(const float* x, double* stats, int B, int64_t CHW, void* stream);
int cwfa_layernorm_apply_f32(const float* x, const double* stats, const float* w, const float* b, float eps,
                             float* y, int B, int64_t CHW, void* stream);
int cwfa_convnext_tail_f32(const float* v, const double* stats, const float* lw, const float* lb, float eps,
                           const float* w1, const float* b1, const float* u, const float* gate, const float* x,
                           const float* w0, const float* b0, int c_in, float* y, int B, int C, int64_t HW,
                           int64_t v_bs, int64_t u_bs, int64_t x_bs, int64_t y_bs, void* stream);
int cwfa_attention_combine_f32(const float* mean, const float* w1, const float* b1, const float* w2, const float* b2,
                               const float* m, const float* x, float* out, int B, int C, int64_t HW, void* stream);
int cwfa_scale_channels_f32(const float* x, const float* scale_bc, float* y, int B, int C, int64_t HW, void* stream);
int cwfa_axpby_f32(const float* x, const float* z, float a, float b, float* y, int64_t n, void* stream);

int64_t cwfa_split_workspace_bytes(int B, int Cin, int64_t HW);
int cwfa_split_input_f32(const float* x, void* ws, int B, int Cin, int64_t HW, int64_t x_bs, const float* in_scale,
                         const float* in_shift, int64_t in_affine_bs, const float* in_add, int64_t in_add_bs, void* stream);
int64_t cwfa_conv_split_packed_bytes(int Cout, int Cin, int ks);
int cwfa_conv_split_pack_f32(const float* w, void* packed, int Cout, int Cin, int ks, int transposed, void* stream);
int64_t cwfa_conv3x3_split_packed_bytes(int Cout, int Cin);
int cwfa_conv3x3_split_pack_f32(const float* w, void* packed, int Cout, int Cin, void* stream);
int cwfa_conv3x3_split_f32(const float* x, const void* w_packed, float* y, int B, int Cin, int H, int W, int Cout,
                           int64_t x_bs, int64_t y_bs, const cwfa_conv_opts* opts, void* stream);
int cwfa_conv_split_f32(const void* ws, const void* w_packed, float* y, int B, int Cin, int H, int W, int Cout, int ks, int64_t y_bs,
                           const cwfa_conv_opts* opts, void* stream);
int64_t cwfa_conv7x7_split_packed_bytes(int Cout, int Cin);
int cwfa_conv7x7_split_pack_f32(const float* w, void* packed, int Cout, int Cin, void* stream);
int cwfa_conv7x7_split_f32(const float* x, const void* w_packed, float* y, int B, int Cin, int H, int W, int Cout,
                           int64_t x_bs, int64_t y_bs, const cwfa_conv_opts* opts, void* stream);

typedef struct {
    const float* x;
    float* y;
    int64_t x_bs, y_bs;
    int n;
    int clamp_kind;
    float clamp, pre_scale;
    int rev;
    double* logdet;
    int in_blocked8;
} cwfa_couple;
int cwfa_couple_rows(int n, int* rows);
int cwfa_conv3x3_split_couple_f32(const float* x, const void* w_packed, const float* bias_rows, int B, int Cin, int H, int W,
                                  int64_t x_bs, const cwfa_couple* cp, void* stream);

int64_t cwfa_subnet_layer_split_packed_bytes(void);
int cwfa_subnet_layer_split_pack_f32(const float* w3, const float* w1, void* packed, void* stream);
int cwfa_subnet_layer_split_f32(const float* x, const void* packed, const float* b3, const float* b1, float* y, int B, int H,
                                int W, int64_t x_bs, int64_t y_bs, int layout, void* stream);
int64_t cwfa_subnet_layer_first_packed_bytes(void);
int cwfa_subnet_layer_first_pack_f32(const float* w3c, const float* w1, const float* w0c, int short_form, void* packed, void* stream);
int cwfa_subnet_layer_first_f32(const float* u, const float* x, const void* packed, const float* b3, const float* b1, float* y, int B,
                                int u_ch, int H, int W, int64_t u_bs, int64_t x_bs, int64_t y_bs, int layout, void* stream);
int cwfa_subnet_layer_split_tape_f32(const float* x, const void* packed, const float* b3, const float* b1, float* y, float* hid, int B,
                                     int H, int W, int64_t x_bs, int64_t y_bs, int64_t hid_bs, void* stream);
int64_t cwfa_conv3x3_out_split_packed_bytes(int Cout);
int cwfa_conv3x3_out_split_pack_f32(const float* w, void* packed, int Cout, void* stream);
int cwfa_conv3x3_out_split_f32(const float* x, const void* packed, const float* bias, float* y, int B, int H, int W, int Cout,
                               int64_t x_bs, int64_t y_bs, int in_blocked, void* stream);

int cwfa_extract_views_f32(const float* image, const int* coords_yx, float* views, int B, int Hs, int Ws, int nviews, int sh,
                           int sw, float mean, float stdv, int64_t image_bs, void* stream);


typedef struct {
    float* ds[CWFA_CHAIN_MAX];
    float* dt[CWFA_CHAIN_MAX];
    int64_t ds_bs[CWFA_CHAIN_MAX], dt_bs[CWFA_CHAIN_MAX];
} cwfa_chain_grads;

int cwfa_chain_bwd_f32(const float* z, const float* gz, const cwfa_chain* ch, const cwfa_chain_grads* grads,
                       const int64_t* final_perm, float* gv0, int B, int C, int H, int W, int64_t z_bs, int64_t gz_bs,
                       int64_t gv0_bs, float gscale, float ldscale, int accumulate, const float* gld, void* stream);

int cwfa_chain_inv_bwd_f32(const float* xhat, const float* gt, const cwfa_chain* ch, const cwfa_chain_grads* grads, int B, int C,
                           int H, int W, int64_t xhat_bs, int64_t gt_bs, float gscale, int loss_kind, int accumulate,
                           double* loss_sum, float* gz_out, float* glow_out, void* stream);

int cwfa_affine_bwd_f32(const float* x, const float* g, const cwfa_affine_stage* st, int rev, int B, int C, int H, int W,
                        int64_t x_bs, int64_t g_bs, const float* gld, float* gx, float* gs_raw, float* gt_raw, void* stream);

int64_t cwfa_conv2d_wgrad_workspace_bytes(int B, int Cin, int H, int W, int Cout, int ks);
int cwfa_conv2d_wgrad_f32(const float* x, const float* dy, float* dw, float* db, void* workspace, int B, int Cin, int H, int W,
                          int Cout, int ks, int64_t x_bs, int64_t dy_bs, float beta, void* stream);

int cwfa_elu_bwd_f32(const float* g, const float* a, const float* add, float* y, int B, int64_t n, int64_t g_bs, int64_t a_bs,
                     int64_t add_bs, int64_t y_bs, void* stream);

int cwfa_conv3d_hidden_fwd_f32(const float* x, const float* w1, const float* b1, float* q, int B, int D, int H, int W, int K,
                               void* stream);
int cwfa_conv3d_hidden_bwd_f32(const float* dy, const float* w2, const float* q, const float* alpha, float* m, double* dalpha,
                               int B, int D, int H, int W, int K, void* stream);
int cwfa_conv3d_input_bwd_f32(const float* m, const float* w1, float* dx, int B, int D, int H, int W, int K, void* stream);
int64_t cwfa_conv3d_wgrad_workspace_bytes(int B, int D, int H, int W);
int cwfa_conv3d_wgrad_f32(const float* a, const float* src, const float* alpha, float* out32, void* workspace, int B, int D, int H,
                          int W, int K, int sign, int want_bias, float beta, void* stream);

int cwfa_prelu_bwd_f32(const float* g, const float* o, const float* alpha, float* y, double* dalpha, int B, int64_t n, int64_t g_bs,
                       int64_t o_bs, int64_t y_bs, void* stream);

int cwfa_plane_affine_f32(const float* x, const float* scale, const float* shift, int per_sample, const float* add, float* y, int B,
                          int C, int64_t HW, int64_t x_bs, int64_t add_bs, int64_t y_bs, void* stream);
int cwfa_bn_bwd_stats_f32(const float* g, const float* y, const float* mask_bc, double* stats, int B, int C, int64_t HW, int64_t g_bs,
                          int64_t y_bs, void* stream);
int cwfa_bn_act_bwd_f32(const float* g, const float* y, const float* A, int per_sample, const float* Bc, const float* Cc,
                        const float* alpha, float* out, double* dalpha, int B, int C, int64_t HW, int64_t g_bs, int64_t y_bs,
                        int64_t out_bs, void* stream);
int cwfa_maxpool2_bwd_f32(const float* full, const float* g_pool, const float* g_skip, float* g_full, int B, int C, int H, int W,
                          void* stream);

int cwfa_gelu_f32(const float* p, const float* other, float* y, int64_t n, int mode, void* stream);
int cwfa_layernorm_bwd_f32(const float* g, const float* v, const float* w, const float* mean, const float* invstd, double* stats,
                           float* gv, float* dw, float* db, int B, int64_t n, void* stream);
int cwfa_attention_bwd_f32(const float* mean, const float* w1, const float* b1, const float* w2, const float* b2, const float* m,
                           const float* g, float* gm, double* pgrad, int B, int C, int64_t HW, void* stream);

#define CWFA_EXTREMA_STRIDE 12
#define CWFA_EVAL_MAX_SPLITS 2048
#define CWFA_SELECT_WORKSPACE_BYTES 8448
typedef struct {
    int enabled;
    float scale, std, mean;
} cwfa_eval_affine;
typedef struct {
    int normalize, threshold;
    float norm_sub, norm_div, vol_min, lower, upper, clamp_value;
} cwfa_eval_post;
int64_t cwfa_eval_splits(int B, int64_t n);
int cwfa_volume_extrema_f32(const float* a, const float* b, float* out, float* workspace, int B, int64_t n, int64_t a_bs,
                            int64_t b_bs, const cwfa_eval_affine* affine, void* stream);
int cwfa_volume_metrics_f32(const float* pred, const float* gt, double* out, double* workspace, int B, int64_t n, int64_t pred_bs,
                            int64_t gt_bs, const cwfa_eval_affine* affine, float pred_offset, float gt_offset, float thr,
                            void* stream);
int cwfa_mip3_f32(const float* a, const float* b, float* zproj, float* xproj, float* yproj, float* gmin, int B, int D, int H, int W,
                  int64_t a_bs, int64_t b_bs, int triple, const cwfa_eval_affine* affine, const cwfa_eval_post* post, void* stream);
int cwfa_projection_compose_f32(const float* zproj, const float* xproj, const float* yproj, const float* fill, float* out, int B,
                                int D, int H, int W, int depth_scale, int border, int scale_bars, void* stream);
int cwfa_roi_means_f32(const float* x, const int32_t* boxes, double* out, int T, int D, int H, int W, int N, int64_t t_stride,
                       void* stream);
int cwfa_select_positive_f32(const float* x, int B, int64_t n, int64_t x_bs, int64_t k, float* value, int64_t* count,
                             void* workspace, void* stream);
int cwfa_select_nonzero_f32(const float* x, int B, int64_t n, int64_t x_bs, int64_t k, float* value, int64_t* count,
                            void* workspace, void* stream);

#define CWFA_PREP_MAX_BINS 10239
#define CWFA_PREP_MOMENTS_WORKSPACE 4096
enum { CWFA_PREP_VOL_NONE = 0, CWFA_PREP_VOL_TWO = 1, CWFA_PREP_VOL_LE = 2, CWFA_PREP_VOL_MAXNORM = 3, CWFA_PREP_VOL_MAX_ONLY = 4 };
enum { CWFA_PREP_CLAMP_ZERO = 0, CWFA_PREP_SUB_DIV = 1, CWFA_PREP_DIV_MUL = 2 };
int cwfa_prep_volumes_f16(const void* x, void* out, float* maxbuf, int N, int D, int H0, int W0, int H, int W, int off_h, int off_w,
                          int mode, float t0, float t1, int out_f16, void* stream);
int cwfa_prep_frames_f32(const float* x, float* out, int N, int h, int w, int S0, int S1, int off_y, int off_x, void* stream);
int cwfa_histogram_f32(const float* x, int64_t n, float lo, float hi, const float* edges, int bins, int64_t* counts, int accumulate,
                       void* stream);
int cwfa_prep_apply_f32(float* x, int64_t n, int mode, float a, float b, int flags, void* stream);
int cwfa_moments_f64(const float* x, int64_t n, double c, double* out, double* workspace, int accumulate, void* stream);
int cwfa_stack_mean_std_f32(const float* x, float* mean, float* std, int N, int64_t m, int64_t x_ss, void* stream);

#define CWFA_LION_MAX_TENSORS 96
#define CWFA_LION_BLOCK_ELEMS 4096
typedef struct {
    float* p;
    const float* g;
    float* m;
    int64_t numel;
} cwfa_lion_tensor;
typedef struct {
    int n;
    cwfa_lion_tensor t[CWFA_LION_MAX_TENSORS];
} cwfa_lion_table;
int cwfa_lion_step_f32(const cwfa_lion_table* tab, float lr, float beta1, float beta2, float weight_decay, const float* grad_scale,
// ... 20 lines not shown
```

Measured before the change: 55.81 volumes/s.

## Keep UNet intermediate maps channel-blocked between split-bf16 convolutions

```diff
diff --git a/cwfa_amd/_lib.py b/cwfa_amd/_lib.py
--- a/cwfa_amd/_lib.py
+++ b/cwfa_amd/_lib.py
@@ -113,6 +113,7 @@
     "cwfa_channel_stats_f32": (i, [p, p, i, i, i64, i64, p]),
     "cwfa_bn_fold_f32": (i, [p, d, p, p, p, p, f, p, i, p, p, i, p]),
     "cwfa_maxpool_f32": (i, [p, p, p, p, p, i, i, i, i, i, i, p]),
+    "cwfa_maxpool2x2_blocked8_f32": (i, [p, p, p, p, p, i64, i, i, i, i, p]),
     "cwfa_sample_stats_f32": (i, [p, p, i, i64, p]),
     "cwfa_layernorm_apply_f32": (i, [p, p, p, p, f, p, i, i64, p]),
     "cwfa_convnext_tail_f32": (i, [p, p, p, p, f, p, p, p, p, p, p, p, i, p, i, i, i64, i64, i64, i64, i64, p]),
@@ -142,6 +143,7 @@
     "cwfa_attention_bwd_f32": (i, [p, p, p, p, p, p, p, p, p, i, i, i64, p]),
     "cwfa_split_workspace_bytes": (i64, [i, i, i64]),
     "cwfa_split_input_f32": (i, [p, p, i, i, i64, i64, p, p, i64, p, i64, p]),
+    "cwfa_split_input_blocked8_f32": (i, [p, p, i, i, i64, i64, p, p, i64, p]),
     "cwfa_conv_split_packed_bytes": (i64, [i, i, i]),
     "cwfa_conv_split_pack_f32": (i, [p, p, i, i, i, i, p]),
     "cwfa_conv_split_f32": (i, [p, p, p, i, i, i, i, i, i, i64, C.POINTER(ConvOpts), p]),
diff --git a/cwfa_amd/csrc/conv2d.hip b/cwfa_amd/csrc/conv2d.hip
--- a/cwfa_amd/csrc/conv2d.hip
+++ b/cwfa_amd/csrc/conv2d.hip
@@ -657,6 +657,49 @@
 }
 
 template <bool F16 = false>
+__global__ __launch_bounds__(256) void split_input_blocked8_kernel(const float* __restrict__ x, uint4* __restrict__ ws, int Cin, int CG2,
+                                                                   int64_t HW, int64_t x_bs, const float* __restrict__ sc,
+                                                                   const float* __restrict__ sh, int64_t aff_bs) {
+    const int64_t px = (int64_t)blockIdx.x * 256 + threadIdx.x;
+    if (px >= HW) return;
+    const int cg = blockIdx.y, b = blockIdx.z;
+    float v[8] = {0.f, 0.f, 0.f, 0.f, 0.f, 0.f, 0.f, 0.f};
+    if (cg * 8 < Cin) {
+        const f32x4* src = reinterpret_cast<const f32x4*>(x + (int64_t)b * x_bs + ((int64_t)cg * HW + px) * 8);
+        const f32x4 lo = src[0], hi = src[1];
+#pragma unroll
+        for (int j = 0; j < 4; ++j) {
+            v[j] = lo[j];
+            v[4 + j] = hi[j];
+        }
+        if (sc) {
+#pragma unroll
+            for (int j = 0; j < 8; ++j) v[j] = v[j] * sc[(int64_t)b * aff_bs + cg * 8 + j] + sh[(int64_t)b * aff_bs + cg * 8 + j];
+        }
+    }
+    unsigned short pc[3][8];
+#pragma unroll
+    for (int j = 0; j < 8; ++j) {
+        if constexpr (F16) {
+            pc[0][j] = f16_bits(v[j]);
+            continue;
+        }
+        unsigned short o[3];
+        split3(v[j], o);
+        pc[0][j] = o[0]; pc[1][j] = o[1]; pc[2][j] = o[2];
+    }
+#pragma unroll
+    for (int q = 0; q < (F16 ? 1 : 3); ++q) {
+        uint4 u;
+        u.x = pc[q][0] | ((unsigned)pc[q][1] << 16);
+        u.y = pc[q][2] | ((unsigned)pc[q][3] << 16);
+        u.z = pc[q][4] | ((unsigned)pc[q][5] << 16);
+        u.w = pc[q][6] | ((unsigned)pc[q][7] << 16);
+        ws[(((int64_t)b * 3 + q) * CG2 + cg) * HW + px] = u;
+    }
+}
+
+template <bool F16 = false>
 __global__ __launch_bounds__(256) void split_pack_kernel(const float* __restrict__ w, uint4* __restrict__ out, int Cout, int Cin,
                                                          int nchunks, int taps, int transposed, int64_t total) {
     const int64_t i = (int64_t)blockIdx.x * blockDim.x + threadIdx.x;
@@ -840,6 +883,25 @@
         hipLaunchKernelGGL(split_input_kernel<f16>, dim3((unsigned)((HW + 255) / 256), CG2, B), dim3(256), 0, (hipStream_t)stream, x,
                            reinterpret_cast<uint4*>(ws), Cin, CG2, HW, x_bs, in_scale, in_shift, in_affine_bs, in_add, in_add_bs);
         CWFA_LAUNCH_CHECK("cwfa_split_input_f32");
+        return CWFA_OK;
+    });
+}
+
+extern "C" int cwfa_split_input_blocked8_f32(const float* x, void* ws, int B, int Cin, int64_t HW, int64_t x_bs, const float* in_scale,
+                                             const float* in_shift, int64_t in_affine_bs, void* stream) {
+    CWFA_REQUIRE(x && ws, CWFA_E_INVAL, "cwfa_split_input_blocked8_f32: null pointer");
+    CWFA_REQUIRE(B >= 0 && Cin > 0 && HW >= 0 && B <= 65535, CWFA_E_SHAPE, "cwfa_split_input_blocked8_f32: bad shape");
+    CWFA_REQUIRE(!in_scale == !in_shift, CWFA_E_INVAL, "cwfa_split_input_blocked8_f32: in_scale and in_shift go together");
+    CWFA_REQUIRE(cwfa_aligned16(ws), CWFA_E_ALIGN, "cwfa_split_input_blocked8_f32: workspace must be 16-byte aligned");
+    CWFA_REQUIRE(Cin % 8 == 0 && cwfa_aligned16(x) && (x_bs & 3) == 0, CWFA_E_ALIGN,
+                 "cwfa_split_input_blocked8_f32: a blocked map needs Cin %% 8 == 0 and 16-byte alignment");
+    if (B == 0 || HW == 0) return CWFA_OK;
+    const int CG2 = 2 * ((Cin + 15) / 16);
+    CWFA_REQUIRE((int64_t)3 * CG2 * HW * 16 < (1ll << 31), CWFA_E_SHAPE, "cwfa_split_input_blocked8_f32: one sample's planes must stay below 2 GiB");
+    return cwfa_with_operand([&](auto, auto f16) -> int {
+        hipLaunchKernelGGL(split_input_blocked8_kernel<f16>, dim3((unsigned)((HW + 255) / 256), CG2, B), dim3(256), 0, (hipStream_t)stream, x,
+                           reinterpret_cast<uint4*>(ws), Cin, CG2, HW, x_bs, in_scale, in_shift, in_affine_bs);
+        CWFA_LAUNCH_CHECK("cwfa_split_input_blocked8_f32");
         return CWFA_OK;
     });
 }
diff --git a/cwfa_amd/csrc/conv_split3x3.hip b/cwfa_amd/csrc/conv_split3x3.hip
--- a/cwfa_amd/csrc/conv_split3x3.hip
+++ b/cwfa_amd/csrc/conv_split3x3.hip
@@ -405,6 +405,14 @@
 #pragma unroll
                     for (int r = 0; r < 4; ++r) o4[r] = cwfa_act_ct<ACT1>(acc[mt][nt][r] + bias[r], al[r]);
                     const unsigned pb = (row < p.H && col < p.W) ? (unsigned)(((g >> 1) * HW + row * p.W + col) * 32 + (g & 1) * 16) : OOB;
+                    if (want_stats) {
+#pragma unroll
+                        for (int r = 0; r < 4; ++r) {
+                            const float vm = pb != OOB ? o4[r] : 0.f;
+                            st1[r] += vm;
+                            st2[r] += vm * vm;
+                        }
+                    }
                     cwfa_buffer_store_b128(__builtin_bit_cast(u32x4, o4), ry, pb, (cwave + mt * 16) * plane);
                     continue;
                 }
@@ -874,9 +882,8 @@
                                        (p.o.act == CWFA_ACT_NONE || p.o.act == CWFA_ACT_PRELU)),
                  CWFA_E_ALIGN, "cwfa_conv3x3_split_f32: blocked output needs Cout %% 8 == 0, 16-byte alignment and a bias / PReLU epilogue");
     CWFA_REQUIRE(!(p.o.in_scale && !p.o.in_shift), CWFA_E_INVAL, "cwfa_conv3x3_split_f32: in_scale without in_shift");
-    CWFA_REQUIRE(!p.o.out_stats || (!p.o.out_blocked8 && !p.o.residual && p.o.act2 == CWFA_ACT_NONE &&
-                                    (p.o.act == CWFA_ACT_NONE || p.o.act == CWFA_ACT_PRELU)),
-                 CWFA_E_INVAL, "cwfa_conv3x3_split_f32: out_stats needs an NCHW output and a bias / PReLU epilogue");
+    CWFA_REQUIRE(!p.o.out_stats || (!p.o.residual && p.o.act2 == CWFA_ACT_NONE && (p.o.act == CWFA_ACT_NONE || p.o.act == CWFA_ACT_PRELU)),
+                 CWFA_E_INVAL, "cwfa_conv3x3_split_f32: out_stats needs a bias / PReLU epilogue");
     CWFA_REQUIRE(!((p.o.out_stats || p.o.out_blocked8) && p.o.in_add && p.o.act == CWFA_ACT_NONE), CWFA_E_INVAL,
                  "cwfa_conv3x3_split_f32: out_stats / out_blocked8 with in_add need a PReLU epilogue");
     CWFA_REQUIRE(p.o.act >= 0 && p.o.act <= CWFA_ACT_RELU && p.o.act2 >= 0 && p.o.act2 <= CWFA_ACT_RELU, CWFA_E_INVAL,
diff --git a/cwfa_amd/csrc/lrnn_ops.hip b/cwfa_amd/csrc/lrnn_ops.hip
--- a/cwfa_amd/csrc/lrnn_ops.hip
+++ b/cwfa_amd/csrc/lrnn_ops.hip
@@ -251,6 +251,74 @@
         m[k] = a;
     }
     *reinterpret_cast<float2*>(y + (int64_t)bc * Ho * Wo + (int64_t)oy * Wo + 2 * q) = make_float2(m[0], m[1]);
+}
+
+__global__ __launch_bounds__(256) void maxpool2x2_blocked8_kernel(const float* __restrict__ x, float* __restrict__ y, float* __restrict__ full,
+                                                                  const float* __restrict__ scale, const float* __restrict__ shift,
+                                                                  int64_t aff_bs, int C, int H, int W) {
+    const int Wo = W >> 1, Ho = H >> 1, wq = W >> 2, CB = C >> 3;
+    const int64_t t = (int64_t)blockIdx.x * blockDim.x + threadIdx.x;
+    const int64_t i = t >> 1;
+    if (i >= (int64_t)Ho * wq) return;
+    const int half = (int)(t & 1);
+    const int bcb = blockIdx.y, b = bcb / CB, c0 = (bcb % CB) * 8 + 4 * half;
+    const int oy = (int)(i / wq), q = (int)(i % wq);
+    const float* px = x + ((int64_t)bcb * H * W + (int64_t)(2 * oy) * W + 4 * q) * 8 + 4 * half;
+    f32x4 v[2][4];
+#pragma unroll
+    for (int r = 0; r < 2; ++r)
+#pragma unroll
+        for (int c = 0; c < 4; ++c) v[r][c] = *reinterpret_cast<const f32x4*>(px + ((int64_t)r * W + c) * 8);
+    if (scale) {
+#pragma unroll
+        for (int j = 0; j < 4; ++j) {
+            const float sc = scale[(int64_t)b * aff_bs + c0 + j], sh = shift[(int64_t)b * aff_bs + c0 + j];
+#pragma unroll
+            for (int r = 0; r < 2; ++r)
+#pragma unroll
+                for (int c = 0; c < 4; ++c) v[r][c][j] = v[r][c][j] * sc + sh;
+        }
+    }
+    if (full) {
+#pragma unroll
+        for (int j = 0; j < 4; ++j)
+#pragma unroll
+            for (int r = 0; r < 2; ++r)
+                *reinterpret_cast<f32x4*>(full + (((int64_t)b * C + c0 + j) * H + 2 * oy + r) * W + 4 * q) =
+                    f32x4{v[r][0][j], v[r][1][j], v[r][2][j], v[r][3][j]};
+    }
+    float* py = y + ((int64_t)bcb * Ho * Wo + (int64_t)oy * Wo + 2 * q) * 8 + 4 * half;
+#pragma unroll
+    for (int k = 0; k < 2; ++k) {
+        f32x4 m;
+#pragma unroll
+        for (int j = 0; j < 4; ++j) {
+            float a = -INFINITY;
+            const float v4[4] = {v[0][2 * k][j], v[0][2 * k + 1][j], v[1][2 * k][j], v[1][2 * k + 1][j]};
+#pragma unroll
+            for (int u = 0; u < 4; ++u) a = (v4[u] > a || v4[u] != v4[u]) ? v4[u] : a;
+            m[j] = a;
+        }
+        *reinterpret_cast<f32x4*>(py + 8 * k) = m;
+    }
+}
+
+extern "C" int cwfa_maxpool2x2_blocked8_f32(const float* x, float* y, float* full, const float* scale, const float* shift,
+                                            int64_t affine_bs, int B, int C, int H, int W, void* stream) {
+    CWFA_REQUIRE(x && y, CWFA_E_INVAL, "cwfa_maxpool2x2_blocked8_f32: null pointer");
+    CWFA_REQUIRE(!scale == !shift, CWFA_E_INVAL, "cwfa_maxpool2x2_blocked8_f32: scale and shift go together");
+    CWFA_REQUIRE(B >= 0 && C >= 0 && H > 0 && W > 0 && (H & 1) == 0 && (W & 3) == 0 && (C & 7) == 0, CWFA_E_SHAPE,
+                 "cwfa_maxpool2x2_blocked8_f32: needs C %% 8 == 0, an even H and W %% 4 == 0");
+    CWFA_REQUIRE(affine_bs == 0 || affine_bs == C, CWFA_E_INVAL, "cwfa_maxpool2x2_blocked8_f32: affine tables are [C] or [B][C]");
+    CWFA_REQUIRE(cwfa_aligned16(x) && cwfa_aligned16(y) && (!full || cwfa_aligned16(full)), CWFA_E_ALIGN,
+                 "cwfa_maxpool2x2_blocked8_f32: maps must be 16-byte aligned");
+    CWFA_REQUIRE((int64_t)B * (C >> 3) <= 65535, CWFA_E_SHAPE, "cwfa_maxpool2x2_blocked8_f32: B*C/8 too large");
+    if (B == 0 || C == 0) return CWFA_OK;
+    const int64_t n = (int64_t)(H >> 1) * (W >> 2) * 2;
+    hipLaunchKernelGGL(maxpool2x2_blocked8_kernel, dim3((unsigned)((n + 255) / 256), B * (C >> 3)), dim3(256), 0, (hipStream_t)stream, x, y,
+                       full, scale, shift, affine_bs, C, H, W);
+    CWFA_LAUNCH_CHECK("cwfa_maxpool2x2_blocked8_f32");
+    return CWFA_OK;
 }
 
 extern "C" int cwfa_maxpool_f32(const float* x, float* y, float* full, const float* scale, const float* shift, int B, int C,
diff --git a/cwfa_amd/ops.py b/cwfa_amd/ops.py
--- a/cwfa_amd/ops.py
+++ b/cwfa_amd/ops.py
@@ -585,7 +585,7 @@
 
 
 def conv_writes_stats(pc, act=None, residual=None, act2=None, out_blocked=False, in_add=False):
-    return bool(pc.split and pc.ks == 3 and act in (None, "prelu") and residual is None and act2 is None and not out_blocked
+    return bool(pc.split and pc.ks == 3 and act in (None, "prelu") and residual is None and act2 is None
                 and not (in_add and act is None))
 
 
@@ -654,9 +654,11 @@
         keep.append(in_add)
     o.upshuffle2 = int(up)
     if in_blocked:
-        if not (walk or (pc.split and pc.ks == 3)):
-            raise ValueError("conv2d: channel-blocked input is read by the split-bf16 3x3 kernels only")
-        o.in_blocked8 = 1
+        split1 = pc.split and pc.ks == 1 and in_add is None and Cin % 8 == 0
+        if not (walk or (pc.split and pc.ks == 3) or split1):
+            raise ValueError("conv2d: channel-blocked input is read by the split-bf16 3x3 kernels and, without an added tensor, by "
+                             "the pre-split pass of the split-bf16 1x1 / transposed convolutions only")
+        o.in_blocked8 = 0 if split1 else 1
     if out_blocked:
         ok3 = (pc.split and pc.ks == 3 and pc.cout % 8 == 0 and residual is None and act2 is None and act in (None, "prelu")
                and not split3x3_narrow(pc.cout) and not (in_add is not None and act is None))
@@ -667,7 +669,7 @@
         o.out_blocked8 = 1
     if out_stats is not None:
         if not conv_writes_stats(pc, act, residual, act2, out_blocked, in_add is not None):
-            raise ValueError("conv2d: out_stats needs the split-bf16 3x3 kernel with an NCHW output and a bias / PReLU epilogue")
+            raise ValueError("conv2d: out_stats needs the split-bf16 3x3 kernel with a bias / PReLU epilogue")
         if out_stats.dtype != torch.float64 or out_stats.numel() != 2 * pc.cout or not out_stats.is_cuda:
             raise ValueError("conv2d: out_stats must be a float64 [2*Cout] tensor on the HIP device")
         o.out_stats = out_stats.data_ptr()
@@ -714,8 +716,12 @@
     elif pc.split:
         ws = torch.empty(L.cwfa_split_workspace_bytes(B, Cin, H * W), dtype=torch.uint8, device=x.device)
         per_sample = in_scale is not None and in_scale.numel() == B * Cin and B > 1
-        check(L.cwfa_split_input_f32(_p(x), _p(ws), B, Cin, H * W, xbs, _p(in_scale), _p(in_shift), Cin if per_sample else 0,
-                                     _p(in_add), in_add.stride(0) if in_add is not None else 0, _stream()), "split_input")
+        if in_blocked:
+            check(L.cwfa_split_input_blocked8_f32(_p(x), _p(ws), B, Cin, H * W, xbs, _p(in_scale), _p(in_shift), Cin if per_sample else 0,
+                                                  _stream()), "split_input_blocked8")
+        else:
+            check(L.cwfa_split_input_f32(_p(x), _p(ws), B, Cin, H * W, xbs, _p(in_scale), _p(in_shift), Cin if per_sample else 0,
+                                         _p(in_add), in_add.stride(0) if in_add is not None else 0, _stream()), "split_input")
         o.in_scale = o.in_shift = o.in_add = None
         check(L.cwfa_conv_split_f32(_p(ws), _p(pc.packed), _p(out), B, Cin, H, W, pc.cout, pc.ks, ybs, C.byref(o), _stream()),
               "conv_split")
@@ -785,6 +791,7 @@
 
 
 BLOCKED_MAPS = True
+UNET_BLOCKED = ("inner", "up")
 SPLIT_7X7 = True
 VIRTUAL_CAT = True
 COUPLE_EPILOGUE = True
@@ -796,6 +803,17 @@
 
 def split3x3_narrow(cout):
     return cout <= 48 or 64 < cout <= 96
+
+
+def conv_writes_blocked(pc, act=None, in_add=False):
+    return bool(pc.split and pc.ks == 3 and pc.cout % 8 == 0 and act in (None, "prelu") and not split3x3_narrow(pc.cout)
+                and not (in_add and act is None))
+
+
+def conv_reads_blocked(pc, in_add=False):
+    if in_add or pc.cin % 8 or not pc.split:
+        return False
+    return pc.ks == 1 or (pc.ks == 3 and not split3x3_narrow(pc.cout))
 
 
 SPLIT_3X3_MIN_COUT = 1
@@ -1305,10 +1323,28 @@
     return scale, shift
 
 
-def maxpool(x, Ho, Wo, scale=None, shift=None, want_full=False):
+def maxpool_blocked_ok(C, H, W, Ho, Wo):
+    return C % 8 == 0 and H == 2 * Ho and W == 2 * Wo and W % 4 == 0
+
+
+def maxpool(x, Ho, Wo, scale=None, shift=None, want_full=False, in_blocked=False):
     L = _lib.lib()
     x = _dev(x, "x").contiguous()
     B, Cc, H, W = x.shape
+    if in_blocked:
+        if not maxpool_blocked_ok(Cc, H, W, Ho, Wo):
+            raise ValueError("maxpool: a channel-blocked map needs C % 8 == 0 and exact 2x2 windows with W % 4 == 0")
+        for t in (scale, shift):
+            if t is not None and t.numel() not in (Cc, B * Cc):
+                raise ValueError("maxpool: the load-side affine must be a [C] or [B,C] table")
+        if scale is not None and shift.numel() != scale.numel():
+            raise ValueError("maxpool: scale and shift must have the same size")
+        abs_ = Cc if (scale is not None and scale.numel() == B * Cc and B > 1) else 0
+        y = torch.empty((B, Cc, Ho, Wo), dtype=x.dtype, device=x.device)
+        full = torch.empty_like(x) if want_full else None
+        check(L.cwfa_maxpool2x2_blocked8_f32(_p(x), _p(y), _p(full), _p(scale), _p(shift), abs_, B, Cc, H, W, _stream()),
+              "maxpool2x2_blocked8")
+        return (y, full) if want_full else y
     for t in (scale, shift):
         if t is not None and t.numel() != Cc:
             raise ValueError("maxpool: the load-side affine must be a [C] table")
diff --git a/cwfa_amd/unet.py b/cwfa_amd/unet.py
--- a/cwfa_amd/unet.py
+++ b/cwfa_amd/unet.py
@@ -137,24 +137,41 @@
             return "relu", None
         raise NotImplementedError(f"activation {type(a).__name__} has no HIP epilogue")
 
-    def run(self, x, in_affine=None, in_add=None, out_mask=None):
+    def _stats_in_epilogue(self, bn, pack, kind, add):
+        return bool(STATS_IN_EPILOGUE and bn is not None and _bn_batch_stats(bn) and ops.conv_writes_stats(pack, kind, in_add=add))
+
+    def _writes_blocked(self, li, add=False):
+        conv, act, bn = self._layers()[li]
+        pack, kind = self._packed.get(conv), self._act(act)[0]
+        if not ops.conv_writes_blocked(pack, kind, in_add=add):
+            return False
+        return bn is None or not _bn_batch_stats(bn) or self._stats_in_epilogue(bn, pack, kind, add)
+
+    def blocked_out_ok(self):
+        return self._writes_blocked(1)
+
+    def blocked_in_ok(self):
+        return ops.conv_reads_blocked(self._packed.get(self.block[0]))
+
+    def run(self, x, in_affine=None, in_add=None, out_mask=None, in_blocked=False, out_blocked=False):
         aff = in_affine
         layers = self._layers()
         packs = [self._packed.get(conv) for conv, _, _ in layers]
+        inner = ("inner" in ops.UNET_BLOCKED and self._writes_blocked(0, add=in_add is not None) and ops.conv_reads_blocked(packs[1]))
         for li, (conv, act, bn) in enumerate(layers):
             kind, alpha = self._act(act)
             sc, sh = aff if aff is not None else (None, None)
             add = in_add if li == 0 else None
+            ib, ob = (in_blocked, inner) if li == 0 else (inner, out_blocked)
             if (_MATERIALIZE and ops._split_bf16 < 2 and (sc is not None or add is not None)
                     and (x.shape[2] * x.shape[3]) % 4 == 0):
                 x = ops.plane_affine(x, sc, sh, add=add)
                 sc = sh = add = None
             st = None
-            if (STATS_IN_EPILOGUE and bn is not None and _bn_batch_stats(bn)
-                    and ops.conv_writes_stats(packs[li], kind, in_add=add is not None)):
+            if self._stats_in_epilogue(bn, packs[li], kind, add is not None):
                 st = _bn_stats_buffer(bn, x.device)
             x = ops.conv2d(x, packs[li], bias=conv.bias, act=kind, prelu_alpha=alpha, in_scale=sc,
-                           in_shift=sh, in_add=add, out_stats=st)
+                           in_shift=sh, in_add=add, out_stats=st, in_blocked=ib, out_blocked=ob)
             last = li == len(layers) - 1
             m = out_mask if last else None
             if bn is not None:
@@ -192,14 +209,18 @@
         dy, dx = (h - target_size[0]) // 2, (w - target_size[1]) // 2
         return layer[:, :, dy:(dy + target_size[0]), dx:(dx + target_size[1])]
 
-    def run(self, x, bridge, in_affine=None, out_mask=None):
+    def blocked_in_ok(self):
+        return ops.conv_reads_blocked(self._packed.get(self.up, transposed=True))
+
+    def run(self, x, bridge, in_affine=None, out_mask=None, in_blocked=False, out_blocked=False):
         sc, sh = in_affine if in_affine is not None else (None, None)
         if _MATERIALIZE_UP and ops._split_bf16 < 1 and sc is not None and (x.shape[2] * x.shape[3]) % 4 == 0:
             x = ops.plane_affine(x, sc, sh)
             sc = sh = None
-        up = ops.conv2d(x, self._packed.get(self.up, transposed=True), bias=self.up.bias, in_scale=sc, in_shift=sh)
+        up = ops.conv2d(x, self._packed.get(self.up, transposed=True), bias=self.up.bias, in_scale=sc, in_shift=sh,
+                        in_blocked=in_blocked)
         add = self.center_crop(bridge, up.shape[2:]) if self.skip_conn else None
-        return self.conv_block.run(up, in_add=add, out_mask=out_mask)
+        return self.conv_block.run(up, in_add=add, out_mask=out_mask, out_blocked=out_blocked)
 
     @amp_entry
     def forward(self, x, bridge):
@@ -239,17 +260,29 @@
             n_draw = B * (sum(d.block[0].out_channels for d in list(self.down_path)[:-1]) +
                           sum(u.conv_block.block[0].out_channels for u in self.up_path))
         pool = _DrawPool(n_draw, dev)
+        stages = ops.UNET_BLOCKED
+        nd, blk = len(self.down_path), False
         for i, down in enumerate(self.down_path):
-            x, aff = down.run(x, in_affine=aff)
-            if i != len(self.down_path) - 1:
+            H, W = x.shape[-2:]
+            if i != nd - 1:
+                ob = ("pool" in stages and down.blocked_out_ok() and self.down_path[i + 1].blocked_in_ok()
+                      and ops.maxpool_blocked_ok(down.block[0].out_channels, H, W, W // 2, W // 2))
+            else:
+                ob = "up" in stages and len(self.up_path) > 0 and down.blocked_out_ok() and self.up_path[0].blocked_in_ok()
+            x, aff = down.run(x, in_affine=aff, in_blocked=blk, out_blocked=ob)
+            blk = ob
+            if i != nd - 1:
                 sc, sh = aff if aff is not None else (None, None)
-                x, full = ops.maxpool(x, x.shape[-1] // 2, x.shape[-1] // 2, sc, sh, want_full=True)
+                x, full = ops.maxpool(x, x.shape[-1] // 2, x.shape[-1] // 2, sc, sh, want_full=True, in_blocked=blk)
                 skips.append(full)
                 m = _drop(self.drop_out, B, x.shape[1], dev, pool)
                 aff = _drop_affine(x.shape[1], m) if m is not None else None
         for i, up in enumerate(self.up_path):
             m = _drop(self.drop_out, B, up.conv_block.block[0].out_channels, dev, pool)
-            x, aff = up.run(x, skips[-i - 1], in_affine=aff, out_mask=m)
+            ob = ("up" in stages and i != len(self.up_path) - 1 and up.conv_block.blocked_out_ok()
+                  and self.up_path[i + 1].blocked_in_ok())
+            x, aff = up.run(x, skips[-i - 1], in_affine=aff, out_mask=m, in_blocked=blk, out_blocked=ob)
+            blk = ob
         kind, alpha = UNetConvBlock._act(self.last[1])
         sc, sh = aff if aff is not None else (None, None)
         return ops.conv2d(x, self._packed.get(self.last[0]), bias=self.last[0].bias, act=kind, prelu_alpha=alpha,
diff --git a/include/cwfa_hip.h b/include/cwfa_hip.h
--- a/include/cwfa_hip.h
+++ b/include/cwfa_hip.h
@@ -165,6 +165,8 @@
                                long long* num_batches_tracked, int C, void* stream);
 int cwfa_maxpool_f32(const float* x, float* y, float* full, const float* scale, const float* shift, int B, int C,
                      int H, int W, int Ho, int Wo, void* stream);
+int cwfa_maxpool2x2_blocked8_f32(const float* x, float* y, float* full, const float* scale, const float* shift,
+                                 int64_t affine_bs, int B, int C, int H, int W, void* stream);
 int cwfa_sample_stats_f32(const float* x, double* stats, int B, int64_t CHW, void* stream);
 int cwfa_layernorm_apply_f32(const float* x, const double* stats, const float* w, const float* b, float eps,
                              float* y, int B, int64_t CHW, void* stream);
@@ -180,6 +182,8 @@
 int64_t cwfa_split_workspace_bytes(int B, int Cin, int64_t HW);
 int cwfa_split_input_f32(const float* x, void* ws, int B, int Cin, int64_t HW, int64_t x_bs, const float* in_scale,
                          const float* in_shift, int64_t in_affine_bs, const float* in_add, int64_t in_add_bs, void* stream);
+int cwfa_split_input_blocked8_f32(const float* x, void* ws, int B, int Cin, int64_t HW, int64_t x_bs, const float* in_scale,
+                                  const float* in_shift, int64_t in_affine_bs, void* stream);
 int64_t cwfa_conv_split_packed_bytes(int Cout, int Cin, int ks);
 int cwfa_conv_split_pack_f32(const float* w, void* packed, int Cout, int Cin, int ks, int transposed, void* stream);
 int64_t cwfa_conv3x3_split_packed_bytes(int Cout, int Cin);
```

Measured after the change: 56.03 volumes/s, median of 6. Within noise of the previous version (+0.4%).
